# francescovezzi/quadruped-springs

Hardware: AMD Instinct MI355X
Metric: env-steps/sec (whole node), Go1+PEA jump-in-place, N=8192 envs (higher is better)
Workload: dtype f32

## Files before the change

include/qs_amd.h:

```cpp
#ifndef QS_AMD_H
#define QS_AMD_H
#include <stdint.h>

#ifdef __cplusplus
extern "C" {
#endif

enum { QS_ACT_DEFAULT = 0, QS_ACT_SYMMETRIC = 1, QS_ACT_SYMMETRIC_NO_HIP = 2, QS_ACT_CPG = 3  };
enum { QS_MOTOR_PD = 0, QS_MOTOR_CARTESIAN_PD = 1, QS_MOTOR_TORQUE = 2 };
enum {
    QS_TASK_NO_TASK = 0, QS_TASK_JUMPING_IN_PLACE = 1, QS_TASK_JUMPING_FORWARD = 2,
    QS_TASK_CONT_JUMPING_FORWARD = 3, QS_TASK_CONT_JUMPING_FORWARD2 = 4,
    QS_TASK_JUMPING_IN_PLACE_PPO = 5, QS_TASK_JUMPING_FORWARD_PPO = 6, QS_TASK_BACKFLIP = 7,
    QS_TASK_JUMPING_IN_PLACE_PPO_HP = 8, QS_TASK_JUMPING_FORWARD_PPO_HP = 9, QS_TASK_BACKFLIP_PPO = 10,
    QS_TASK_CONT_JUMPING_FORWARD3 = 11, QS_TASK_CONT_JUMPING_FORWARD_PPO = 12,
    QS_TASK_JUMPING_IN_PLACE_DEMO = 13, QS_TASK_JUMPING_FORWARD_DEMO = 14, QS_TASK_BACKFLIP_DEMO = 15,
    QS_TASK_CONT_JUMPING_FORWARD_DEMO = 16,
};
enum {
    QS_SENS_JOINT_POS = 0, QS_SENS_JOINT_VEL = 1, QS_SENS_PITCH = 2, QS_SENS_HEIGHT = 3, QS_SENS_VEL_Z = 4,
    QS_SENS_LANDING = 5, QS_SENS_JUMPING = 6, QS_SENS_PITCH_RATE = 7, QS_SENS_VEL_X = 8, QS_SENS_BOOL_CONTACT = 9,
    QS_SENS_LIN_VEL = 10, QS_SENS_ANG_VEL = 11, QS_SENS_FEET_POS = 12, QS_SENS_FEET_VEL = 13,
    QS_SENS_PITCH_BACKFLIP = 14, QS_SENS_RPY = 15, QS_SENS_QUAT = 16,
};
#define QS_RAND_GROUND 1
#define QS_RAND_MASSES 2
#define QS_RAND_SPRINGS 4
#define QS_RAND_KEEP 8
enum { QS_WRAP_NONE = 0, QS_WRAP_LANDING = 1, QS_WRAP_GO_TO_REST = 2, QS_WRAP_LANDING2 = 3, QS_WRAP_LANDING_BACKFLIP = 4,
       QS_WRAP_LANDING_BACKFLIP2 = 5, QS_WRAP_LANDING_CONTINUOUS = 6 };
enum { QS_PHASE_POLICY = 0, QS_PHASE_TAKEOFF = 1, QS_PHASE_LANDING = 2, QS_PHASE_REST = 3 };

#define QS_MAX_SENSORS 16
#define QS_MAX_OBS 64
#define QS_STATE_DIM 37
#define QS_PARAM_DIM 24
#define QS_TASK_DIM 48
#define QS_TRACE_DIM 70

typedef struct qs_config {
    int32_t n_envs;
    int32_t action_dim;
    int32_t action_space_mode;
    int32_t motor_control_mode;
    int32_t symm_idx;
    int32_t rl_interface;
    int32_t task;
    int32_t n_sensors;
    int32_t sensors[QS_MAX_SENSORS];
    int32_t obs_dim;
    int32_t enable_springs;
    int32_t enable_filter;
    int32_t enable_interp;
    int32_t action_repeat;
    int32_t solver_iters;
    int32_t settle_steps;
    int32_t max_sim_steps;
    int32_t randomizer_flags;
    int32_t noise_enabled;
    int32_t auto_reset;
    int32_t reset_lookahead;
    int32_t env_id_offset;
    int32_t wrapper_mode;
    uint64_t seed;
    double dt;
    double filt_b[3], filt_a[3];
    float gravity;
    float kp[3], kd[3], tau_max[3];
    float cmd_lo[12], cmd_hi[12];
    float settle_cmd[12];
    float settle_action[12];
    float spring_k[3], spring_b[3], spring_rest[3];
    float fallen_height;
    float leg_len[3];
    float contact_erp, joint_erp, warmstart, vel_cap;
    float obs_noise_std[QS_MAX_OBS];
    float task_p[16];
    float contact_slop;
    int32_t body_contacts;
    int32_t self_collision;
    int32_t info_fields;
    int32_t payload_soft;
    float support_margin;
    float reserved_f[2];
    float cpg_phi[16];
    float cpg_lo[5], cpg_hi[5];
    float cpg_clearance, cpg_penetration, cpg_coupling, cpg_alpha;
    float solver_residual_threshold;
    int32_t friction_cone;
    float landing_action[12];
    float landing_kp, landing_kd;
    float rest_kp, rest_kd, rest_time;
    float reserved_h[3];
    float unit_inertia[4][6];
} qs_config;

typedef struct qs_handle qs_handle;

int qs_create(const qs_config* cfg, int device, qs_handle** out);
typedef struct qs_rack {
    int32_t on;
    float anchor_pos[3];
    float anchor_quat[4];
} qs_rack;
int qs_create_ex(const qs_config* cfg, const qs_rack* rack, int device, qs_handle** out);
int qs_set_rack(qs_handle* h, const uint8_t* mask, int hung);
void qs_destroy(qs_handle* h);
int qs_set_stream(qs_handle* h, void* hip_stream);
int qs_reset(qs_handle* h, const uint8_t* mask);
int qs_reset_to(qs_handle* h, const uint8_t* mask, const float* states);
int qs_get_obs(qs_handle* h, float* obs );
int qs_set_demo(qs_handle* h, const float* rows, int length);
int qs_set_demo_counter(qs_handle* h, const uint8_t* mask, const int32_t* values);
int qs_step(qs_handle* h, const float* actions , float* obs , float* rew ,
            uint8_t* done , uint8_t* truncated );
int qs_get_state(qs_handle* h, float* state );
enum { QS_FRAME_LINK = 1, QS_FRAME_WORLD = 2 };
int qs_set_external_wrench(qs_handle* h, const uint8_t* mask, const float* wrench , const int32_t* substeps , int frame);
int qs_set_state(qs_handle* h, const float* state );
enum {
    QS_INFO_FOOT_FORCE = 0, QS_INFO_FOOT_CONTACT = 1, QS_INFO_TORQUE = 2, QS_INFO_SPRING_TORQUE = 3, QS_INFO_TASK = 4,
    QS_INFO_N_INVALID = 5, QS_INFO_PARAMS = 6, QS_INFO_COUNTERS = 7, QS_INFO_LAST_ACTION = 8, QS_INFO_TERMINAL_OBS = 9,
    QS_INFO_FILTERED_ACTION = 11,
    QS_INFO_REWARD_END = 12,
    QS_INFO_PAYLOAD_BLOCK = 13,
    QS_INFO_WRAPPER = 10,
    QS_INFO_EXTERNAL_WRENCH = 14,
    QS_INFO_RACK = 15,
};
int qs_info_dim(const qs_handle* h, int which);
int qs_get_info(qs_handle* h, int which, float* out );
enum { QS_PARAM_MU = 0, QS_PARAM_SPRING_K = 1, QS_PARAM_SPRING_B = 2, QS_PARAM_KP = 3, QS_PARAM_KD = 4, QS_PARAM_ALL = 5 };
int qs_set_params(qs_handle* h, int which, const float* vals);
int qs_stats(qs_handle* h, uint64_t* settle_substeps, uint64_t* resets);
int qs_step_fused(qs_handle* h, const float* actions, float* fused);
typedef struct qs_host_result {
    const float* obs;
    const float* rew;
    const uint8_t* done;
    const uint8_t* truncated;
    const float* terminal_rows;
    int32_t terminal_cap;
} qs_host_result;
int qs_host_step_begin(qs_handle* h, const float* actions);
int qs_host_step_end(qs_handle* h, qs_host_result* out);

enum { QS_COUNTER_SETTLE_SUBSTEPS = 0,
       QS_COUNTER_RESETS = 1,
       QS_COUNTER_LOOKAHEAD_SERVED = 2,
       QS_COUNTER_LOOKAHEAD_SETTLED = 3,
       QS_COUNTER_LIMIT_PATH_SUBSTEPS = 4,
       QS_COUNTER_SELF_NARROW_SUBSTEPS = 5,
       QS_COUNTER_RESET_STALLS = 6,
       QS_COUNTER_LOOKAHEAD_BACKLOG = 7      };
int qs_counter(qs_handle* h, int which, uint64_t* value);
int qs_counters_async(qs_handle* h, uint64_t* dev_out);
int qs_enable_timing(qs_handle* h, int on);
int qs_last_step_kernel_ms(qs_handle* h, float* ms);
int qs_settle_lanes(qs_handle* h, int on);
int qs_set_trace(qs_handle* h, int env, float* rows);

typedef struct qs_norm qs_norm;
int qs_norm_create(int n_envs, int obs_dim, double clip_obs, double clip_reward, double gamma, double epsilon, int device, qs_norm** out);
void qs_norm_destroy(qs_norm* h);
int qs_norm_set_stream(qs_norm* h, void* hip_stream);
int qs_norm_set_stats(qs_norm* h, const double* obs_mean, const double* obs_var, double obs_count, double ret_mean, double ret_var, double ret_count);
int qs_norm_dims(const qs_norm* h, int* n_envs, int* obs_dim, int* device);
int qs_norm_get_stats(qs_norm* h, double* obs_mean, double* obs_var, double* obs_count, double* ret_mean, double* ret_var, double* ret_count);
int qs_norm_reset(qs_norm* h, float* obs , int training, int norm_obs);
int qs_norm_step(qs_norm* h, float* obs , float* rew , const uint8_t* done , float* term_obs ,
                 int training, int norm_obs, int norm_reward, float* raw_obs, float* raw_rew);

typedef struct qs_norm_io {
    float* obs; float* rew; const uint8_t* done; const uint8_t* trunc; float* term_obs; float* tail_rows; int32_t tail_cap;
    float* out_obs; float* out_rew; uint8_t* out_done; uint8_t* out_trunc; float* out_tail;
    float* raw_obs; float* raw_rew;
    const uint64_t* tail_count;
} qs_norm_io;
int qs_norm_step_io(qs_norm* h, const qs_norm_io* io, int training, int norm_obs, int norm_reward);
int qs_host_set_norm(qs_handle* h, qs_norm* norm, int training, int norm_obs, int norm_reward, float* raw_obs, float* raw_rew);

typedef struct qs_camera {
    float target[3];
    float distance, yaw_deg, pitch_deg, fov_deg, near_clip, far_clip;
    int32_t follow_base;
    int32_t draw_payload;
} qs_camera;
int qs_render(qs_handle* h, const int32_t* env_ids, int m, const qs_camera* cam, int width, int height,
              uint32_t* rgba , float* depth , int32_t* seg );
int qs_render_states(const float* states, const float* params, int m, const qs_camera* cam, int width, int height,
                     uint32_t* rgba, float* depth, int32_t* seg, void* stream);

#define QS_POLICY_MAX_HIDDEN 4
enum { QS_POLICY_ACT_NONE = 0, QS_POLICY_ACT_TANH = 1, QS_POLICY_ACT_RELU = 2 };
typedef struct qs_policy qs_policy;
typedef struct qs_policy_desc {
    int32_t n_envs, n_policies, obs_dim, action_dim, n_hidden, hidden[QS_POLICY_MAX_HIDDEN];
    int32_t activation;
    int32_t squash_output;
    int32_t has_bias;
    float clip_lo, clip_hi;
} qs_policy_desc;
int qs_policy_create(const qs_policy_desc* d, int device, qs_policy** out);
void qs_policy_destroy(qs_policy* p);
int qs_policy_set_stream(qs_policy* p, void* hip_stream);
int qs_policy_param_count(const qs_policy* p);
int qs_policy_set_params(qs_policy* p, const float* dev_params);
int qs_policy_act(qs_policy* p, const float* obs, const float* eps, const float* log_std, float* actions, float* mean_out, float* log_prob);

typedef struct qs_ac qs_ac;
int qs_ac_create(const qs_policy_desc* actor, const qs_policy_desc* critic, int device, qs_ac** out);
void qs_ac_destroy(qs_ac* h);
int qs_ac_set_stream(qs_ac* h, void* hip_stream);
int qs_ac_set_params(qs_ac* h, const float* actor_params, const float* critic_params);
int qs_ac_collect(qs_ac* h, const float* obs, const float* eps, const float* log_std, float* env_actions, float* obs_row, float* action_row,
                  float* value_row, float* log_prob_row);
int qs_ac_values(qs_ac* h, const float* obs, const uint8_t* mask_or_null, float* values_out);
int qs_ac_bootstrap(qs_ac* h, const float* terminal_obs, const uint8_t* truncated, float gamma, float* rewards_inout);
int qs_gae(const float* rewards, const float* values, const float* episode_starts, const float* last_values, const uint8_t* last_dones, int T, int N,
           float gamma, float lambda, float* advantages, float* returns, void* hip_stream);

typedef struct qs_ppo qs_ppo;
typedef struct qs_ppo_hyper {
    float clip_range, ent_coef, vf_coef;
    float max_grad_norm;
    int32_t normalize_advantage;
    int32_t reserved;
    double lr, beta_one, beta_two, adam_eps;
} qs_ppo_hyper;
enum { QS_PPO_STAT_POLICY_LOSS = 0, QS_PPO_STAT_VALUE_LOSS = 1, QS_PPO_STAT_ENTROPY_LOSS = 2, QS_PPO_STAT_APPROX_KL = 3,
       QS_PPO_STAT_CLIP_FRACTION = 4, QS_PPO_STAT_GRAD_NORM = 5, QS_PPO_STAT_REFUSED = 6, QS_PPO_STAT_LOSS = 7, QS_PPO_N_STATS = 8 };
int qs_ppo_create(const qs_policy_desc* actor, const qs_policy_desc* critic, int max_batch, int device, qs_ppo** out);
void qs_ppo_destroy(qs_ppo* h);
int qs_ppo_set_stream(qs_ppo* h, void* hip_stream);
int qs_ppo_bind(qs_ppo* h, float* actor_params, float* critic_params, float* log_std, float* exp_avg, float* exp_avg_sq);
int qs_ppo_grad(qs_ppo* h, const float* observations, const float* actions, const float* old_log_prob, const float* advantages, const float* returns,
                long long total, const long long* indices, int batch, const qs_ppo_hyper* hyper, float* grad_out, float* stats_out);
int qs_ppo_adam(qs_ppo* h, const float* grad, const qs_ppo_hyper* hyper, int step, float* stats_inout);
int qs_ppo_refusals(qs_ppo* h, unsigned long long* out);

struct qs_snapshot_info {
    uint64_t bytes;
    int32_t n_envs, row_floats, rec_floats, push_floats, obs_dim;
    int32_t layout_version;
    uint64_t layout_digest;
    uint64_t config_digest;
};
int qs_snapshot_info(const qs_handle* h, struct qs_snapshot_info* out);
int qs_snapshot(qs_handle* h, const uint8_t* mask, float* rows);
int qs_restore(qs_handle* h, const uint8_t* mask, const float* rows);
int qs_fork(qs_handle* h, const int32_t* src_of);
int qs_norm_get_returns(qs_norm* h, double* returns );
int qs_norm_set_returns(qs_norm* h, const double* returns );

const char* qs_last_error(void);
const char* qs_version(void);
#define QS_ABI_VERSION 9
int qs_abi_version(void);

#ifdef __cplusplus
}
#endif
#endif
```

quadruped-springs_amd/csrc/qs_core.h:

```cpp
#pragma once
#include "qs_lane.h"
#include "qs_layout.h"
#include "../../include/qs_amd.h"

#if defined(QS_PROFILE_PHASES) && defined(__HIPCC__)
__device__ unsigned long long qs_phase_cycles[48];
__device__ unsigned long long qs_phase_t0, qs_phase_sub0;
#endif
#if defined(QS_PROFILE_PHASES) && defined(__HIP_DEVICE_COMPILE__)
#define QS_PHASE_BEGIN if (blockIdx.x == 0 && threadIdx.x == 0) qs_phase_t0 = __builtin_readcyclecounter();
#define QS_PHASE_G(k) if (blockIdx.x == 0 && threadIdx.x == 0) { unsigned long long n_ = __builtin_readcyclecounter(); qs_phase_cycles[k] += n_ - qs_phase_t0; qs_phase_t0 = n_; }
#define QS_PHASE(k) QS_PHASE_G(k)
#define QS_PHASE_SUB(k) if (blockIdx.x == 0 && threadIdx.x == 0) { qs_phase_cycles[16 + ((k) < 15 ? (k) : 15)] += __builtin_readcyclecounter() - qs_phase_sub0; }
#define QS_PHASE_SUB_BEGIN if (blockIdx.x == 0 && threadIdx.x == 0) qs_phase_sub0 = __builtin_readcyclecounter();
#define QS_PHASE_END
#elif defined(QS_COUNT_PHASES) && defined(__HIP_DEVICE_COMPILE__)
#define QS_PHASE_BEGIN { __builtin_amdgcn_sched_barrier(0); asm volatile("; QS_PHASE_MARK 0"); __builtin_amdgcn_sched_barrier(0); }
#define QS_PHASE_G(k) { __builtin_amdgcn_sched_barrier(0); asm volatile("; QS_PHASE_MARK " #k); __builtin_amdgcn_sched_barrier(0); }
#define QS_PHASE(k) QS_PHASE_G(k)
#define QS_PHASE_SUB(k)
#define QS_PHASE_SUB_BEGIN
#define QS_PHASE_END
#else
#define QS_PHASE_BEGIN
// ... 1145 lines not shown
        M rare_mine = qgt(T::quad_sum(qflag(any_lim)), V(0.5f));
        State s_r = s; Out o_r = o;
        PayRows pay_c, pay_r;
        if (!HOT && soft) payload_rows(cfg, Pr, s, vs, Rx, Ry, Rz, Sm, Ld, blk, pay_c);
        if (!HOT && rack) rack_rows(cfg, s, vs, Rx, Ry, Rz, Sm, Ld, blk, pay_c);
        QS_PHASE_G(39)
        if (!HOT && T::any(qor(any_lim, any_extra))) {
            Row xr[12];
#pragma unroll
            for (int r = 0; r < 3; r++) xr[r] = rows[r];
#pragma unroll
            for (int r = 3; r < 12; r++) {
                Row& e_ = xr[r];
                e_.rhs = zero; e_.dinv = zero; e_.act = zero; e_.diag = zero;
#pragma unroll
                for (int i = 0; i < 6; i++) e_.w[i] = zero;
#pragma unroll
                for (int i = 0; i < 3; i++) { e_.jq[i] = zero; e_.u[i] = zero; }
            }
            M extra_live = qlt(one, zero);
#if defined(QS_PROBE_WARM) && defined(__HIP_DEVICE_COMPILE__)
            M probe_live[2] = {qlt(one, zero), qlt(one, zero)};
#endif
#if defined(QS_PROBE_LAZY) && defined(__HIP_DEVICE_COMPILE__)
            M probe_rule[2][4];
#pragma unroll
            for (int a_ = 0; a_ < 2; a_++)
#pragma unroll
                for (int m_ = 0; m_ < 4; m_++) probe_rule[a_][m_] = qlt(one, zero);
#endif
            const M lim_env = qgt(T::quad_sum(qflag(any_lim)), V(0.5f));
            if (T::any(any_extra)) {
                const V bigh = V(1e9f);
                V hh[5] = {qsel(qlt(h_trunk, V(THR_TRUNK)), h_trunk, bigh), qsel(qlt(h_hip, V(THR_HIP)), h_hip, bigh), qsel(qlt(h_th_hi, V(THR_THIGH)), h_th_hi, bigh),
                           qsel(qlt(h_th_lo, V(THR_THIGH)), h_th_lo, bigh), qsel(qlt(h_cf_hi, V(THR_CALF)), h_cf_hi, bigh)};
                V sgz = qsel(qlt(Rz.z, zero), -one, one), sga = qsel(qlt(az, zero), -one, one);
                V sg2 = qsel(qlt(gx2, zero), -one, one), sg3 = qsel(qlt(gx3, zero), -one, one);
                V rad = HIP_CYL_R * qrsqrt(qmax(one - az * az, V(1e-12f)));
                V3v pc[5];
                pc[0] = mk3<V>(fx * TRUNK_HALF[0], sy * TRUNK_HALF[1], sgz * (-TRUNK_HALF[2]));
                pc[1] = p1 - Y * (sga * HIP_CYL_HALF_LEN) - (Rz - Y * az) * rad;
                V3v toff = X2 * (sg2 * THIGH_HALF[0]) + Y * (sga * THIGH_HALF[1]);
                pc[2] = p2 - toff; pc[3] = p3 - toff;
                pc[4] = p3 - X3 * (sg3 * CALF_HALF[0]) - Y * (sga * CALF_HALF[1]);
                const float depth[5] = {0.0f, 1.0f, 2.0f, 2.0f, 3.0f};
                const M foot_off = qnot(act_m);
#pragma unroll
                for (int pass = 0; pass < 3; pass++) {
                    const int slot = pass - 1;
                    const M elig = pass == 0 ? foot_off : qlt(zero, one);
                    V best = qsel(elig, hh[0], bigh), bi = zero;
#pragma unroll
                    for (int i = 1; i < 5; i++) { M m = qand(elig, qlt(hh[i], best)); best = qsel(m, hh[i], best); bi = qsel(m, V((float)i), bi); }
                    if (!T::any(qlt(best, V(1e8f)))) { if (pass == 0) continue; else break; }
                    bi = qsel(qlt(best, V(1e8f)), bi, V(4.0f));
                    V3v pt = pc[0]; V dep = V(depth[0]);
#pragma unroll
                    for (int i = 1; i < 5; i++) {
                        M m = qgt(bi, V(i - 0.5f));
                        pt = mk3<V>(qsel(m, pc[i].x, pt.x), qsel(m, pc[i].y, pt.y), qsel(m, pc[i].z, pt.z));
                        dep = qsel(m, V(depth[i]), dep);
                    }
#pragma unroll
                    for (int i = 0; i < 5; i++) hh[i] = qsel(qand(qlt(best, V(1e8f)), qand(qgt(bi, V(i - 0.5f)), qlt(bi, V(i + 0.5f)))), bigh, hh[i]);
                    V dist_x = qsel(qlt(best, V(1e8f)), best, zero);
                    V f1 = qflag(qgt(dep, V(0.5f))), f2 = qflag(qgt(dep, V(1.5f))), f3 = qflag(qgt(dep, V(2.5f)));
                    V3v e1 = cross(ax1, pt - p1) * f1, e2 = cross(Y, pt - p2) * f2, e3 = cross(Y, pt - p3) * f3;
                    V3v jan = cross(pt, Rz);
                    V reln = jan.x * vs.a.x + jan.y * vs.a.y + jan.z * vs.a.z + Rz.x * vs.l.x + Rz.y * vs.l.y + Rz.z * vs.l.z +
                             dot(Rz, e1) * s.qd[0] + dot(Rz, e2) * s.qd[1] + dot(Rz, e3) * s.qd[2];
                    V pen_x = dist_x + cfg.contact_slop;
                    M live = qand(qlt(best, V(1e8f)), qor(qor(lim_env, qle(pen_x, zero)), qgt((-reln) - pen_x * inv_dt, V(-cfg.support_margin))));
#if defined(QS_PROBE_LAZY) && defined(__HIP_DEVICE_COMPILE__)
#pragma unroll
                    for (int m_ = 0; m_ < 4; m_++) probe_rule[slot][m_] = qand(qlt(best, V(1e8f)), qor(qor(lim_env, qle(pen_x, zero)), qgt((-reln) - pen_x * inv_dt, V(-0.25f * (float)((1 << m_) >> 1)))));
                    live = qlt(best, V(1e8f));
#endif
                    extra_live = qor(extra_live, live);
#if defined(QS_PROBE_WARM) && defined(__HIP_DEVICE_COMPILE__)
                    probe_live[pass == 0 ? 0 : slot] = pass == 0 ? probe_live[0] : live;
#endif
                    if (!T::any(live)) continue;
                    V act_x = qflag(live);
                    if (pass == 0) {
                        Row t0_, t1_, t2_;
                        QS_CONTACT_ROW_AT(t0_, Rz, true, pt, e1, e2, e3, dist_x, act_x)
                        QS_CONTACT_ROW_AT(t1_, (mk3<V>(-Ry.x, -Ry.y, -Ry.z)), false, pt, e1, e2, e3, dist_x, act_x)
                        QS_CONTACT_ROW_AT(t2_, Rx, false, pt, e1, e2, e3, dist_x, act_x)
                        const Row* tt_[3] = {&t0_, &t1_, &t2_};
#pragma unroll
                        for (int r = 0; r < 3; r++) {
                            Row& d_ = xr[r]; const Row& a_ = *tt_[r];
#pragma unroll
                            for (int i = 0; i < 6; i++) d_.w[i] = qsel(live, a_.w[i], d_.w[i]);
#pragma unroll
                            for (int i = 0; i < 3; i++) { d_.jq[i] = qsel(live, a_.jq[i], d_.jq[i]); d_.u[i] = qsel(live, a_.u[i], d_.u[i]); }
                            d_.rhs = qsel(live, a_.rhs, d_.rhs); d_.dinv = qsel(live, a_.dinv, d_.dinv); d_.diag = qsel(live, a_.diag, d_.diag); d_.act = qsel(live, a_.act, d_.act);
                        }
                    } else {
                        QS_CONTACT_ROW_AT(xr[3 + 3 * slot], Rz, true, pt, e1, e2, e3, dist_x, act_x)
                        QS_CONTACT_ROW_AT(xr[4 + 3 * slot], (mk3<V>(-Ry.x, -Ry.y, -Ry.z)), false, pt, e1, e2, e3, dist_x, act_x)
                        QS_CONTACT_ROW_AT(xr[5 + 3 * slot], Rx, false, pt, e1, e2, e3, dist_x, act_x)
                    }
                }
            }
            rare_mine = qgt(T::quad_sum(qflag(qor(any_lim, extra_live))), V(0.5f));
#if defined(QS_PROBE_WARM) && defined(__HIP_DEVICE_COMPILE__)
            {
                unsigned long long* pc = reinterpret_cast<const QsDevCfg&>(cfg).counters + 2;
                const float pts_leg = qflag(probe_live[0]) + qflag(probe_live[1]);
                const float pts = T::quad_sum(pts_leg), two = T::quad_sum(pts_leg > 1.5f ? 1.0f : 0.0f);
                const bool mine = rare_mine, lim = lim_env;
                const bool simple = mine && !lim && two < 0.5f;
                const unsigned long long b0 = __ballot(mine), b1 = __ballot(mine && lim), b2 = __ballot(mine && !lim && two > 0.5f),
                                         b3 = __ballot(simple && pts < 1.5f), b4 = __ballot(simple && pts > 1.5f && pts < 2.5f), b5 = __ballot(simple && pts > 2.5f);
                if (threadIdx.x == 0) {
                    atomicAdd(&pc[0], (unsigned long long)(__popcll(b0) / 4)); atomicAdd(&pc[1], (unsigned long long)(__popcll(b1) / 4));
                    atomicAdd(&pc[2], (unsigned long long)(__popcll(b2) / 4)); atomicAdd(&pc[3], (unsigned long long)(__popcll(b3) / 4));
                    atomicAdd(&pc[4], (unsigned long long)(__popcll(b4) / 4)); atomicAdd(&pc[5], (unsigned long long)(__popcll(b5) / 4));
                    atomicAdd(&pc[6], 1ull);
                    if (b0) atomicAdd(&pc[7], 1ull);
                    if (b0 && b0 == (b3 | b4 | b5)) atomicAdd(&pc[8], 1ull);
                }
            }
#endif
            if (T::any(rare_mine)) {
                T::count_rare_path(cfg);
                if (T::any(any_lim)) { QS_LIMIT_ROWS(xr + 9) }
                QS_PHASE_G(40)
                V lam12[12], plam[6];
                if (soft || rack) pay_r = pay_c;
                RareSolver<T, CONE>::solve(cfg, Pr.mu, xr, (soft || rack) ? &pay_r : nullptr, rare_mine, s.warm * cfg.warmstart * rows[0].act, T::wave_scratch(scratch_row), lam12, plam);
                integrate_rare(cfg, s_r, o_r, xr, lam12, Sm, Ld, BK, R, (soft || rack) ? &pay_r : nullptr, plam, active);
#if defined(QS_PROBE_LAZY) && defined(__HIP_DEVICE_COMPILE__)
                {
                    unsigned long long* pc = reinterpret_cast<const QsDevCfg&>(cfg).counters + 2;
                    const bool ext_q = T::quad_sum(qflag(any_extra)) > 0.5f;
                    const bool zero_q = !lim_env && T::quad_sum(qabs(lam12[3]) + qabs(lam12[6])) == 0.0f;
                    const unsigned long long b0 = __ballot(ext_q), b1 = __ballot(ext_q && zero_q);
                    if (threadIdx.x == 0) { atomicAdd(&pc[0], (unsigned long long)(__popcll(b0) / 4)); atomicAdd(&pc[1], (unsigned long long)(__popcll(b1) / 4)); }
#pragma unroll
                    for (int m_ = 0; m_ < 4; m_++) {
                        const bool keep_q = lim_env || T::quad_sum(qflag(probe_rule[0][m_]) + qflag(probe_rule[1][m_])) > 0.5f;
                        const float w0 = !probe_rule[0][m_] && qabs(lam12[3]) > 0.0f ? 1.0f : 0.0f, w1 = !probe_rule[1][m_] && qabs(lam12[6]) > 0.0f ? 1.0f : 0.0f;
                        const bool wrong_q = T::quad_sum(w0 + w1) > 0.5f;
                        const unsigned long long bk = __ballot(ext_q && keep_q), bw = __ballot(ext_q && wrong_q);
                        if (threadIdx.x == 0) { atomicAdd(&pc[2 + 2 * m_], (unsigned long long)(__popcll(bk) / 4)); atomicAdd(&pc[3 + 2 * m_], (unsigned long long)(__popcll(bw) / 4)); }
                    }
                }
#endif
                QS_PHASE_G(45)
            }
        }
        if (RACK ? rack : (SOFT || (!HOT && soft))) {
            if (HOT && !RACK) payload_rows(cfg, Pr, s, vs, Rx, Ry, Rz, Sm, Ld, blk, pay_c);
            if (HOT && RACK) rack_rows(cfg, s, vs, Rx, Ry, Rz, Sm, Ld, blk, pay_c);
            if (cfg.solver_residual_threshold > 0.0f) solve_and_integrate<3, true, true>(cfg, Pr.mu, s, o, rows, Sm, Ld, BK, R, &pay_c);
            else solve_and_integrate<3, false, true>(cfg, Pr.mu, s, o, rows, Sm, Ld, BK, R, &pay_c);
            if (HOT && !RACK) payload_integrate(cfg, blk, pay_c);
            if (HOT && RACK) rack_store(blk, pay_c);
        } else {
            if (cfg.solver_residual_threshold > 0.0f) solve_and_integrate<3, true>(cfg, Pr.mu, s, o, rows, Sm, Ld, BK, R);
            else solve_and_integrate<3, false>(cfg, Pr.mu, s, o, rows, Sm, Ld, BK, R);
        }
        if (!HOT) {
#pragma unroll
            for (int j = 0; j < 3; j++) s.qd[j] = qsel(rare_mine, s_r.qd[j], s.qd[j]);
            s.vang = mk3<V>(qsel(rare_mine, s_r.vang.x, s.vang.x), qsel(rare_mine, s_r.vang.y, s.vang.y), qsel(rare_mine, s_r.vang.z, s.vang.z));
            s.vlin = mk3<V>(qsel(rare_mine, s_r.vlin.x, s.vlin.x), qsel(rare_mine, s_r.vlin.y, s.vlin.y), qsel(rare_mine, s_r.vlin.z, s.vlin.z));
            s.warm = qsel(rare_mine, s_r.warm, s.warm); o.foot_force = qsel(rare_mine, o_r.foot_force, o.foot_force);
            if (soft) { keep_rare_payload(pay_c, pay_r, rare_mine); payload_integrate(cfg, blk, pay_c); }
            if (rack) { keep_rare_payload(pay_c, pay_r, rare_mine); rack_store(blk, pay_c); }
        }
#undef QS_LIMIT_ROWS
#undef QS_CONTACT_ROW_AT
        } else {
            o.foot_force = zero; s.warm = zero;
        }
        QS_PHASE(11)
        s.pos.x = s.pos.x + dt * s.vlin.x; s.pos.y = s.pos.y + dt * s.vlin.y; s.pos.z = s.pos.z + dt * s.vlin.z;
        {
            V th2 = dot(s.vang, s.vang) * (dt * dt);
            V sc = V(0.5f * dt) * (one - th2 * (1.0f / 24.0f) * (one - th2 * (1.0f / 80.0f)));
            V dw = one - th2 * 0.125f * (one - th2 * (1.0f / 48.0f));
            V dx = s.vang.x * sc, dy = s.vang.y * sc, dz = s.vang.z * sc;
            V nx = dw * s.qx + dx * s.qw + dy * s.qz - dz * s.qy;
            V ny = dw * s.qy - dx * s.qz + dy * s.qw + dz * s.qx;
            V nz = dw * s.qz + dx * s.qy - dy * s.qx + dz * s.qw;
            V nw = dw * s.qw - dx * s.qx - dy * s.qy - dz * s.qz;
            V inv = qrsqrt(nx * nx + ny * ny + nz * nz + nw * nw);
            s.qx = nx * inv; s.qy = ny * inv; s.qz = nz * inv; s.qw = nw * inv;
        }
#pragma unroll
        for (int j = 0; j < 3; j++) s.q[j] = s.q[j] + dt * s.qd[j];
        QS_PHASE(12)
        QS_PHASE_END
        return HOT && hand_over_next ? 2 : 0;
    }
};

}
```

quadruped-springs_amd/csrc/qs_hip.hip:

```cpp
#include <hip/hip_runtime.h>
#include <stdio.h>
#include <stdlib.h>
#include <string.h>
#include <new>
#include "qs_env.h"
#include "qs_host.h"

using qs::Env;
using E = Env<LaneDev>;

#define QS_TILE_FLOATS (QS_ENVS_PER_WAVE * QS_REC_END)
#ifndef QS_LEAN_WAVES
#define QS_LEAN_WAVES(W) ((W) == 2)
#endif

enum { TILE_INFO = QS_INFO_END, TILE_ALL = QS_REC_END };
__device__ __forceinline__ int tile_extent(const qs_config& cfg, bool store) {
    if (cfg.payload_soft) return TILE_ALL;
    if (cfg.info_fields) return store ? TILE_INFO : QS_HOT_ALL;
    if (cfg.action_space_mode == QS_ACT_CPG || E::demo_task(cfg.task)) return QS_HOT_ALL;
    if (cfg.wrapper_mode != QS_WRAP_NONE) return QS_HOT_WRAP;
    return QS_HOT;
}
__device__ __forceinline__ void keep_loaded(const float4& v) { asm volatile("" ::"v"(v.x), "v"(v.y), "v"(v.z), "v"(v.w)); }
__device__ __forceinline__ void keep_loaded(float v) { asm volatile("" ::"v"(v)); }
template <int PER> __device__ __forceinline__ void tile_load_rounds(float4* __restrict__ dst, const float4* __restrict__ src, int nenv, int stride4, int per_rt) {
    constexpr int MAX_PER = QS_REC_END / 4;
    constexpr int ROUNDS = PER > 0 ? (QS_ENVS_PER_WAVE * PER + QS_WAVE - 1) / QS_WAVE : (QS_ENVS_PER_WAVE * MAX_PER + QS_WAVE - 1) / QS_WAVE;
    const int per = PER > 0 ? PER : per_rt, total = QS_ENVS_PER_WAVE * per;
    const unsigned inv = ((1u << 20) + (unsigned)per - 1u) / (unsigned)per;
    float4 v[ROUNDS];
#pragma unroll
    for (int r = 0; r < ROUNDS; r++) {
        const int i = (int)threadIdx.x + r * QS_WAVE;
        const bool in = (PER > 0 && (QS_ENVS_PER_WAVE * PER) % QS_WAVE == 0) || i < total;
        const int e = PER > 0 ? i / PER : (int)(((unsigned)i * inv) >> 20), o = i - e * per;
        v[r] = src[in ? (e < nenv ? e : 0) * (QS_REC / 4) + o : 0];
    }
    if (!(PER > 0 && (QS_ENVS_PER_WAVE * PER) % QS_WAVE == 0)) {
#pragma unroll
        for (int r = 0; r < ROUNDS; r++) keep_loaded(v[r]);
    }
#pragma unroll
    for (int r = 0; r < ROUNDS; r++) {
        const int i = (int)threadIdx.x + r * QS_WAVE;
        if ((PER > 0 && (QS_ENVS_PER_WAVE * PER) % QS_WAVE == 0) || i < total) {
            const int e = PER > 0 ? i / PER : (int)(((unsigned)i * inv) >> 20), o = i - e * per;
            dst[e * stride4 + o] = v[r];
        }
    }
}
__device__ __forceinline__ void tile_load(float* lds, const float* __restrict__ g, int first_env, int n_envs, int extent, int stride = QS_REC_END) {
    const float4* src = reinterpret_cast<const float4*>(g + (size_t)first_env * QS_REC);
    float4* dst = reinterpret_cast<float4*>(lds);
    const int nenv = min(QS_ENVS_PER_WAVE, n_envs - first_env);
    if (extent == QS_HOT) tile_load_rounds<QS_HOT / 4>(dst, src, nenv, stride / 4, 0);
    else if (extent == QS_SETTLE_END) tile_load_rounds<QS_SETTLE_END / 4>(dst, src, nenv, stride / 4, 0);
    else tile_load_rounds<0>(dst, src, nenv, stride / 4, extent / 4);
}
template <int PER> __device__ __forceinline__ void tile_store_rounds(float4* __restrict__ dst, const float4* __restrict__ src, int nenv, int stride4, int b4, int per_rt) {
    constexpr int MAX_PER = QS_REC_END / 4;
    constexpr int ROUNDS = PER > 0 ? (QS_ENVS_PER_WAVE * PER + QS_WAVE - 1) / QS_WAVE : (QS_ENVS_PER_WAVE * MAX_PER + QS_WAVE - 1) / QS_WAVE;
    const int per = PER > 0 ? PER : per_rt, total = nenv * per;
    const unsigned inv = ((1u << 20) + (unsigned)per - 1u) / (unsigned)per;
    float4 v[ROUNDS];
#pragma unroll
    for (int r = 0; r < ROUNDS; r++) {
        const int i = (int)threadIdx.x + r * QS_WAVE;
        const int e = PER > 0 ? i / PER : (int)(((unsigned)i * inv) >> 20), o = i - e * per + b4;
        v[r] = src[i < total ? e * stride4 + o : 0];
    }
#pragma unroll
    for (int r = 0; r < ROUNDS; r++) keep_loaded(v[r]);
#pragma unroll
    for (int r = 0; r < ROUNDS; r++) {
        const int i = (int)threadIdx.x + r * QS_WAVE;
        if (i < total) { const int e = PER > 0 ? i / PER : (int)(((unsigned)i * inv) >> 20), o = i - e * per + b4; dst[e * (QS_REC / 4) + o] = v[r]; }
    }
}
__device__ __forceinline__ void tile_store(const float* lds, float* __restrict__ g, int first_env, int n_envs, int begin, int end, int stride = QS_REC_END) {
    float4* dst = reinterpret_cast<float4*>(g + (size_t)first_env * QS_REC);
    const float4* src = reinterpret_cast<const float4*>(lds);
    const int nenv = min(QS_ENVS_PER_WAVE, n_envs - first_env);
    if (begin == QS_RW_BEGIN && end == QS_HOT) tile_store_rounds<(QS_HOT - QS_RW_BEGIN) / 4>(dst, src, nenv, stride / 4, QS_RW_BEGIN / 4, 0);
    else if (begin == QS_RW_BEGIN && end == QS_SETTLE_END) tile_store_rounds<(QS_SETTLE_END - QS_RW_BEGIN) / 4>(dst, src, nenv, stride / 4, QS_RW_BEGIN / 4, 0);
    else tile_store_rounds<0>(dst, src, nenv, stride / 4, begin / 4, (end - begin) / 4);
}

__device__ __forceinline__ void obs_store(const float* s_obs, int nrow, int od, int first, float* __restrict__ obs_out, bool fused, float* __restrict__ obs_keep) {
    const unsigned inv = (65536u + (unsigned)od - 1u) / (unsigned)od;
    const int row = fused ? od + 2 : od, total = nrow * od;
    constexpr int ROUNDS = QS_ENVS_PER_WAVE * QS_MAX_OBS / QS_WAVE;
    float v[ROUNDS];
#pragma unroll
    for (int r = 0; r < ROUNDS; r++) {
        const int i = (int)threadIdx.x + r * QS_WAVE;
        const int e = (int)(((unsigned)i * inv) >> 16), o = i - e * od;
        v[r] = s_obs[i < total ? e * QS_MAX_OBS + o : 0];
    }
#pragma unroll
    for (int r = 0; r < ROUNDS; r++) keep_loaded(v[r]);
#pragma unroll
    for (int r = 0; r < ROUNDS; r++) {
        const int i = (int)threadIdx.x + r * QS_WAVE;
        if (i < total) {
            const int e = (int)(((unsigned)i * inv) >> 16), o = i - e * od;
            obs_out[(size_t)(first + e) * row + o] = v[r];
            obs_keep[(size_t)first * od + i] = v[r];
        }
    }
}

struct LookAhead {
    float* slots;
    int* cur;
    int* handed;
    int K;
};
#define QS_COHORTS 5
#define QS_MAX_SLICE 2048
struct SettleLanes { float* staging; const int2* stage_jobs; int n_env_waves, slice; int wave0[QS_COHORTS + 1] ,
                     spawn[QS_COHORTS], last[QS_COHORTS], settle_n[QS_COHORTS]; };
struct TraceTap { float* rows; int env; };
struct DemoTab { const float* rows; int length; };
struct TermTail { float* rows; int cap, parity; };
struct PushTab { float* rows; };
enum { QS_PUSH_F = 8, QS_PUSH_REM = 6, QS_PUSH_FRAME = 7 };
enum { CTL_SETTLE_SUBSTEPS = 0, CTL_RESETS = 1, CTL_SERVED = 2, CTL_SETTLED = 3, CTL_BACKLOG = 4, CTL_STALLS = 6,
       CTL_R = 8 , CTL_TERM_CNT = 8 + QS_COHORTS , CTL_DEV = 10 + QS_COHORTS ,
       CTL_PUSH_REFUSED = 22 + QS_COHORTS ,
       CTL_RENDER_REFUSED = 23 + QS_COHORTS ,
       CTL_FORK_REFUSED = 24 + QS_COHORTS ,
       CTL_N = 25 + QS_COHORTS };

__device__ __forceinline__ float copy_settled(float* rec, const float* __restrict__ src, bool block) {
    static_assert(R_PARAMS == 0 && R_PARAMS + QS_PARAM_DIM == R_POS, "parameters and rigid-body state are one range");
    const int lane = threadIdx.x & 3;
    constexpr int END_A = R_WARM + 4, NA = (END_A + 3) / 4;
    constexpr int NB = (R_TAU_SPRING + 12 - R_FOOT_FORCE) / 4;
    constexpr int NC = QS_BLOCK_DIM / 4;
    static_assert((R_TAU_SPRING + 12 - R_FOOT_FORCE) % 4 == 0 && QS_BLOCK_DIM % 4 == 0, "whole rounds");
    float a[NA], b[NB], c[NC];
#pragma unroll
    for (int k = 0; k < NA; k++) { const int i = lane + 4 * k; a[k] = src[i < END_A ? i : 0]; }
#pragma unroll
    for (int k = 0; k < NB; k++) b[k] = src[R_FOOT_FORCE + lane + 4 * k];
    const float ninv = src[R_N_INVALID], tag = src[R_EPISODE];
    if (block) {
#pragma unroll
        for (int k = 0; k < NC; k++) c[k] = src[R_BLOCK + lane + 4 * k];
    }
#pragma unroll
    for (int k = 0; k < NA; k++) { const int i = lane + 4 * k; if (i < END_A) rec[i] = a[k]; }
#pragma unroll
    for (int k = 0; k < NB; k++) rec[R_FOOT_FORCE + lane + 4 * k] = b[k];
    if (lane == 0) rec[R_N_INVALID] = ninv;
    if (block) {
#pragma unroll
        for (int k = 0; k < NC; k++) rec[R_BLOCK + lane + 4 * k] = c[k];
    }
    return tag;
}
__device__ __forceinline__ void quad_row_store(float* __restrict__ dst, const float* row, int n) {
    float v[QS_MAX_OBS / 4];
#pragma unroll
    for (int k = 0; k < QS_MAX_OBS / 4; k++) { const int i = (int)(threadIdx.x & 3) + 4 * k; v[k] = row[i < n ? i : 0]; }
#pragma unroll
    for (int k = 0; k < QS_MAX_OBS / 4; k++) keep_loaded(v[k]);
#pragma unroll
    for (int k = 0; k < QS_MAX_OBS / 4; k++) { const int i = (int)(threadIdx.x & 3) + 4 * k; if (i < n) dst[i] = v[k]; }
}
__device__ __forceinline__ bool lookahead_take(const LookAhead& la, unsigned long long* __restrict__ ctl, float* rec, int env, int X, bool block, bool count = true) {
    if (la.K == 0) return false;
    const float* slot = la.slots + ((size_t)env * la.K + (size_t)(X % la.K)) * QS_REC;
    const float tag = copy_settled(rec, slot, block);
    const bool ready = qs::f2i(tag) == X;
    if ((threadIdx.x & 3) == 0) {
        la.cur[env] = X;
        if (count) atomicAdd(&ctl[ready ? CTL_SERVED : CTL_STALLS], 1ull);
    }
    return ready;
}
__device__ __forceinline__ void zero_tile_tail(float* lds, int from, int stride) {
    const int per = stride - from;
    for (int i = threadIdx.x; i < QS_ENVS_PER_WAVE * per; i += QS_WAVE) { const int e = i / per; lds[e * stride + from + (i - e * per)] = 0.0f; }
}

__global__ __launch_bounds__(QS_WAVE, 1) void k_init(const qs_config* __restrict__ cfgp, float* __restrict__ recs) {
    const qs_config& cfg = *cfgp;
    int env = blockIdx.x * QS_ENVS_PER_WAVE + (threadIdx.x >> 2);
    if (env >= cfg.n_envs) return;
    float* r = recs + (size_t)env * QS_REC;
    for (int i = threadIdx.x & 3; i < QS_REC_END; i += 4) r[i] = 0.0f;
    LaneDev::sync();
    if ((threadIdx.x & 3) == 0) qs::init_record_row(r);
    E::randomize(cfg, r, (uint32_t)(env + cfg.env_id_offset), -1, true);
}

template <bool CONE, int WAVES, bool SOFT, bool RACK = false> static __device__ __forceinline__ void step_body(const qs_config* __restrict__ cfgp, float* __restrict__ recs,
                                                 const float* __restrict__ actions, float* __restrict__ obs_out,
                                                 float* __restrict__ rew_out, uint8_t* __restrict__ done_out,
                                                 uint8_t* __restrict__ trunc_out, float* __restrict__ obs_keep,
                                                 float* __restrict__ term_obs, LookAhead la,
                                                 unsigned long long* __restrict__ stats, SettleLanes lanes, TraceTap tap, DemoTab demo, TermTail tail,
                                                 PushTab push) {
    using E = Env<LaneDev, CONE, false, false, RACK>;
    using EH = Env<LaneDev, CONE, true, SOFT, RACK>;
    extern __shared__ __attribute__((aligned(16))) float s_dyn[];
    const qs_config& cfg = *cfgp;
    const int ls = (RACK || cfg.payload_soft) ? (int)QS_REC_END : (int)QS_INFO_END;
    float* const s_rec = s_dyn;
    float* const s_obs = s_dyn + QS_ENVS_PER_WAVE * ls;
    float* const s_act = s_obs + QS_ENVS_PER_WAVE * QS_MAX_OBS;
    QS_PHASE_BEGIN
    if (tail.rows && blockIdx.x == 0 && threadIdx.x == 0) stats[CTL_TERM_CNT + (tail.parity ^ 1)] = 0ull;
    const bool settling = (int)blockIdx.x >= lanes.n_env_waves;
    const int sw = (int)blockIdx.x - lanes.n_env_waves;
    int cohort = 0;
#pragma unroll
    for (int c = 1; c < QS_COHORTS; c++) cohort += settling && sw >= lanes.wave0[c] ? 1 : 0;
    const int first = settling ? cohort * lanes.slice + (sw - lanes.wave0[cohort]) * QS_ENVS_PER_WAVE : (int)blockIdx.x * QS_ENVS_PER_WAVE;
    const int limit = settling ? cohort * lanes.slice + (int)stats[CTL_R + cohort] : cfg.n_envs;
    if (first >= limit) return;
    const int settle_n = settling ? lanes.settle_n[cohort] : 0;
    if (settling && settle_n == 0) return;
    float* const base = settling ? lanes.staging : recs;
    const int slot = threadIdx.x >> 2;
    const int env = first + slot;
    const bool valid = env < limit;
    const int d = cfg.action_dim, od = cfg.obs_dim;
    QS_PHASE(26)
    float a_pre[3] = {0.0f, 0.0f, 0.0f};
    float p_rem = 0.0f;
    int2 job = make_int2(0, 0);
    if (!settling) {
#pragma unroll
        for (int j = 0; j < 3; j++) {
            const int k = (int)(threadIdx.x & 3u) + 4 * j;
            if (k < d && valid) a_pre[j] = actions[(size_t)env * d + k];
        }
        if (push.rows && valid) p_rem = push.rows[(size_t)env * QS_PUSH_F + QS_PUSH_REM];
    } else job = lanes.stage_jobs[valid ? env : first];
    const bool spawn = settling && lanes.spawn[cohort], last = settling && lanes.last[cohort];
    const int load_extent = settling ? (spawn ? 0 : ((RACK || cfg.payload_soft) ? (int)TILE_ALL : (int)QS_SETTLE_END)) : (RACK ? (int)TILE_ALL : tile_extent(cfg, false));
    if (load_extent > 0) tile_load(s_rec, base, first, limit, load_extent, ls);
    if (spawn || last) zero_tile_tail(s_rec, load_extent, ls);
    QS_PHASE(27)
    if (!settling) {
#pragma unroll
        for (int j = 0; j < 3; j++) {
            const int k = (int)(threadIdx.x & 3u) + 4 * j;
            if (k < d) s_act[slot * 12 + k] = a_pre[j];
        }
    }
    QS_PHASE(28)
    __syncthreads();
    QS_PHASE(29)
    float* rec = s_rec + slot * ls;
    float* ob = s_obs + slot * QS_MAX_OBS;
    if (cfg.info_fields && !settling && (threadIdx.x & 3) == 0) rec[QS_INFO_END - 1] = 0.0f;
    const uint32_t gid = (uint32_t)((settling ? job.x : env) + cfg.env_id_offset);
    if (spawn) { E::settle_spawn(cfg, rec, gid, job.y); LaneDev::sync(); }
    const bool any_trace = tap.rows != nullptr && !settling && tap.env >= first && tap.env < first + QS_ENVS_PER_WAVE;
    QS_PHASE(13)
    float* const trow = any_trace && env == tap.env ? tap.rows : nullptr;
    const bool any_push = push.rows != nullptr && __any(p_rem > 0.0f);
    const float* const prow = any_push ? push.rows + (size_t)(valid ? env : first) * QS_PUSH_F : nullptr;
    typename E::StepOut r;
    {
        const typename EH::StepOut rh = EH::template step<false, QS_LEAN_WAVES(WAVES)>(cfg, rec, s_act + slot * 12, ob, gid, settle_n, trow, any_trace, demo.rows, demo.length, 0, prow);
        r.reward = rh.reward; r.done = rh.done; r.trunc = rh.trunc; r.resume = rh.resume;
    }
    if (__builtin_expect(r.resume >= 0, 0)) r = E::template step<true>(cfg, rec, s_act + slot * 12, ob, gid, settle_n, trow, any_trace, demo.rows, demo.length, r.resume, prow);
    QS_PHASE(14)
    if (settling) {
        if (valid && (threadIdx.x & 3) == 0) atomicAdd(&stats[CTL_SETTLE_SUBSTEPS], (unsigned long long)settle_n);
        __syncthreads();
        tile_store(s_rec, base, first, limit, spawn ? 0 : (int)QS_RW_BEGIN,
                   (RACK || cfg.payload_soft) ? (int)TILE_ALL : (last ? (int)TILE_INFO : (int)QS_SETTLE_END), ls);
        return;
    }
    const bool dn = r.done > 0.5f;
    if (any_push && valid && p_rem > 0.0f && (threadIdx.x & 3) == 0)
        push.rows[(size_t)env * QS_PUSH_F + QS_PUSH_REM] = dn ? 0.0f : fmaxf(p_rem - (float)cfg.action_repeat, 0.0f);
    if (valid && (threadIdx.x & 3) == 0) {
        if (rew_out) { rew_out[env] = r.reward; done_out[env] = dn ? 1 : 0; trunc_out[env] = r.trunc > 0.5f ? 1 : 0; }
        else {
            float* row = obs_out + (size_t)env * (od + 2);
            row[od] = r.reward; row[od + 1] = (dn ? 1.0f : 0.0f) + (r.trunc > 0.5f ? 2.0f : 0.0f);
        }
    }
    bool any_reset = false;
    if (cfg.auto_reset) {
        const bool do_reset = dn && valid;
        if (__builtin_expect(__any(do_reset), 0)) {
            any_reset = true;
            LaneDev::sync();
            bool ahead = false;
            if (do_reset) {
                quad_row_store(term_obs + (size_t)env * od, ob, od);
                if ((threadIdx.x & 3) == 0) atomicAdd(&stats[CTL_RESETS], 1ull);
                if (tail.rows) {
                    int at = 0;
                    if ((threadIdx.x & 3) == 0) at = (int)atomicAdd(&stats[CTL_TERM_CNT + tail.parity], 1ull);
                    at = __shfl(at, (int)(threadIdx.x & ~3u));
                    if (at < tail.cap) {
                        float* row = tail.rows + (size_t)at * (od + 1);
                        if ((threadIdx.x & 3) == 0) row[0] = qs::i2f(env);
                        quad_row_store(row + 1, ob, od);
                    }
                }
                ahead = lookahead_take(la, stats, rec, env, qs::f2i(rec[R_EPISODE]) + 1, RACK || cfg.payload_soft != 0);
            }
            LaneDev::sync();
            if (__builtin_expect(__any(do_reset && !ahead), 0)) {
                __syncthreads();
                tile_store(s_rec, recs, first, cfg.n_envs, QS_RW_BEGIN, RACK ? (int)TILE_ALL : tile_extent(cfg, true), ls);
                obs_store(s_obs, min(QS_ENVS_PER_WAVE, cfg.n_envs - first), od, first, obs_out, rew_out == nullptr, obs_keep);
                __syncthreads();
                E::reset(cfg, rec, ob, gid, true);
                if (do_reset && !ahead && (threadIdx.x & 3) == 0) atomicAdd(&stats[CTL_SETTLE_SUBSTEPS], (unsigned long long)cfg.settle_steps);
                LaneDev::sync();
                if (do_reset) {
                    float* g = recs + (size_t)env * QS_REC;
                    const int end = RACK ? (int)TILE_ALL : tile_extent(cfg, true);
                    for (int i = threadIdx.x & 3; i < end; i += 4) g[i] = rec[i];
                    for (int i = threadIdx.x & 3; i < od; i += 4) {
                        if (rew_out) obs_out[(size_t)env * od + i] = ob[i];
                        else obs_out[(size_t)env * (od + 2) + i] = ob[i];
                        obs_keep[(size_t)env * od + i] = ob[i];
                    }
                }
                return;
            }
            if (do_reset) E::reset(cfg, rec, ob, gid, false);
        }
    }
    __syncthreads();
    tile_store(s_rec, recs, first, cfg.n_envs, any_reset ? 0 : (int)QS_RW_BEGIN, RACK ? (int)TILE_ALL : tile_extent(cfg, true), ls);
    obs_store(s_obs, min(QS_ENVS_PER_WAVE, cfg.n_envs - first), od, first, obs_out, rew_out == nullptr, obs_keep);
    QS_PHASE(15)
}

#define QS_STEP_ARGS const qs_config* __restrict__ cfgp, float* __restrict__ recs, const float* __restrict__ actions, float* __restrict__ obs_out,    \
                     float* __restrict__ rew_out, uint8_t* __restrict__ done_out, uint8_t* __restrict__ trunc_out, float* __restrict__ obs_keep, \
                     float* __restrict__ term_obs, LookAhead la, unsigned long long* __restrict__ stats, SettleLanes lanes, TraceTap tap, DemoTab demo, TermTail tail, \
                     PushTab push
#define QS_STEP_PASS cfgp, recs, actions, obs_out, rew_out, done_out, trunc_out, obs_keep, term_obs, la, stats, lanes, tap, demo, tail, push
template <bool CONE, bool SOFT> __global__ __launch_bounds__(QS_WAVE, 1) void k_step(QS_STEP_ARGS) { step_body<CONE, 1, SOFT>(QS_STEP_PASS); }
template <bool CONE, bool SOFT> __global__ __launch_bounds__(QS_WAVE, 2) void k_step_dense(QS_STEP_ARGS) { step_body<CONE, 2, SOFT>(QS_STEP_PASS); }
template <bool CONE> __global__ __launch_bounds__(QS_WAVE, 1) void k_step_rack(QS_STEP_ARGS) { step_body<CONE, 1, CONE, true>(QS_STEP_PASS); }
template <bool CONE> __global__ __launch_bounds__(QS_WAVE, 2) void k_step_dense_rack(QS_STEP_ARGS) { step_body<CONE, 2, CONE, true>(QS_STEP_PASS); }

__global__ void k_lookahead_publish(unsigned long long* __restrict__ ctl, const float* __restrict__ staging, const int2* __restrict__ stage_jobs,
                                    LookAhead la, int cohort, int slice) {
    const int n = (int)ctl[CTL_R + cohort];
    const float* src = staging + (size_t)cohort * slice * QS_REC;
    const int2* jobs = stage_jobs + (size_t)cohort * slice;
    for (size_t i = (size_t)blockIdx.x * blockDim.x + threadIdx.x; i < (size_t)n * QS_REC_END; i += (size_t)gridDim.x * blockDim.x) {
        const int e = (int)(i / QS_REC_END), f = (int)(i % QS_REC_END);
        const int2 job = jobs[e];
        if (job.y <= la.cur[job.x]) continue;
        float* dst = la.slots + ((size_t)job.x * la.K + (size_t)(job.y % la.K)) * QS_REC;
        dst[f] = f == R_EPISODE ? qs::i2f(job.y) : src[(size_t)e * QS_REC + f];
        if (f == 0) atomicAdd(&ctl[CTL_SETTLED], 1ull);
    }
}
__global__ __launch_bounds__(1024) void k_lookahead_plan(unsigned long long* __restrict__ ctl, LookAhead la, int n_envs, int2* __restrict__ stage_jobs, int cohort,
                                                          int slice, int base_cap, int take, int offset) {
    __shared__ int s_count, s_want, s_urgent;
    if (threadIdx.x == 0) { s_count = 0; s_want = 0; s_urgent = 0; }
    __syncthreads();
    int2* dst = stage_jobs + (size_t)cohort * slice;
    for (int pass = 0; pass < 2; pass++) {
        const int cap = take ? (pass == 0 ? slice : (s_count > base_cap ? 0 : base_cap)) : 0;
        for (int i = threadIdx.x; i < n_envs; i += blockDim.x) {
            const int e = (i + offset) % n_envs;
            const int X = la.cur[e];
            int h = la.handed[e];
            if (h < X) h = X;
            const int want = X + la.K - h;
            if (want <= 0 || (4 * want > la.K) != (pass == 0)) continue;
            atomicAdd(&s_want, want);
            if (cap <= 0) continue;
            const int at = atomicAdd(&s_count, want);
            int took = 0;
            for (int j = 0; j < want && at + j < cap; j++) { dst[at + j] = make_int2(e, h + 1 + j); took++; }
            if (took) la.handed[e] = h + took;
        }
        __syncthreads();
        if (threadIdx.x == 0 && pass == 0) { if (s_count > slice) s_count = slice; s_urgent = s_count; }
        __syncthreads();
    }
    if (threadIdx.x == 0) {
        int n = s_count;
        const int lim = s_urgent > base_cap ? s_urgent : base_cap;
        if (n > lim) n = lim;
        if (take) ctl[CTL_R + cohort] = (unsigned long long)n;
        ctl[CTL_BACKLOG] = (unsigned long long)(s_want - (take ? n : 0));
    }
}
__global__ void k_lookahead_requeue(unsigned long long* __restrict__ ctl, LookAhead la, const int2* __restrict__ stage_jobs, int slice) {
    for (int c = 0; c < QS_COHORTS; c++) {
        const int n = (int)ctl[CTL_R + c];
        for (int i = threadIdx.x; i < n; i += blockDim.x) { const int2 job = stage_jobs[(size_t)c * slice + i]; atomicMin(&la.handed[job.x], job.y - 1); }
    }
    __syncthreads();
    if (threadIdx.x == 0) for (int c = 0; c < QS_COHORTS; c++) ctl[CTL_R + c] = 0;
}

template <bool CONE, bool RACK> static __device__ __forceinline__ void reset_body(const qs_config* __restrict__ cfgp, float* __restrict__ recs,
                                                      const uint8_t* __restrict__ mask, float* __restrict__ obs_keep,
                                                      unsigned long long* __restrict__ stats, const float* __restrict__ states, LookAhead la,
                                                      float* __restrict__ push_rows, float* s_rec, float* s_obs) {
    using E = Env<LaneDev, CONE, false, false, RACK>;
    const qs_config& cfg = *cfgp;
    const int first = blockIdx.x * QS_ENVS_PER_WAVE;
    const int slot = threadIdx.x >> 2, env = first + slot;
    const bool valid = env < cfg.n_envs;
    const bool sel = valid && (mask == nullptr || mask[env] != 0);
    if (!__any(sel)) return;
    tile_load(s_rec, recs, first, cfg.n_envs, QS_REC_END);
    const int od = cfg.obs_dim;
    __syncthreads();
    float* rec = s_rec + slot * QS_REC_END;
    float* ob = s_obs + slot * QS_MAX_OBS;
    const uint32_t gid = (uint32_t)((valid ? env : 0) + cfg.env_id_offset);
    bool ahead = false;
    if (sel) {
        if (states == nullptr) ahead = lookahead_take(la, stats, rec, env, qs::f2i(rec[R_EPISODE]) + 1, RACK || cfg.payload_soft != 0);
        else if (la.K > 0 && (threadIdx.x & 3) == 0) la.cur[env] = qs::f2i(rec[R_EPISODE]) + 1;
        if ((threadIdx.x & 3) == 0) atomicAdd(&stats[CTL_RESETS], 1ull);
        if ((threadIdx.x & 3) == 0) push_rows[(size_t)env * QS_PUSH_F + QS_PUSH_REM] = 0.0f;
    }
    bool write_back = false;
    if (states) {
        if (sel) {
            E::randomize(cfg, rec, gid, qs::f2i(rec[R_EPISODE]) + 1, false);
            for (int i = threadIdx.x & 3; i < 37; i += 4) rec[R_POS + i] = states[(size_t)env * 37 + i];
            for (int i = threadIdx.x & 3; i < 4; i += 4) rec[R_WARM + i] = 0.0f;
            if (RACK) for (int i = threadIdx.x & 3; i < 6; i += 4) rec[R_BLOCK + RK_LAM + i] = 0.0f;
            if ((threadIdx.x & 3) == 0) {
                for (int i = 0; i < 4; i++) { rec[R_FOOT_FORCE + i] = 0.0f; rec[R_FOOT_CONTACT + i] = 0.0f; }
                rec[R_N_INVALID] = 0.0f;
                for (int i = 0; i < 24; i++) rec[R_TAU_PD + i] = 0.0f;
            }
        }
        LaneDev::sync();
        if (cfg.payload_soft) { E::place_block(cfg, rec); LaneDev::sync(); }
        E::reset(cfg, rec, ob, gid, false);
        LaneDev::sync();
        if (sel)
            for (int i = threadIdx.x & 3; i < 12 + 24 + 24; i += 4) rec[R_LAST_ACTION + i] = 0.0f;
        write_back = sel;
    } else {
        LaneDev::sync();
        if (ahead) {
            E::reset(cfg, rec, ob, gid, false);
            float* g = recs + (size_t)env * QS_REC;
            for (int i = threadIdx.x & 3; i < QS_REC_END; i += 4) g[i] = rec[i];
            for (int i = threadIdx.x & 3; i < od; i += 4) obs_keep[(size_t)env * od + i] = ob[i];
        }
        const bool settle = sel && !ahead;
        if (__any(settle)) {
            __syncthreads();
            E::reset(cfg, rec, ob, gid, true);
            if (settle && (threadIdx.x & 3) == 0) atomicAdd(&stats[CTL_SETTLE_SUBSTEPS], (unsigned long long)cfg.settle_steps);
        }
        write_back = settle;
    }
    __syncthreads();
    if (write_back) {
        float* g = recs + (size_t)env * QS_REC;
        for (int i = threadIdx.x & 3; i < QS_REC_END; i += 4) g[i] = rec[i];
        for (int i = threadIdx.x & 3; i < od; i += 4) obs_keep[(size_t)env * od + i] = ob[i];
    }
}
#define QS_RESET_ARGS const qs_config* __restrict__ cfgp, float* __restrict__ recs, const uint8_t* __restrict__ mask, float* __restrict__ obs_keep, \
                      unsigned long long* __restrict__ stats, const float* __restrict__ states, LookAhead la, float* __restrict__ push_rows
#define QS_RESET_PASS cfgp, recs, mask, obs_keep, stats, states, la, push_rows
#define QS_RESET_LDS __shared__ __attribute__((aligned(16))) float s_rec[QS_TILE_FLOATS]; __shared__ __attribute__((aligned(16))) float s_obs[QS_ENVS_PER_WAVE * QS_MAX_OBS];
template <bool CONE> __global__ __launch_bounds__(QS_WAVE, 1) void k_reset(QS_RESET_ARGS) { QS_RESET_LDS reset_body<CONE, false>(QS_RESET_PASS, s_rec, s_obs); }
template <bool CONE> __global__ __launch_bounds__(QS_WAVE, 1) void k_reset_rack(QS_RESET_ARGS) { QS_RESET_LDS reset_body<CONE, true>(QS_RESET_PASS, s_rec, s_obs); }

template <bool CONE, bool RACK> static __device__ __forceinline__ void lookahead_fill_body(const qs_config* __restrict__ cfgp, LookAhead la, float* s_rec, float* s_obs) {
    using E = Env<LaneDev, CONE, false, false, RACK>;
    const qs_config& cfg = *cfgp;
    const int slot = threadIdx.x >> 2;
    const long long j = (long long)blockIdx.x * QS_ENVS_PER_WAVE + slot, total = (long long)cfg.n_envs * la.K;
    const int env = (int)((j < total ? j : 0) % cfg.n_envs), episode = (int)((j < total ? j : 0) / cfg.n_envs);
    float* rec = s_rec + slot * QS_REC_END;
    for (int i = threadIdx.x & 3; i < QS_REC_END; i += 4) rec[i] = 0.0f;
    LaneDev::sync();
    if ((threadIdx.x & 3) == 0) rec[R_EPISODE] = qs::i2f(episode - 1);
    LaneDev::sync();
    E::reset(cfg, rec, s_obs + slot * QS_MAX_OBS, (uint32_t)(env + cfg.env_id_offset), true);
    LaneDev::sync();
    if (j < total) {
        float* g = la.slots + ((size_t)env * la.K + (size_t)(episode % la.K)) * QS_REC;
        for (int i = threadIdx.x & 3; i < QS_REC_END; i += 4) g[i] = rec[i];
        if (episode == la.K - 1 && (threadIdx.x & 3) == 0) { la.handed[env] = la.K - 1; la.cur[env] = -1; }
    }
}
template <bool CONE> __global__ __launch_bounds__(QS_WAVE, 1) void k_lookahead_fill(const qs_config* __restrict__ cfgp, LookAhead la) { QS_RESET_LDS lookahead_fill_body<CONE, false>(cfgp, la, s_rec, s_obs); }
template <bool CONE> __global__ __launch_bounds__(QS_WAVE, 1) void k_lookahead_fill_rack(const qs_config* __restrict__ cfgp, LookAhead la) { QS_RESET_LDS lookahead_fill_body<CONE, true>(cfgp, la, s_rec, s_obs); }
#undef QS_RESET_LDS

__global__ void k_gather(const float* __restrict__ recs, int n, int off, int dim, float* __restrict__ out, int as_int) {
    int i = blockIdx.x * blockDim.x + threadIdx.x;
    if (i >= n * dim) return;
    float v = recs[(size_t)(i / dim) * QS_REC + off + i % dim];
    out[i] = as_int ? (float)qs::f2i(v) : v;
}
__global__ void k_scatter(float* __restrict__ recs, int n, int off, int dim, const float* __restrict__ in, int zero_warm) {
    int i = blockIdx.x * blockDim.x + threadIdx.x;
    if (i >= n * dim) return;
    recs[(size_t)(i / dim) * QS_REC + off + i % dim] = in[i];
    if (zero_warm && i % dim < 4) recs[(size_t)(i / dim) * QS_REC + R_WARM + i % dim] = 0.0f;
}
__global__ void k_task_info(const float* __restrict__ recs, int n, float* __restrict__ out, int demo, int info) {
    int e = blockIdx.x * blockDim.x + threadIdx.x;
    if (e >= n) return;
    const float* r = recs + (size_t)e * QS_REC;
    float* o = out + (size_t)e * QS_TASK_DIM;
    for (int k = 0; k < T_N; k++) o[k] = r[R_TASK + k];
    for (int k = 0; k < 9; k++) o[T_N + k] = info ? r[R_POSE_CACHE + k] : 0.0f;
    o[41] = r[R_N_INVALID];
    o[42] = info ? r[R_FOOT_FORCE] + r[R_FOOT_FORCE + 1] + r[R_FOOT_FORCE + 2] + r[R_FOOT_FORCE + 3] : 0.0f;
    o[43] = (float)qs::f2i(r[R_SIM_STEP]);
    o[44] = demo ? r[R_DEMO] : 0.0f; o[45] = demo ? r[R_DEMO + 1] : 0.0f;
    for (int k = 46; k < QS_TASK_DIM; k++) o[k] = 0.0f;
}

__global__ void k_set_rack(float* __restrict__ recs, int n, const uint8_t* __restrict__ mask, int hung) {
    const int e = blockIdx.x * blockDim.x + threadIdx.x;
    if (e >= n || (mask && !mask[e])) return;
    qs::set_rack_row(recs + (size_t)e * QS_REC, hung);
}

__global__ void k_rack_info(const float* __restrict__ recs, int n, float inv_dt, float ax, float ay, float az, float* __restrict__ out) {
    const int e = blockIdx.x * blockDim.x + threadIdx.x;
    if (e >= n) return;
    qs::rack_info_row(recs + (size_t)e * QS_REC, inv_dt, ax, ay, az, out + (size_t)e * 8);
}

#ifdef QS_ISA_ONLY
#if defined(QS_ISA_PYRAMID)
template __global__ void k_step<false, false>(QS_STEP_ARGS);
#elif !defined(QS_ISA_DENSE)
template __global__ void k_step<true, false>(QS_STEP_ARGS);
#else
template __global__ void k_step_dense<true, false>(QS_STEP_ARGS);
#endif
#else
thread_local char qs_g_err[512] = "";
int qs_check_device(int device) {
    int ndev = 0;
    hipError_t derr = hipGetDeviceCount(&ndev);
    if (derr != hipSuccess || ndev <= 0)
        QS_FAIL(-3, "no HIP device available (hipGetDeviceCount: %s, %d devices): this library has no CPU path", hipGetErrorString(derr), ndev);
    if (device < 0 || device >= ndev) QS_FAIL(-3, "HIP device %d out of range (%d visible)", device, ndev);
    return 0;
}

struct HostPath;
struct qs_handle {
    qs_config cfg;
    int device;
    hipStream_t stream;
    qs_config* d_cfg;
    float* d_rec;
    float* d_obs;
    float* d_term_obs;
    LookAhead la;
    float* d_staging;
    int2* d_stage_jobs;
    int slice;
    int lanes_on;
    long long tick;
    float* trace_rows; int trace_env;
    float* d_demo; int demo_len;
    float* d_push;
    float* d_fork;
    qs_rack rack;
    int push_live;
    int n_simd, step_variant;
    unsigned long long* d_stats;
    TermTail tail;
    struct HostPath* host;
    hipEvent_t ev0, ev1;
    int timing;
    long long timed_launches;
};

static int sensor_dim(int s) {
    switch (s) {
    case QS_SENS_JOINT_POS: case QS_SENS_JOINT_VEL: case QS_SENS_FEET_POS: case QS_SENS_FEET_VEL: return 12;
    case QS_SENS_BOOL_CONTACT: case QS_SENS_QUAT: return 4;
    case QS_SENS_LIN_VEL: case QS_SENS_ANG_VEL: case QS_SENS_RPY: return 3;
    default: return 1;
    }
}
static int n_waves(int n) { return (n + QS_ENVS_PER_WAVE - 1) / QS_ENVS_PER_WAVE; }
static qs::Build handle_build(const qs_handle* h) { return qs::Build::of(h->cfg, h->rack.on != 0); }

#define QS_STR2(x) #x
#define QS_STR(x) QS_STR2(x)

extern "C" {

const char* qs_last_error(void) { return qs_g_err; }
#ifndef QS_SOURCE_SHA
#define QS_SOURCE_SHA "unknown"
#endif
const char* qs_version(void) { return "qs_amd 0.6 (gfx950, quad-per-env; ABI " QS_STR(QS_ABI_VERSION) "; source " QS_SOURCE_SHA ")"; }
int qs_abi_version(void) { return QS_ABI_VERSION; }

static int create_impl(const qs_config* cfg, const qs_rack* rack, int device, qs_handle* h);

int qs_create(const qs_config* cfg, int device, qs_handle** out) { return qs_create_ex(cfg, nullptr, device, out); }

int qs_create_ex(const qs_config* cfg, const qs_rack* rack_in, int device, qs_handle** out) {
    if (!cfg || !out) QS_FAIL(-1, "null argument");
    qs_rack rack;
    memset(&rack, 0, sizeof(rack));
    if (rack_in && rack_in->on) {
        if (rack_in->on != 1) QS_FAIL(-1, "qs_rack::on must be 0 or 1, got %d", rack_in->on);
        if (cfg->payload_soft)
            QS_FAIL(-1, "on_rack together with payload_soft is not supported: both are a six-row fixed constraint on the trunk, and the solvers hold "
                        "one such set; use the welded payload (payload_soft = 0) on a rack");
        double n2 = 0.0;
        bool finite = true;
        auto fin = [](float x) { uint32_t u; memcpy(&u, &x, 4); return (u & 0x7f800000u) != 0x7f800000u; };
        for (int i = 0; i < 3; i++) finite = finite && fin(rack_in->anchor_pos[i]);
        for (int i = 0; i < 4; i++) { finite = finite && fin(rack_in->anchor_quat[i]); n2 += (double)rack_in->anchor_quat[i] * rack_in->anchor_quat[i]; }
        if (!finite || !(n2 > 1e-12)) QS_FAIL(-1, "the rack's anchor needs a finite position and a finite, non-zero quaternion (xyzw)");
        rack.on = 1;
        for (int i = 0; i < 3; i++) rack.anchor_pos[i] = rack_in->anchor_pos[i];
        for (int i = 0; i < 4; i++) rack.anchor_quat[i] = (float)(rack_in->anchor_quat[i] / sqrt(n2));
    }
    if (cfg->n_envs <= 0) QS_FAIL(-1, "n_envs must be positive");
    if (cfg->n_envs > (1 << 24)) QS_FAIL(-1, "n_envs %d exceeds %d environments per handle (16 GB of records); shard over more handles", cfg->n_envs, 1 << 24);
    if (cfg->obs_dim <= 0 || cfg->obs_dim > QS_MAX_OBS || cfg->n_sensors > QS_MAX_SENSORS) QS_FAIL(-1, "observation bundle too large");
    if (cfg->action_dim != 12 && cfg->action_dim != 6 && cfg->action_dim != 4 && cfg->action_dim != 5) QS_FAIL(-1, "action_dim must be 12, 6, 4 or 5 (CPG)");
    if (cfg->wrapper_mode != QS_WRAP_NONE && (cfg->action_space_mode == QS_ACT_CPG || !cfg->rl_interface))
        QS_FAIL(-1, "the landing / go-to-rest phase machine needs an RL action space (not CPG, not raw commands)");
    if (cfg->task >= QS_TASK_JUMPING_IN_PLACE_DEMO && cfg->task <= QS_TASK_CONT_JUMPING_FORWARD_DEMO && (cfg->action_space_mode == QS_ACT_CPG || !cfg->rl_interface))
        QS_FAIL(-1, "the DEMO tasks compare the policy's action with a recorded one: they need an RL action space (not CPG, not raw commands)");
    if (cfg->task < 0 || cfg->task > QS_TASK_CONT_JUMPING_FORWARD_DEMO) QS_FAIL(-1, "unknown task id %d", cfg->task);
    if (cfg->friction_cone != 0 && cfg->friction_cone != 1) QS_FAIL(-1, "friction_cone must be 0 (pyramid) or 1 (implicit cone), got %d", cfg->friction_cone);
    if (cfg->action_repeat < 1 || cfg->action_repeat >= (int)E::RESUME_AT_BOUNDARY)
        QS_FAIL(-1, "action_repeat must be between 1 and %d substeps per env step, got %d", (int)E::RESUME_AT_BOUNDARY - 1, cfg->action_repeat);
    if (cfg->settle_steps < 0 || cfg->settle_steps >= (int)E::RESUME_AT_BOUNDARY)
        QS_FAIL(-1, "settle_steps must be between 0 and %d substeps, got %d", (int)E::RESUME_AT_BOUNDARY - 1, cfg->settle_steps);
    if (cfg->settle_steps == 0 && cfg->reset_lookahead > 0)
        QS_FAIL(-1, "reset_lookahead > 0 settles reset states ahead of time in slices of the settle: it needs settle_steps > 0 (got 0; use reset_lookahead = 0)");
    if (cfg->reset_lookahead < 0 || cfg->reset_lookahead > 64) QS_FAIL(-1, "reset_lookahead must be between 0 (settle inside the step) and 64 reset states per environment, got %d", cfg->reset_lookahead);
    if (cfg->motor_control_mode == QS_MOTOR_TORQUE && cfg->rl_interface)
        QS_FAIL(-1, "the motor control mode TORQUE not implemented yet for RL Gym interface.");
    int od = 0;
    for (int i = 0; i < cfg->n_sensors; i++) od += sensor_dim(cfg->sensors[i]);
    if (od != cfg->obs_dim) QS_FAIL(-1, "obs_dim %d does not match the sensor bundle (%d)", cfg->obs_dim, od);
    if (int rc = qs_check_device(device)) return rc;
    DeviceGuard guard(device);
    qs_handle* h = new (std::nothrow) qs_handle();
    if (!h) QS_FAIL(-4, "out of host memory");
    memset(h, 0, sizeof(*h));
    int rc = create_impl(cfg, &rack, device, h);
    if (rc != 0) { qs_destroy(h); return rc; }
    *out = h;
    return 0;
}

static int create_impl(const qs_config* cfg, const qs_rack* rack, int device, qs_handle* h) {
    h->cfg = *cfg; h->device = device; h->stream = nullptr; h->rack = *rack;
    {
        hipDeviceProp_t prop;
        QS_HIP(hipGetDeviceProperties(&prop, device));
        h->n_simd = 4 * prop.multiProcessorCount;
        const char* v = getenv("QS_STEP_VARIANT");
        h->step_variant = v ? atoi(v) : 0;
    }
    const size_t n = (size_t)cfg->n_envs;
    QS_HIP(hipMalloc(&h->d_cfg, sizeof(QsDevCfg)));
    QS_HIP(hipMalloc(&h->d_rec, n * QS_REC * sizeof(float)));
    QS_HIP(hipMalloc(&h->d_obs, n * cfg->obs_dim * sizeof(float)));
    QS_HIP(hipMalloc(&h->d_term_obs, n * cfg->obs_dim * sizeof(float)));
    QS_HIP(hipMalloc(&h->d_stats, CTL_N * sizeof(unsigned long long)));
    QS_HIP(hipMalloc(&h->d_push, n * QS_PUSH_F * sizeof(float)));
    {
        QsDevCfg dc;
        memset(&dc, 0, sizeof(dc));
        dc.cfg = h->cfg; dc.counters = h->d_stats + CTL_DEV;
        for (int i = 0; i < 3; i++) dc.rack_pos[i] = h->rack.anchor_pos[i];
        for (int i = 0; i < 4; i++) dc.rack_quat[i] = h->rack.anchor_quat[i];
        QS_HIP(hipMemcpy(h->d_cfg, &dc, sizeof(dc), hipMemcpyHostToDevice));
    }
    QS_HIP(hipMemset(h->d_obs, 0, n * cfg->obs_dim * sizeof(float)));
    QS_HIP(hipMemset(h->d_term_obs, 0, n * cfg->obs_dim * sizeof(float)));
    QS_HIP(hipMemset(h->d_stats, 0, CTL_N * sizeof(unsigned long long)));
    QS_HIP(hipMemset(h->d_push, 0, n * QS_PUSH_F * sizeof(float)));
    QS_HIP(hipEventCreate(&h->ev0));
    QS_HIP(hipEventCreate(&h->ev1));
    hipLaunchKernelGGL(k_init, dim3(n_waves(cfg->n_envs)), dim3(QS_WAVE), 0, h->stream, h->d_cfg, h->d_rec);
    QS_HIP(hipGetLastError());
    if (h->rack.on) {
        hipLaunchKernelGGL(k_set_rack, dim3((cfg->n_envs + 255) / 256), dim3(256), 0, h->stream, h->d_rec, cfg->n_envs, (const uint8_t*)nullptr, 1);
        QS_HIP(hipGetLastError());
    }
    memset(&h->la, 0, sizeof(h->la));
    if (cfg->reset_lookahead > 0 && !(cfg->randomizer_flags & QS_RAND_KEEP)) {
        const int K = cfg->reset_lookahead;
        h->la.K = K;
        h->slice = (int)((2 * n + QS_ENVS_PER_WAVE - 1) / QS_ENVS_PER_WAVE * QS_ENVS_PER_WAVE);
        if (h->slice < QS_MAX_SLICE) h->slice = QS_MAX_SLICE;
        if (h->slice > 131072) h->slice = 131072;
        QS_HIP(hipMalloc(&h->la.slots, n * K * QS_REC * sizeof(float)));
        QS_HIP(hipMalloc(&h->la.cur, n * sizeof(int)));
        QS_HIP(hipMalloc(&h->la.handed, n * sizeof(int)));
        QS_HIP(hipMalloc(&h->d_staging, (size_t)QS_COHORTS * h->slice * QS_REC * sizeof(float)));
        QS_HIP(hipMalloc(&h->d_stage_jobs, (size_t)QS_COHORTS * h->slice * sizeof(int2)));
        QS_HIP(hipMemsetAsync(h->d_staging, 0, (size_t)QS_COHORTS * h->slice * QS_REC * sizeof(float), h->stream));
        QS_HIP(hipMemsetAsync(h->d_stage_jobs, 0, (size_t)QS_COHORTS * h->slice * sizeof(int2), h->stream));

        const unsigned fill_grid = (unsigned)((n * K + QS_ENVS_PER_WAVE - 1) / QS_ENVS_PER_WAVE);
        auto launch = [&](auto kernel) { hipLaunchKernelGGL(kernel, dim3(fill_grid), dim3(QS_WAVE), 0, h->stream, h->d_cfg, h->la); };
        qs::with_build(handle_build(h), [&](auto cone, auto, auto rack) {
            if constexpr (rack()) launch(k_lookahead_fill_rack<cone()>); else launch(k_lookahead_fill<cone()>);
        });
        QS_HIP(hipGetLastError());
        h->lanes_on = 1;
    }
    QS_HIP(hipStreamSynchronize(h->stream));
    return 0;
}

static void host_path_free(qs_handle* h);
void qs_destroy(qs_handle* h) {
    if (!h) return;
    QS_ON_DEVICE(h);
    hipStreamSynchronize(h->stream);
    hipFree(h->d_cfg); hipFree(h->d_rec); hipFree(h->d_obs); hipFree(h->d_term_obs); hipFree(h->d_stats);
    if (h->la.slots) hipFree(h->la.slots);
    if (h->la.cur) hipFree(h->la.cur);
    if (h->la.handed) hipFree(h->la.handed);
    if (h->d_staging) hipFree(h->d_staging);
    if (h->d_stage_jobs) hipFree(h->d_stage_jobs);
    if (h->d_demo) hipFree(h->d_demo);
    if (h->d_push) hipFree(h->d_push);
    if (h->d_fork) hipFree(h->d_fork);
    host_path_free(h);
    if (h->ev0) hipEventDestroy(h->ev0);
    if (h->ev1) hipEventDestroy(h->ev1);
    delete h;
}

#if defined(QS_PROBE_LAZY) || defined(QS_PROBE_SWEEPS) || defined(QS_PROBE_WARM)
extern "C" int qs_probe_counters(qs_handle* h, unsigned long long* out10) {
    QS_ON_DEVICE(h);
    QS_HIP(hipStreamSynchronize(h->stream));
    QS_HIP(hipMemcpy(out10, h->d_stats + CTL_DEV + 2, 10 * sizeof(unsigned long long), hipMemcpyDeviceToHost));
    return 0;
}
#endif
int qs_set_stream(qs_handle* h, void* s) { if (!h) QS_FAIL(-1, "null handle"); h->stream = (hipStream_t)s; return 0; }
int qs_enable_timing(qs_handle* h, int on) {
    if (!h) QS_FAIL(-1, "null handle");
    if (on == 2) {
        if (h->timing != 2 || h->timed_launches <= 0) QS_FAIL(-1, "no step has been launched since qs_enable_timing(h, 1)");
        QS_ON_DEVICE(h);
        QS_HIP(hipEventRecord(h->ev1, h->stream));
        h->timing = 3;
        return 0;
    }
    h->timing = on ? 1 : 0; h->timed_launches = 0;
    return 0;
}

static void launch_reset(qs_handle* h, const uint8_t* mask, const float* states) {
    auto launch = [&](auto kernel) {
        hipLaunchKernelGGL(kernel, dim3(n_waves(h->cfg.n_envs)), dim3(QS_WAVE), 0, h->stream, h->d_cfg, h->d_rec, mask, h->d_obs, h->d_stats, states, h->la, h->d_push);
    };
    qs::with_build(handle_build(h), [&](auto cone, auto, auto rack) {
        if constexpr (rack()) launch(k_reset_rack<cone()>); else launch(k_reset<cone()>);
    });
}

int qs_reset(qs_handle* h, const uint8_t* mask) {
    if (!h) QS_FAIL(-1, "null handle");
    QS_ON_DEVICE(h);
    launch_reset(h, mask, nullptr);
    QS_HIP(hipGetLastError());
    if (!mask) h->push_live = 0;
    return 0;
}

int qs_reset_to(qs_handle* h, const uint8_t* mask, const float* states) {
    if (!h || !states) QS_FAIL(-1, "null argument");
    QS_ON_DEVICE(h);
    launch_reset(h, mask, states);
    QS_HIP(hipGetLastError());
    if (!mask) h->push_live = 0;
    return 0;
}

int qs_get_obs(qs_handle* h, float* obs) {
    if (!h || !obs) QS_FAIL(-1, "null argument");
    QS_ON_DEVICE(h);
    QS_HIP(hipMemcpyAsync(obs, h->d_obs, (size_t)h->cfg.n_envs * h->cfg.obs_dim * sizeof(float), hipMemcpyDeviceToDevice, h->stream));
    return 0;
}

int qs_settle_lanes(qs_handle* h, int on) {
    if (!h) QS_FAIL(-1, "null handle");
    QS_ON_DEVICE(h);
    if (h->la.K == 0) { if (on) QS_FAIL(-1, "this handle keeps no look-ahead reset states (cfg.reset_lookahead = 0, or QS_RAND_KEEP)"); return 0; }
    if (!on && h->lanes_on) {
        hipLaunchKernelGGL(k_lookahead_requeue, dim3(1), dim3(256), 0, h->stream, h->d_stats, h->la, h->d_stage_jobs, h->slice);
        QS_HIP(hipGetLastError());
    }
    if (on && !h->lanes_on) h->tick = 0;
    h->lanes_on = on ? 1 : 0;
    return 0;
}

static int launch_step(qs_handle* h, const float* actions, float* obs, float* rew, uint8_t* done, uint8_t* trunc);

int qs_step(qs_handle* h, const float* actions, float* obs, float* rew, uint8_t* done, uint8_t* trunc) {
    if (!h || !actions || !obs || !rew || !done || !trunc) QS_FAIL(-1, "null argument");
    return launch_step(h, actions, obs, rew, done, trunc);
}

int qs_step_fused(qs_handle* h, const float* actions, float* fused) {
    if (!h || !actions || !fused) QS_FAIL(-1, "null argument");
    return launch_step(h, actions, fused, nullptr, nullptr, nullptr);
}

static int launch_step(qs_handle* h, const float* actions, float* obs, float* rew, uint8_t* done, uint8_t* trunc) {
    QS_ON_DEVICE(h);
    SettleLanes lanes;
    memset(&lanes, 0, sizeof(lanes));
    lanes.n_env_waves = n_waves(h->cfg.n_envs); lanes.slice = 0;
    TraceTap tap; tap.rows = h->trace_rows; tap.env = h->trace_env;
    DemoTab demo; demo.rows = h->d_demo; demo.length = h->demo_len;
    if (E::demo_task(h->cfg.task) && !h->d_demo) QS_FAIL(-1, "the DEMO tasks need a demonstration: qs_set_demo first");
    TermTail tail = h->tail;
    memset(&h->tail, 0, sizeof(h->tail));
    PushTab push; push.rows = h->push_live ? h->d_push : nullptr;
    int grid = lanes.n_env_waves;
    bool lanes_fit = true;
    if (h->la.K > 0 && h->lanes_on) {
        const int rep = h->cfg.action_repeat, epoch = (h->cfg.settle_steps + rep - 1) / rep;
        const int slice = h->slice;
        lanes.staging = h->d_staging; lanes.stage_jobs = h->d_stage_jobs; lanes.slice = slice;
        const int free_simd = h->n_simd - lanes.n_env_waves;
        const int cohort_waves = slice / QS_ENVS_PER_WAVE;
        int base_waves = cohort_waves;
        if (h->step_variant != 2 && free_simd / QS_COHORTS >= 64 && base_waves > free_simd / QS_COHORTS) base_waves = free_simd / QS_COHORTS;
        lanes_fit = n_waves(h->cfg.n_envs) + QS_COHORTS * base_waves <= h->n_simd;
        for (int c = 0; c < QS_COHORTS; c++) {
            const long long t = h->tick - (long long)c * epoch / QS_COHORTS;
            lanes.wave0[c] = c * cohort_waves;
            if (t < 0) continue;
            const int phase = (int)(t % epoch);
            if (phase == 0) {
                hipLaunchKernelGGL(k_lookahead_publish, dim3(128), dim3(256), 0, h->stream, h->d_stats, h->d_staging, h->d_stage_jobs, h->la, c, slice);
                hipLaunchKernelGGL(k_lookahead_plan, dim3(1), dim3(1024), 0, h->stream, h->d_stats, h->la, h->cfg.n_envs, h->d_stage_jobs, c, slice, base_waves * QS_ENVS_PER_WAVE, 1,
                                   (int)((h->tick / (epoch / QS_COHORTS > 0 ? epoch / QS_COHORTS : 1)) * 4099 % h->cfg.n_envs));
            }
            lanes.spawn[c] = phase == 0; lanes.last[c] = phase == epoch - 1;
            lanes.settle_n[c] = phase == epoch - 1 ? h->cfg.settle_steps - rep * (epoch - 1) : rep;
        }
        lanes.wave0[QS_COHORTS] = QS_COHORTS * cohort_waves;
        grid += lanes.wave0[QS_COHORTS];
        h->tick++;
    }
    if (h->timing == 1) { hipEventRecord(h->ev0, h->stream); h->timing = 2; }
    if (h->timing == 1 || h->timing == 2) h->timed_launches++;
    const bool dense = h->step_variant == 2 || (h->step_variant == 0 && (lanes.n_env_waves > h->n_simd || !lanes_fit));
    const qs::Build build = handle_build(h);
    auto launch = [&](auto kernel) {
        hipLaunchKernelGGL(kernel, dim3(grid), dim3(QS_WAVE), build.step_lds_bytes(), h->stream, h->d_cfg, h->d_rec, actions, obs, rew, done, trunc,
                           h->d_obs, h->d_term_obs, h->la, h->d_stats, lanes, tap, demo, tail, push);
    };
    qs::with_build(build, [&](auto cone, auto soft, auto rack) {
        if constexpr (rack()) launch(dense ? k_step_dense_rack<cone()> : k_step_rack<cone()>);
        else launch(dense ? k_step_dense<cone(), soft()> : k_step<cone(), soft()>);
    });
    QS_HIP(hipGetLastError());
    return 0;
}

struct HostPath {
    size_t bytes, off_rew, off_done, off_trunc, off_tail;
    int cap;
    int zero_copy;
    uint8_t* d_block;
    uint8_t* h_block[2];
    uint8_t* hd_block[2];
    float* h_act; float* d_act; float* hd_act;
    int cur, parity, pending;
    int late_rc;
    int registered;
    hipEvent_t ev;
    qs_norm* norm; int norm_training, norm_obs, norm_rew; float* raw_obs; float* raw_rew;
};
static void host_path_release(HostPath* p) {
    if (!p) return;
    for (int k = 0; k < 2; k++) if (p->h_block[k]) { if (p->registered & (1 << k)) hipHostUnregister(p->h_block[k]); free(p->h_block[k]); }
    if (p->h_act) { if (p->registered & 4) hipHostUnregister(p->h_act); free(p->h_act); }
    if (p->d_block) hipFree(p->d_block);
    if (p->d_act) hipFree(p->d_act);
    if (p->ev) hipEventDestroy(p->ev);
    delete p;
}
static void host_path_free(qs_handle* h) { host_path_release(h->host); h->host = nullptr; }
static int host_path_build(qs_handle* h, HostPath* p);
static int host_path_init(qs_handle* h) {
    if (h->host) return 0;
    HostPath* p = new (std::nothrow) HostPath();
    if (!p) QS_FAIL(-4, "out of host memory");
    memset(p, 0, sizeof(*p));
    if (int rc = host_path_build(h, p)) { host_path_release(p); return rc; }
    h->host = p;
    return 0;
}
static int host_path_build(qs_handle* h, HostPath* p) {
    const size_t n = (size_t)h->cfg.n_envs, o = (size_t)h->cfg.obs_dim, d = (size_t)h->cfg.action_dim;
    p->cap = (int)(n < 256 ? n : 256);
    p->off_rew = n * o * 4; p->off_done = p->off_rew + n * 4; p->off_trunc = p->off_done + n;
    p->off_tail = (p->off_trunc + n + 15) / 16 * 16;
    p->bytes = p->off_tail + (size_t)p->cap * (o + 1) * 4;
    const char* mode = getenv("QS_HOST_PATH");
    p->zero_copy = !(mode && strcmp(mode, "copy") == 0);
    const unsigned flags = p->zero_copy ? hipHostRegisterMapped : hipHostRegisterDefault;
    const size_t page = 4096, hb = (p->bytes + page - 1) / page * page, ab = (n * d * 4 + page - 1) / page * page;
    for (int k = 0; k < 2; k++) {
        void* m = nullptr;
        if (posix_memalign(&m, page, hb) != 0) QS_FAIL(-4, "out of host memory");
        memset(m, 0, hb);
        p->h_block[k] = (uint8_t*)m;
        QS_HIP(hipHostRegister(m, hb, flags));
        p->registered |= 1 << k;
        if (p->zero_copy) QS_HIP(hipHostGetDevicePointer((void**)&p->hd_block[k], m, 0));
    }
    void* m = nullptr;
    if (posix_memalign(&m, page, ab) != 0) QS_FAIL(-4, "out of host memory");
    memset(m, 0, ab);
    p->h_act = (float*)m;
    QS_HIP(hipHostRegister(m, ab, flags));
    p->registered |= 4;
    if (p->zero_copy) QS_HIP(hipHostGetDevicePointer((void**)&p->hd_act, m, 0));
    else {
        QS_HIP(hipMalloc(&p->d_block, p->bytes));
        QS_HIP(hipMemset(p->d_block, 0, p->bytes));
        QS_HIP(hipMalloc(&p->d_act, n * d * 4));
    }
    QS_HIP(hipEventCreateWithFlags(&p->ev, hipEventDisableTiming));
    return 0;
}

static int host_step_after_launch(qs_handle* h, HostPath* p, uint8_t* blk, bool via_device) {
    if (p->norm) {
        if (int rc = qs_norm_set_stream(p->norm, (void*)h->stream)) return rc;
        qs_norm_io io;
        memset(&io, 0, sizeof(io));
        io.obs = (float*)blk; io.rew = (float*)(blk + p->off_rew); io.done = blk + p->off_done; io.trunc = blk + p->off_trunc;
        io.tail_rows = (float*)(blk + p->off_tail); io.tail_cap = p->cap; io.raw_obs = p->raw_obs; io.raw_rew = p->raw_rew;
        io.tail_count = (const uint64_t*)&h->d_stats[CTL_TERM_CNT + p->parity];
        if (p->zero_copy) {
            uint8_t* to = p->hd_block[p->cur];
            io.out_obs = (float*)to; io.out_rew = (float*)(to + p->off_rew); io.out_done = to + p->off_done; io.out_trunc = to + p->off_trunc;
            io.out_tail = (float*)(to + p->off_tail);
        }
        if (int rc = qs_norm_step_io(p->norm, &io, p->norm_training, p->norm_obs, p->norm_rew)) return rc;
    }
    if (via_device && !(p->norm && p->zero_copy)) QS_HIP(hipMemcpyAsync(p->h_block[p->cur], p->d_block, p->bytes, hipMemcpyDeviceToHost, h->stream));
    return 0;
}

int qs_host_step_begin(qs_handle* h, const float* actions_host) {
    if (!h || !actions_host) QS_FAIL(-1, "null argument");
    QS_ON_DEVICE(h);
    if (int rc = host_path_init(h)) return rc;
    HostPath* p = h->host;
    if (p->pending) QS_FAIL(-1, "qs_host_step_begin: the previous step has not been collected (qs_host_step_end)");
    const size_t n = (size_t)h->cfg.n_envs, d = (size_t)h->cfg.action_dim;
    memcpy(p->h_act, actions_host, n * d * 4);
    const int cur = p->cur ^ 1, parity = p->parity ^ 1;
    const bool via_device = !p->zero_copy || p->norm != nullptr;
    if (via_device && !p->d_block) {
        QS_HIP(hipMalloc(&p->d_block, p->bytes));
        QS_HIP(hipMemsetAsync(p->d_block, 0, p->bytes, h->stream));
    }
    uint8_t* blk = via_device ? p->d_block : p->hd_block[cur];
    const float* act = p->zero_copy ? p->hd_act : p->d_act;
    if (!p->zero_copy) QS_HIP(hipMemcpyAsync(p->d_act, p->h_act, n * d * 4, hipMemcpyHostToDevice, h->stream));
    h->tail.rows = (float*)(blk + p->off_tail); h->tail.cap = p->cap; h->tail.parity = parity;
    if (int rc = launch_step(h, act, (float*)blk, (float*)(blk + p->off_rew), blk + p->off_done, blk + p->off_trunc)) { memset(&h->tail, 0, sizeof(h->tail)); return rc; }
    p->cur = cur; p->parity = parity;
    const int late = host_step_after_launch(h, p, blk, via_device);
    hipEventRecord(p->ev, h->stream);
    p->pending = 1; p->late_rc = late;
    return late;
}

int qs_host_set_norm(qs_handle* h, qs_norm* norm, int training, int norm_obs, int norm_reward, float* raw_obs, float* raw_rew) {
    if (!h) QS_FAIL(-1, "null handle");
    QS_ON_DEVICE(h);
    if (!norm && !h->host) return 0;
    if (int rc = host_path_init(h)) return rc;
    HostPath* p = h->host;
    if (p->pending && norm) QS_FAIL(-1, "qs_host_set_norm between qs_host_step_begin and qs_host_step_end");
    if (norm) {
        int nn = 0, no = 0, nd = -1;
        if (int rc = qs_norm_dims(norm, &nn, &no, &nd)) return rc;
        if (nn != h->cfg.n_envs || no != h->cfg.obs_dim || nd != h->device)
            QS_FAIL(-1, "qs_host_set_norm: the normalisation handle is for %d environments x %d observations on device %d, the simulation handle for %d x %d on device %d",
                    nn, no, nd, h->cfg.n_envs, h->cfg.obs_dim, h->device);
    }
    p->norm = norm; p->norm_training = training; p->norm_obs = norm_obs; p->norm_rew = norm_reward; p->raw_obs = raw_obs; p->raw_rew = raw_rew;
    return 0;
}

int qs_host_step_end(qs_handle* h, qs_host_result* out) {
    if (!h || !out) QS_FAIL(-1, "null argument");
    HostPath* p = h->host;
    if (!p || !p->pending) QS_FAIL(-1, "qs_host_step_end without qs_host_step_begin");
    QS_ON_DEVICE(h);
    QS_HIP(hipEventSynchronize(p->ev));
    p->pending = 0;
    if (p->late_rc) {
        const int rc = p->late_rc;
        p->late_rc = 0;
        QS_FAIL(rc, "qs_host_step_end: the step ran, but what qs_host_step_begin enqueued behind it (normalisation / copy) had failed with %d: the host block does not hold its results", rc);
    }
// ... 1 lines not shown
    out->obs = (const float*)b; out->rew = (const float*)(b + p->off_rew); out->done = b + p->off_done; out->truncated = b + p->off_trunc;
    out->terminal_rows = (const float*)(b + p->off_tail); out->terminal_cap = p->cap;
    return 0;
}

__global__ void k_set_demo_counter(float* __restrict__ recs, int n, const uint8_t* __restrict__ mask, const int32_t* __restrict__ values, int length) {
    int e = blockIdx.x * blockDim.x + threadIdx.x;
    if (e >= n || (mask && !mask[e])) return;
    int v = values[e];
    v = v < 0 ? 0 : (v >= length ? length - 1 : v);
    float* r = recs + (size_t)e * QS_REC + R_DEMO;
    r[0] = (float)v; r[1] = (float)v;
}

int qs_set_demo(qs_handle* h, const float* rows, int length) {
    if (!h || !rows) QS_FAIL(-1, "null argument");
    if (!E::demo_task(h->cfg.task)) QS_FAIL(-1, "task %d is not a DEMO task", h->cfg.task);
    if (length <= 0 || length >= (1 << 24)) QS_FAIL(-1, "a demonstration has between 1 and 2^24 rows (got %d)", length);
    QS_ON_DEVICE(h);
    const size_t bytes = (size_t)length * (size_t)(h->cfg.action_dim + 38) * sizeof(float);
    float* copy = nullptr;
    QS_HIP(hipMalloc(&copy, bytes));
    hipError_t e = hipMemcpyAsync(copy, rows, bytes, hipMemcpyDeviceToDevice, h->stream);
    if (e == hipSuccess) e = hipStreamSynchronize(h->stream);
    if (e != hipSuccess) { hipFree(copy); QS_FAIL(-2, "copying the demonstration failed: %s", hipGetErrorString(e)); }
    if (h->d_demo) hipFree(h->d_demo);
    h->d_demo = copy; h->demo_len = length;
    return 0;
}

int qs_set_demo_counter(qs_handle* h, const uint8_t* mask, const int32_t* values) {
    if (!h || !values) QS_FAIL(-1, "null argument");
    if (!h->d_demo) QS_FAIL(-1, "no demonstration (qs_set_demo)");
    QS_ON_DEVICE(h);
    hipLaunchKernelGGL(k_set_demo_counter, dim3((h->cfg.n_envs + 255) / 256), dim3(256), 0, h->stream, h->d_rec, h->cfg.n_envs, mask, values, h->demo_len);
    QS_HIP(hipGetLastError());
    return 0;
}

__global__ void k_set_wrench(float* __restrict__ rows, int n, const uint8_t* __restrict__ mask, const float* __restrict__ wrench,
                             const int32_t* __restrict__ substeps, int frame, unsigned long long* __restrict__ refused) {
    const int e = blockIdx.x * blockDim.x + threadIdx.x;
    if (e >= n || (mask && !mask[e])) return;
    float w[6];
    bool ok = substeps[e] >= 0;
    for (int i = 0; i < 6; i++) { w[i] = wrench[(size_t)e * 6 + i]; ok = ok && (__float_as_uint(w[i]) & 0x7f800000u) != 0x7f800000u; }
    if (!ok) { atomicCAS(refused, 0ull, (unsigned long long)e + 1ull); return; }
    const int k = min(substeps[e], 1 << 24);
    float* r = rows + (size_t)e * QS_PUSH_F;
    for (int i = 0; i < 6; i++) r[i] = w[i];
    r[QS_PUSH_REM] = (float)k; r[QS_PUSH_FRAME] = (float)frame;
}

int qs_set_external_wrench(qs_handle* h, const uint8_t* mask, const float* wrench, const int32_t* substeps, int frame) {
    if (!h || !wrench || !substeps) QS_FAIL(-1, "null argument");
    if (frame != QS_FRAME_LINK && frame != QS_FRAME_WORLD) QS_FAIL(-1, "unknown frame %d (QS_FRAME_LINK = 1, QS_FRAME_WORLD = 2)", frame);
    QS_ON_DEVICE(h);
    hipLaunchKernelGGL(k_set_wrench, dim3((h->cfg.n_envs + 255) / 256), dim3(256), 0, h->stream, h->d_push, h->cfg.n_envs, mask, wrench, substeps, frame,
                       h->d_stats + CTL_PUSH_REFUSED);
    QS_HIP(hipGetLastError());
    h->push_live = 1;
    return 0;
}

int qs_set_rack(qs_handle* h, const uint8_t* mask, int hung) {
    if (!h) QS_FAIL(-1, "null handle");
    if (!h->rack.on) QS_FAIL(-1, "this handle was created without a rack (qs_create_ex with qs_rack::on = 1)");
    if (hung != 0 && hung != 1) QS_FAIL(-1, "hung must be 0 (release) or 1 (hang), got %d", hung);
    QS_ON_DEVICE(h);
    hipLaunchKernelGGL(k_set_rack, dim3((h->cfg.n_envs + 255) / 256), dim3(256), 0, h->stream, h->d_rec, h->cfg.n_envs, mask, hung);
    QS_HIP(hipGetLastError());
    return 0;
}

static int push_refusal(qs_handle* h) {
    unsigned long long v = 0, r = 0, f = 0;
    QS_HIP(hipMemcpy(&f, &h->d_stats[CTL_FORK_REFUSED], sizeof(f), hipMemcpyDeviceToHost));
    if (f != 0) {
        QS_HIP(hipMemset(&h->d_stats[CTL_FORK_REFUSED], 0, sizeof(f)));
        QS_FAIL(-1, "qs_fork refused the source of environment %llu (and maybe others): outside [-1, %d); those environments were left alone", f - 1, h->cfg.n_envs);
    }
    QS_HIP(hipMemcpy(&v, &h->d_stats[CTL_PUSH_REFUSED], sizeof(v), hipMemcpyDeviceToHost));
    QS_HIP(hipMemcpy(&r, &h->d_stats[CTL_RENDER_REFUSED], sizeof(r), hipMemcpyDeviceToHost));
    if (v == 0 && r != 0) {
        QS_HIP(hipMemset(&h->d_stats[CTL_RENDER_REFUSED], 0, sizeof(r)));
        QS_FAIL(-1, "qs_render got an environment id out of range (%d environments) at position %llu of env_ids (and maybe others): drawn as sky "
                    "with segmentation id -2", h->cfg.n_envs, r - 1);
    }
    if (v == 0) return 0;
    QS_HIP(hipMemset(&h->d_stats[CTL_PUSH_REFUSED], 0, sizeof(v)));
    QS_FAIL(-1, "qs_set_external_wrench refused the row of environment %llu (and maybe others): a negative duration or a non-finite force / "
                "torque; those environments kept their earlier push", v - 1);
}

}
int qs_render_view(qs_handle* h, QsRenderView* v) {
    v->rec = h->d_rec; v->n_envs = h->cfg.n_envs; v->payload_soft = h->cfg.payload_soft; v->device = h->device;
    v->stream = h->stream; v->refused = h->d_stats + CTL_RENDER_REFUSED;
    return 0;
}
static_assert(QS_PUSH_F == 8, "qs_snapshot.h's PUSH_F");
int qs_snapshot_view(qs_handle* h, QsSnapshotView* v) {
    v->cfg = &h->cfg; v->rack = &h->rack;
    v->rec = h->d_rec; v->push = h->d_push; v->obs = h->d_obs; v->term = h->d_term_obs;
    v->la_cur = h->la.cur; v->la_handed = h->la.handed; v->la_K = h->la.K;
    v->device = h->device; v->stream = h->stream;
    v->fork_refused = h->d_stats + CTL_FORK_REFUSED; v->fork_rows = &h->d_fork; v->push_live = &h->push_live;
    return 0;
}
extern "C" {

int qs_set_trace(qs_handle* h, int env, float* rows) {
    if (!h) QS_FAIL(-1, "null handle");
    if (env >= h->cfg.n_envs) QS_FAIL(-1, "trace environment %d out of range (%d environments)", env, h->cfg.n_envs);
    h->trace_env = env; h->trace_rows = env >= 0 ? rows : nullptr;
    return 0;
}

int qs_counters_async(qs_handle* h, uint64_t* dev_out) {
    if (!h || !dev_out) QS_FAIL(-1, "null argument");
    QS_ON_DEVICE(h);
    static_assert(CTL_SETTLE_SUBSTEPS == QS_COUNTER_SETTLE_SUBSTEPS && CTL_RESETS == QS_COUNTER_RESETS && CTL_SERVED == QS_COUNTER_LOOKAHEAD_SERVED &&
                  CTL_SETTLED == QS_COUNTER_LOOKAHEAD_SETTLED && CTL_STALLS == QS_COUNTER_RESET_STALLS, "the handle's counters sit at their public indices");
    unsigned long long* out = reinterpret_cast<unsigned long long*>(dev_out);
    QS_HIP(hipMemcpyAsync(out, h->d_stats, 4 * sizeof(unsigned long long), hipMemcpyDeviceToDevice, h->stream));
    QS_HIP(hipMemcpyAsync(out + QS_COUNTER_RESET_STALLS, h->d_stats + CTL_STALLS, sizeof(unsigned long long), hipMemcpyDeviceToDevice, h->stream));
    QS_HIP(hipMemcpyAsync(out + QS_COUNTER_LIMIT_PATH_SUBSTEPS, h->d_stats + CTL_DEV + QS_DEVCTR_RARE_PATH, sizeof(unsigned long long), hipMemcpyDeviceToDevice, h->stream));
    QS_HIP(hipMemcpyAsync(out + QS_COUNTER_SELF_NARROW_SUBSTEPS, h->d_stats + CTL_DEV + QS_DEVCTR_SELF_NARROW, sizeof(unsigned long long), hipMemcpyDeviceToDevice, h->stream));
    return 0;
}

int qs_counter(qs_handle* h, int which, uint64_t* value) {
    if (!h || !value) QS_FAIL(-1, "null argument");
    QS_ON_DEVICE(h);
    QS_HIP(hipStreamSynchronize(h->stream));
    if (int rc = push_refusal(h)) return rc;
    unsigned long long v = 0;
    switch (which) {
    case QS_COUNTER_SETTLE_SUBSTEPS: QS_HIP(hipMemcpy(&v, &h->d_stats[CTL_SETTLE_SUBSTEPS], sizeof(v), hipMemcpyDeviceToHost)); break;
    case QS_COUNTER_RESETS: QS_HIP(hipMemcpy(&v, &h->d_stats[CTL_RESETS], sizeof(v), hipMemcpyDeviceToHost)); break;
    case QS_COUNTER_LOOKAHEAD_SERVED: QS_HIP(hipMemcpy(&v, &h->d_stats[CTL_SERVED], sizeof(v), hipMemcpyDeviceToHost)); break;
    case QS_COUNTER_LOOKAHEAD_SETTLED: QS_HIP(hipMemcpy(&v, &h->d_stats[CTL_SETTLED], sizeof(v), hipMemcpyDeviceToHost)); break;
    case QS_COUNTER_RESET_STALLS: QS_HIP(hipMemcpy(&v, &h->d_stats[CTL_STALLS], sizeof(v), hipMemcpyDeviceToHost)); break;
    case QS_COUNTER_LOOKAHEAD_BACKLOG:
        if (h->la.K > 0) {
            hipLaunchKernelGGL(k_lookahead_plan, dim3(1), dim3(1024), 0, h->stream, h->d_stats, h->la, h->cfg.n_envs, h->d_stage_jobs, 0, h->slice, 0, 0, 0);
            QS_HIP(hipGetLastError());
            QS_HIP(hipStreamSynchronize(h->stream));
            QS_HIP(hipMemcpy(&v, &h->d_stats[CTL_BACKLOG], sizeof(v), hipMemcpyDeviceToHost));
        }
        break;
    case QS_COUNTER_LIMIT_PATH_SUBSTEPS: QS_HIP(hipMemcpy(&v, &h->d_stats[CTL_DEV + QS_DEVCTR_RARE_PATH], sizeof(v), hipMemcpyDeviceToHost)); break;
    case QS_COUNTER_SELF_NARROW_SUBSTEPS: QS_HIP(hipMemcpy(&v, &h->d_stats[CTL_DEV + QS_DEVCTR_SELF_NARROW], sizeof(v), hipMemcpyDeviceToHost)); break;
    default: QS_FAIL(-1, "unknown counter %d", which);
    }
    *value = v;
    return 0;
}

int qs_last_step_kernel_ms(qs_handle* h, float* ms) {
    if (!h || !ms) QS_FAIL(-1, "null argument");
    if ((h->timing != 2 && h->timing != 3) || h->timed_launches <= 0) QS_FAIL(-1, "no step has been launched since qs_enable_timing(h, 1)");
    QS_ON_DEVICE(h);
    if (h->timing == 2) QS_HIP(hipEventRecord(h->ev1, h->stream));
    QS_HIP(hipEventSynchronize(h->ev1));
    float total = 0.0f;
    QS_HIP(hipEventElapsedTime(&total, h->ev0, h->ev1));
    *ms = total / (float)h->timed_launches;
    h->timing = 1; h->timed_launches = 0;
    return 0;
}

__global__ __launch_bounds__(QS_WAVE) void k_block_place(const qs_config* __restrict__ cfgp, float* __restrict__ recs) {
    const qs_config& cfg = *cfgp;
    const int env = blockIdx.x * QS_ENVS_PER_WAVE + (threadIdx.x >> 2);
    if (env >= cfg.n_envs) return;
    E::place_block(cfg, recs + (size_t)env * QS_REC);
}
static int place_blocks(qs_handle* h) {
    if (!h->cfg.payload_soft) return 0;
    hipLaunchKernelGGL(k_block_place, dim3(n_waves(h->cfg.n_envs)), dim3(QS_WAVE), 0, h->stream, h->d_cfg, h->d_rec);
    QS_HIP(hipGetLastError());
    return 0;
}
static int gather(qs_handle* h, int off, int dim, float* out, int as_int) {
    int total = h->cfg.n_envs * dim;
    hipLaunchKernelGGL(k_gather, dim3((total + 255) / 256), dim3(256), 0, h->stream, h->d_rec, h->cfg.n_envs, off, dim, out, as_int);
    QS_HIP(hipGetLastError());
    return 0;
}
static int scatter(qs_handle* h, int off, int dim, const float* in, int zero_warm) {
    int total = h->cfg.n_envs * dim;
    hipLaunchKernelGGL(k_scatter, dim3((total + 255) / 256), dim3(256), 0, h->stream, h->d_rec, h->cfg.n_envs, off, dim, in, zero_warm);
    QS_HIP(hipGetLastError());
    return 0;
}

__global__ __launch_bounds__(QS_WAVE) void k_reward_end(const qs_config* __restrict__ cfgp, const float* __restrict__ recs, float* __restrict__ out) {
    const qs_config& cfg = *cfgp;
    const int env = blockIdx.x * QS_ENVS_PER_WAVE + (threadIdx.x >> 2);
    const float* rec = recs + (size_t)(env < cfg.n_envs ? env : 0) * QS_REC;
    typename E::S::State s; E::Task t;
    E::load_state(rec, s); E::load_task(rec, t);
    t.pos[0] = s.pos.x; t.pos[1] = s.pos.y; t.pos[2] = s.pos.z;
    float term = E::task_terminated(cfg, t, s, rec[R_N_INVALID], false);
    float r = E::task_reward_end(cfg, t, term, (float)((double)qs::f2i(rec[R_SIM_STEP]) * cfg.dt));
    if (env < cfg.n_envs && (threadIdx.x & 3) == 0) out[env] = r;
}
__global__ void k_wrapper_info(const float* __restrict__ recs, int n, float* __restrict__ out) {
    int e = blockIdx.x * blockDim.x + threadIdx.x;
    if (e >= n) return;
    const float* w = recs + (size_t)e * QS_REC + R_WRAP;
    out[4 * e] = w[W_PHASE]; out[4 * e + 1] = w[W_SCRIPTED]; out[4 * e + 2] = w[W_TIMER]; out[4 * e + 3] = w[W_END];
}
static int gather_wrapper(qs_handle* h, float* out) {
    hipLaunchKernelGGL(k_wrapper_info, dim3((h->cfg.n_envs + 255) / 256), dim3(256), 0, h->stream, h->d_rec, h->cfg.n_envs, out);
    QS_HIP(hipGetLastError());
    return 0;
}

int qs_get_state(qs_handle* h, float* st) { if (!h || !st) QS_FAIL(-1, "null argument"); QS_ON_DEVICE(h); return gather(h, R_POS, QS_STATE_DIM, st, 0); }
int qs_set_state(qs_handle* h, const float* st) {
    if (!h || !st) QS_FAIL(-1, "null argument");
    QS_ON_DEVICE(h);
    if (int rc = scatter(h, R_POS, QS_STATE_DIM, st, 1)) return rc;
    return place_blocks(h);
}

int qs_info_dim(const qs_handle* h, int which) {
    switch (which) {
    case QS_INFO_FOOT_FORCE: case QS_INFO_FOOT_CONTACT: case QS_INFO_COUNTERS: return 4;
    case QS_INFO_TORQUE: case QS_INFO_SPRING_TORQUE: case QS_INFO_LAST_ACTION: return 12;
    case QS_INFO_TASK: return QS_TASK_DIM;
    case QS_INFO_N_INVALID: return 1;
    case QS_INFO_PARAMS: return QS_PARAM_DIM;
    case QS_INFO_TERMINAL_OBS: return h ? h->cfg.obs_dim : -1;
    case QS_INFO_WRAPPER: return 4;
    case QS_INFO_FILTERED_ACTION: return 12;
    case QS_INFO_REWARD_END: return 1;
    case QS_INFO_PAYLOAD_BLOCK: return QS_BLOCK_DIM;
    case QS_INFO_EXTERNAL_WRENCH: return QS_PUSH_F;
    case QS_INFO_RACK: return 8;
    default: return -1;
    }
}

int qs_get_info(qs_handle* h, int which, float* out) {
    if (!h || !out) QS_FAIL(-1, "null argument");
    QS_ON_DEVICE(h);
    if (!h->cfg.info_fields && (which == QS_INFO_FOOT_FORCE || which == QS_INFO_FOOT_CONTACT || which == QS_INFO_TORQUE || which == QS_INFO_SPRING_TORQUE))
        QS_FAIL(-1, "info id %d lives in the records' info block, which this handle does not write (cfg.info_fields = 0)", which);
    switch (which) {
    case QS_INFO_FOOT_FORCE: return gather(h, R_FOOT_FORCE, 4, out, 0);
    case QS_INFO_FOOT_CONTACT: return gather(h, R_FOOT_CONTACT, 4, out, 0);
    case QS_INFO_TORQUE: return gather(h, R_TAU_PD, 12, out, 0);
    case QS_INFO_SPRING_TORQUE: return gather(h, R_TAU_SPRING, 12, out, 0);
    case QS_INFO_N_INVALID: return gather(h, R_N_INVALID, 1, out, 0);
    case QS_INFO_PARAMS: return gather(h, R_PARAMS, QS_PARAM_DIM, out, 0);
    case QS_INFO_COUNTERS: return gather(h, R_SIM_STEP, 4, out, 1);
    case QS_INFO_LAST_ACTION: return gather(h, R_LAST_ACTION, 12, out, 0);
    case QS_INFO_WRAPPER: return gather_wrapper(h, out);
    case QS_INFO_FILTERED_ACTION: return gather(h, R_YHIST, 12, out, 0);
    case QS_INFO_PAYLOAD_BLOCK:
        if (!h->cfg.payload_soft) QS_FAIL(-1, "the payload block is a body of its own only under cfg.payload_soft");
        return gather(h, R_BLOCK, QS_BLOCK_DIM, out, 0);
    case QS_INFO_REWARD_END:
        hipLaunchKernelGGL(k_reward_end, dim3(n_waves(h->cfg.n_envs)), dim3(QS_WAVE), 0, h->stream, h->d_cfg, h->d_rec, out);
        QS_HIP(hipGetLastError());
        return 0;
    case QS_INFO_TASK:
        hipLaunchKernelGGL(k_task_info, dim3((h->cfg.n_envs + 255) / 256), dim3(256), 0, h->stream, h->d_rec, h->cfg.n_envs, out, (int)E::demo_task(h->cfg.task), h->cfg.info_fields);
        QS_HIP(hipGetLastError());
        return 0;
    case QS_INFO_EXTERNAL_WRENCH:
        QS_HIP(hipMemcpyAsync(out, h->d_push, (size_t)h->cfg.n_envs * QS_PUSH_F * sizeof(float), hipMemcpyDeviceToDevice, h->stream));
        return 0;
    case QS_INFO_RACK:
        if (!h->rack.on) QS_FAIL(-1, "this handle was created without a rack (qs_create_ex with qs_rack::on = 1)");
        hipLaunchKernelGGL(k_rack_info, dim3((h->cfg.n_envs + 255) / 256), dim3(256), 0, h->stream, h->d_rec, h->cfg.n_envs, (float)(1.0 / h->cfg.dt),
                           h->rack.anchor_pos[0], h->rack.anchor_pos[1], h->rack.anchor_pos[2], out);
        QS_HIP(hipGetLastError());
        return 0;
    case QS_INFO_TERMINAL_OBS:
        QS_HIP(hipMemcpyAsync(out, h->d_term_obs, (size_t)h->cfg.n_envs * h->cfg.obs_dim * sizeof(float), hipMemcpyDeviceToDevice, h->stream));
        return 0;
    default: QS_FAIL(-1, "unknown info id %d", which);
    }
}

int qs_set_params(qs_handle* h, int which, const float* v) {
    if (!h || !v) QS_FAIL(-1, "null argument");
    QS_ON_DEVICE(h);
    switch (which) {
    case QS_PARAM_MU: return scatter(h, R_PARAMS + P_MU, 1, v, 0);
    case QS_PARAM_SPRING_K: return scatter(h, R_PARAMS + P_K, 3, v, 0);
    case QS_PARAM_SPRING_B: return scatter(h, R_PARAMS + P_B, 3, v, 0);
    case QS_PARAM_KP: return scatter(h, R_PARAMS + P_KP, 3, v, 0);
    case QS_PARAM_KD: return scatter(h, R_PARAMS + P_KD, 3, v, 0);
    case QS_PARAM_ALL: if (int rc = scatter(h, R_PARAMS, QS_PARAM_DIM, v, 0)) return rc; return place_blocks(h);
    default: QS_FAIL(-1, "unknown param id %d", which);
    }
}

int qs_stats(qs_handle* h, uint64_t* settle_substeps, uint64_t* resets) {
    if (!h) QS_FAIL(-1, "null handle");
    QS_ON_DEVICE(h);
// ... 21 lines not shown
```

quadruped-springs_amd/csrc/qs_lane.h:

```cpp
#pragma once
#include <math.h>
#include <stdint.h>
#include "../../include/qs_amd.h"

#if defined(__HIPCC__)
#define QS_FN __host__ __device__ __forceinline__
#define QS_DEV __device__ __forceinline__
#else
#define QS_FN inline
#endif

QS_FN float qabs(float x) { return fabsf(x); }
QS_FN float qfloor(float x) { return floorf(x); }
QS_FN float qmin(float a, float b) { return fminf(a, b); }
QS_FN float qmax(float a, float b) { return fmaxf(a, b); }
QS_FN float qsin(float x) { return sinf(x); }
QS_FN float qcos(float x) { return cosf(x); }
QS_FN float qexp(float x) { return expf(x); }
QS_FN float qlog(float x) { return logf(x); }
#if defined(__HIP_DEVICE_COMPILE__)
QS_FN float qsqrt(float x) { return __builtin_amdgcn_sqrtf(x); }
QS_FN float qrcp(float x) { return __builtin_amdgcn_rcpf(x); }
QS_FN float qrsqrt(float x) { return __builtin_amdgcn_rsqf(x); }
#else
QS_FN float qsqrt(float x) { return sqrtf(x); }
QS_FN float qrcp(float x) { return 1.0f / x; }
QS_FN float qrsqrt(float x) { return 1.0f / sqrtf(x); }
#endif
QS_FN float qatan2(float y, float x) {
    const float ax = fabsf(x), ay = fabsf(y);
    const float mx = fmaxf(ax, ay), mn = fminf(ax, ay);
    float a = mx > 0.0f ? mn * qrcp(mx) : 0.0f;
    const bool mid = a > 0.4142135623730950f;
    const float t = mid ? (a - 1.0f) * qrcp(a + 1.0f) : a;
    const float z = t * t;
    float r = ((((8.05374449538e-2f * z - 1.38776856032e-1f) * z + 1.99777106478e-1f) * z - 3.33329491539e-1f) * z) * t + t;
    r = mid ? r + 0.7853981633974483f : r;
    r = ay > ax ? 1.5707963267948966f - r : r;
    r = x < 0.0f ? 3.141592653589793f - r : r;
    return y < 0.0f ? -r : r;
}
QS_FN float qasin(float x) { return qatan2(x, qsqrt(fmaxf(1.0f - x * x, 0.0f))); }
QS_FN void qsincos(float x, float& s, float& c) {
    float k = rintf(x * 0.636619772367581343f);
    float r = fmaf(k, -1.57079601287841796875f, x);
    r = fmaf(k, -3.139164786504813217e-7f, r);
    float r2 = r * r;
    float sp = fmaf(fmaf(fmaf(-1.9515295891e-4f, r2, 8.3321608736e-3f), r2, -1.6666654611e-1f), r2 * r, r);
    float cp = fmaf(fmaf(fmaf(fmaf(2.443315711809948e-5f, r2, -1.388731625493765e-3f), r2, 4.166664568298827e-2f), r2, -0.5f), r2, 1.0f);
    int q = (int)k;
    float ss = (q & 1) ? cp : sp, cc = (q & 1) ? sp : cp;
    s = (q & 2) ? -ss : ss;
    c = ((q + 1) & 2) ? -cc : cc;
}
#if defined(__HIP_DEVICE_COMPILE__)
QS_FN float qmed3(float x, float lo, float hi) { return __builtin_amdgcn_fmed3f(x, lo, hi); }
#else
QS_FN float qmed3(float x, float lo, float hi) { return fminf(fmaxf(x, lo), hi); }
#endif
QS_FN float qsel(bool m, float a, float b) { return m ? a : b; }
QS_FN bool qlt(float a, float b) { return a < b; }
QS_FN bool qgt(float a, float b) { return a > b; }
QS_FN bool qle(float a, float b) { return a <= b; }
QS_FN bool qge(float a, float b) { return a >= b; }
QS_FN bool qand(bool a, bool b) { return a && b; }
QS_FN bool qor(bool a, bool b) { return a || b; }
QS_FN bool qnot(bool a) { return !a; }
QS_FN float qflag(bool m) { return m ? 1.0f : 0.0f; }

struct QsDevCfg { qs_config cfg; unsigned long long* counters; float rack_pos[3]; float rack_quat[4]; };
#if defined(__HIPCC__)
enum { QS_DEVCTR_RARE_PATH = 0, QS_DEVCTR_SELF_NARROW = 1 };
struct LaneDev {
    using V = float;
    using M = bool;
    template <int CTRL> static QS_DEV float dpp(float x) {
        return __builtin_bit_cast(float, __builtin_amdgcn_mov_dpp(__builtin_bit_cast(int, x), CTRL, 0xF, 0xF, true));
    }
    static QS_DEV float quad_sum(float x) {
        x += dpp<0xB1>(x);
        x += dpp<0x4E>(x);
        return x;
    }
    template <int K> static QS_DEV float bcast(float x) { return dpp<K * 0x55>(x); }
    template <int K> static QS_DEV float xorl(float x) { return dpp<K == 1 ? 0xB1 : (K == 2 ? 0x4E : 0x1B)>(x); }
    template <int K> static QS_DEV float fma_bcast(float d, float a, float acc) {
        float b = __builtin_bit_cast(float, __builtin_amdgcn_update_dpp(__builtin_bit_cast(int, acc), __builtin_bit_cast(int, d), K * 0x55, 0xF, 0xF, true));
        return fmaf(b, a, acc);
    }
    typedef float F2 __attribute__((ext_vector_type(2)));
    static QS_DEV void fma2(float a0, float a1, float b, float& c0, float& c1) {
        F2 a = {a0, a1}, c = {c0, c1}, bb = {b, b};
        c = __builtin_elementwise_fma(a, bb, c);
        c0 = c.x; c1 = c.y;
    }
    static QS_DEV float absmax_mul2(float m, float x0, float d0, float x1, float d1) {
        F2 x = {x0, x1}, d = {d0, d1};
        F2 p = x * d;
        return __builtin_fmaxf(m, __builtin_fmaxf(__builtin_fabsf(p.x), __builtin_fabsf(p.y)));
    }
    typedef float Acc4 __attribute__((ext_vector_type(4)));
    static QS_DEV Acc4 acc4_zero() { Acc4 z = {0.0f, 0.0f, 0.0f, 0.0f}; return z; }
    static QS_DEV void outer_fma(float a, float b, Acc4& acc) { acc = __builtin_amdgcn_mfma_f32_4x4x1f32(a, b, acc, 0, 0, 0); }
    static QS_DEV void outer_fma_valu(float a, float b, Acc4& acc) {
        acc[0] = fmaf(bcast<0>(a), b, acc[0]); acc[1] = fmaf(bcast<1>(a), b, acc[1]);
        acc[2] = fmaf(bcast<2>(a), b, acc[2]); acc[3] = fmaf(bcast<3>(a), b, acc[3]);
    }
    template <int K> static QS_DEV float acc4_get(const Acc4& acc) { return acc[K]; }
    static QS_DEV float bcast_dyn(float x, int k) { return __shfl(x, (int)((threadIdx.x & 60u) | (unsigned)k), 64); }
    static QS_DEV int leg() { return (int)(threadIdx.x & 3u); }
    static QS_DEV float fx() { return (threadIdx.x & 2u) ? -1.0f : 1.0f; }
    static QS_DEV float sy() { return (threadIdx.x & 1u) ? 1.0f : -1.0f; }
    static QS_DEV bool is_leg(int k) { return (int)(threadIdx.x & 3u) == k; }
    static QS_DEV bool any(bool m) { return __any(m); }
    static QS_DEV float ld_leg(const float* rec, int base, int stride) { return rec[base + stride * (int)(threadIdx.x & 3u)]; }
    static QS_DEV void st_leg(float* rec, int base, int stride, float v) { rec[base + stride * (int)(threadIdx.x & 3u)] = v; }
    static QS_DEV float ld(const float* rec, int i) { return rec[i]; }
    static QS_DEV void st(float* rec, int i, float v) { if ((threadIdx.x & 3u) == 0) rec[i] = v; }
    static QS_DEV float first(float x) { return x; }
    static QS_DEV void opaque(float& x) { asm volatile("" : "+v"(x)); }
    static QS_DEV float* wave_scratch(float* row) { return row - (size_t)(threadIdx.x >> 2) * QS_MAX_OBS; }
    static QS_DEV void count_rare_path(const qs_config& cfg) { if (threadIdx.x == 0) atomicAdd(&reinterpret_cast<const QsDevCfg&>(cfg).counters[QS_DEVCTR_RARE_PATH], 1ull); }
    static QS_DEV void count_self_narrow(const qs_config& cfg) { if (threadIdx.x == 0) atomicAdd(&reinterpret_cast<const QsDevCfg&>(cfg).counters[QS_DEVCTR_SELF_NARROW], 1ull); }
    static QS_DEV void sync() {
        __builtin_amdgcn_fence(__ATOMIC_RELEASE, "wavefront");
        __builtin_amdgcn_wave_barrier();
        __builtin_amdgcn_fence(__ATOMIC_ACQUIRE, "wavefront");
    }
};
#endif

#if !defined(__HIP_DEVICE_COMPILE__)
struct V4 {
    float v[4];
    V4() : v{0, 0, 0, 0} {}
    V4(float a) : v{a, a, a, a} {}
    V4(float a, float b, float c, float d) : v{a, b, c, d} {}
};
struct M4 { bool v[4]; };
#define QS_V4_BIN(op)                                                                                          \
    inline V4 operator op(V4 a, V4 b) { V4 r; for (int i = 0; i < 4; i++) r.v[i] = a.v[i] op b.v[i]; return r; } \
    inline V4 operator op(V4 a, float b) { V4 r; for (int i = 0; i < 4; i++) r.v[i] = a.v[i] op b; return r; }   \
    inline V4 operator op(float a, V4 b) { V4 r; for (int i = 0; i < 4; i++) r.v[i] = a op b.v[i]; return r; }
QS_V4_BIN(+) QS_V4_BIN(-) QS_V4_BIN(*) QS_V4_BIN(/)
inline V4 operator-(V4 a) { V4 r; for (int i = 0; i < 4; i++) r.v[i] = -a.v[i]; return r; }
inline V4& operator+=(V4& a, V4 b) { a = a + b; return a; }
inline V4& operator-=(V4& a, V4 b) { a = a - b; return a; }
inline V4& operator*=(V4& a, V4 b) { a = a * b; return a; }
#define QS_V4_FN1(name, f) inline V4 name(V4 a) { V4 r; for (int i = 0; i < 4; i++) r.v[i] = f(a.v[i]); return r; }
QS_V4_FN1(qsqrt, sqrtf) QS_V4_FN1(qabs, fabsf) QS_V4_FN1(qfloor, floorf) QS_V4_FN1(qsin, sinf) QS_V4_FN1(qcos, cosf) QS_V4_FN1(qasin, asinf)
QS_V4_FN1(qexp, expf) QS_V4_FN1(qlog, logf) QS_V4_FN1(qrcp, qrcp) QS_V4_FN1(qrsqrt, qrsqrt)
inline void qsincos(V4 x, V4& s, V4& c) { for (int i = 0; i < 4; i++) qsincos(x.v[i], s.v[i], c.v[i]); }
inline V4 qmin(V4 a, V4 b) { V4 r; for (int i = 0; i < 4; i++) r.v[i] = fminf(a.v[i], b.v[i]); return r; }
inline V4 qmax(V4 a, V4 b) { V4 r; for (int i = 0; i < 4; i++) r.v[i] = fmaxf(a.v[i], b.v[i]); return r; }
inline V4 qatan2(V4 a, V4 b) { V4 r; for (int i = 0; i < 4; i++) r.v[i] = atan2f(a.v[i], b.v[i]); return r; }
inline V4 qmed3(V4 x, V4 lo, V4 hi) { return qmin(qmax(x, lo), hi); }
inline V4 qsel(M4 m, V4 a, V4 b) { V4 r; for (int i = 0; i < 4; i++) r.v[i] = m.v[i] ? a.v[i] : b.v[i]; return r; }
#define QS_V4_CMP(name, op) inline M4 name(V4 a, V4 b) { M4 r; for (int i = 0; i < 4; i++) r.v[i] = a.v[i] op b.v[i]; return r; }
QS_V4_CMP(qlt, <) QS_V4_CMP(qgt, >) QS_V4_CMP(qle, <=) QS_V4_CMP(qge, >=)
inline M4 qand(M4 a, M4 b) { M4 r; for (int i = 0; i < 4; i++) r.v[i] = a.v[i] && b.v[i]; return r; }
inline M4 qor(M4 a, M4 b) { M4 r; for (int i = 0; i < 4; i++) r.v[i] = a.v[i] || b.v[i]; return r; }
inline M4 qnot(M4 a) { M4 r; for (int i = 0; i < 4; i++) r.v[i] = !a.v[i]; return r; }
inline V4 qflag(M4 m) { V4 r; for (int i = 0; i < 4; i++) r.v[i] = m.v[i] ? 1.0f : 0.0f; return r; }

struct LaneEmu {
    using V = V4;
    using M = M4;
    static V4 quad_sum(V4 x) {
        V4 t, r;
        for (int i = 0; i < 4; i++) t.v[i] = x.v[i] + x.v[i ^ 1];
        for (int i = 0; i < 4; i++) r.v[i] = t.v[i] + t.v[i ^ 2];
        return r;
    }
    template <int K> static V4 bcast(V4 x) { return V4(x.v[K]); }
    template <int K> static V4 xorl(V4 x) { V4 r; for (int i = 0; i < 4; i++) r.v[i] = x.v[i ^ K]; return r; }
    static V4 bcast_dyn(V4 x, int k) { return V4(x.v[k]); }
    template <int K> static V4 fma_bcast(V4 d, V4 a, V4 acc) { V4 r; for (int i = 0; i < 4; i++) r.v[i] = acc.v[i] + d.v[K] * a.v[i]; return r; }
    static V4 fx() { return V4(1, 1, -1, -1); }
    static V4 sy() { return V4(-1, 1, -1, 1); }
    static M4 is_leg(int k) { M4 m; for (int i = 0; i < 4; i++) m.v[i] = (i == k); return m; }
    static V4 absmax_mul2(V4 m, V4 x0, V4 d0, V4 x1, V4 d1) {
        V4 r;
        for (int l = 0; l < 4; l++) r.v[l] = fmaxf(m.v[l], fmaxf(fabsf(x0.v[l] * d0.v[l]), fabsf(x1.v[l] * d1.v[l])));
        return r;
    }
    static void fma2(V4 a0, V4 a1, V4 b, V4& c0, V4& c1) { for (int l = 0; l < 4; l++) { c0.v[l] = fmaf(a0.v[l], b.v[l], c0.v[l]); c1.v[l] = fmaf(a1.v[l], b.v[l], c1.v[l]); } }
    static float* wave_scratch(float* row) { return row; }
    static void count_rare_path(const qs_config&) {}
    static void count_self_narrow(const qs_config&) {}
    struct Acc4 { V4 k[4]; };
    static Acc4 acc4_zero() { Acc4 z; for (int i = 0; i < 4; i++) z.k[i] = V4(0.0f); return z; }
    static void outer_fma(V4 a, V4 b, Acc4& acc) { for (int K = 0; K < 4; K++) for (int l = 0; l < 4; l++) acc.k[K].v[l] = fmaf(a.v[K], b.v[l], acc.k[K].v[l]); }
    static void outer_fma_valu(V4 a, V4 b, Acc4& acc) { outer_fma(a, b, acc); }
    template <int K> static V4 acc4_get(const Acc4& acc) { return acc.k[K]; }
    static bool any(M4 m) { return m.v[0] || m.v[1] || m.v[2] || m.v[3]; }
    static V4 ld_leg(const float* rec, int base, int stride) { V4 r; for (int i = 0; i < 4; i++) r.v[i] = rec[base + stride * i]; return r; }
    static void st_leg(float* rec, int base, int stride, V4 v) { for (int i = 0; i < 4; i++) rec[base + stride * i] = v.v[i]; }
    static V4 ld(const float* rec, int i) { return V4(rec[i]); }
    static void st(float* rec, int i, V4 v) { rec[i] = v.v[0]; }
    static float first(V4 x) { return x.v[0]; }
    static void opaque(V4&) {}
    static void sync() {}
};
#endif
```

quadruped-springs_amd/qs_amd/lib.py:

```python
import ctypes as C
import os

from .config import QsConfig

_HERE = os.path.dirname(os.path.abspath(__file__))
LIB_PATH = os.environ.get("QS_LIB_PATH") or os.path.join(_HERE, "libqs_hip.so")

ABI_VERSION = 8
ABI_LIBRARY = 9

EXPORTS = (
    "qs_create", "qs_destroy", "qs_set_stream", "qs_reset", "qs_reset_to", "qs_get_obs", "qs_step", "qs_step_fused", "qs_get_state", "qs_set_state",
    "qs_info_dim", "qs_get_info", "qs_set_params", "qs_stats", "qs_enable_timing", "qs_last_step_kernel_ms",
    "qs_settle_lanes", "qs_host_step_begin", "qs_host_step_end", "qs_set_trace", "qs_counter", "qs_counters_async", "qs_set_demo", "qs_set_demo_counter", "qs_set_external_wrench", "qs_create_ex", "qs_set_rack", "qs_render", "qs_render_states", "qs_last_error", "qs_version", "qs_abi_version",
    "qs_norm_create", "qs_norm_destroy", "qs_norm_dims", "qs_norm_set_stream", "qs_norm_set_stats", "qs_norm_get_stats", "qs_norm_reset", "qs_norm_step",
    "qs_norm_step_io", "qs_host_set_norm",
    "qs_policy_create", "qs_policy_destroy", "qs_policy_set_stream", "qs_policy_param_count", "qs_policy_set_params", "qs_policy_act",
    "qs_ac_create", "qs_ac_destroy", "qs_ac_set_stream", "qs_ac_set_params", "qs_ac_collect", "qs_ac_values", "qs_ac_bootstrap", "qs_gae",
    "qs_snapshot_info", "qs_snapshot", "qs_restore", "qs_fork", "qs_norm_get_returns", "qs_norm_set_returns",
    "qs_ppo_create", "qs_ppo_destroy", "qs_ppo_set_stream", "qs_ppo_bind", "qs_ppo_grad", "qs_ppo_adam", "qs_ppo_refusals",
)



class HostResult(C.Structure):
    _fields_ = [("obs", C.c_void_p), ("rew", C.c_void_p), ("done", C.c_void_p), ("truncated", C.c_void_p), ("terminal_rows", C.c_void_p),
                ("terminal_cap", C.c_int32)]


class NormIO(C.Structure):
    _fields_ = [("obs", C.c_void_p), ("rew", C.c_void_p), ("done", C.c_void_p), ("trunc", C.c_void_p), ("term_obs", C.c_void_p), ("tail_rows", C.c_void_p),
                ("tail_cap", C.c_int32),
                ("out_obs", C.c_void_p), ("out_rew", C.c_void_p), ("out_done", C.c_void_p), ("out_trunc", C.c_void_p), ("out_tail", C.c_void_p),
                ("raw_obs", C.c_void_p), ("raw_rew", C.c_void_p), ("tail_count", C.c_void_p)]


class QsCamera(C.Structure):
    _fields_ = [("target", C.c_float * 3), ("distance", C.c_float), ("yaw_deg", C.c_float), ("pitch_deg", C.c_float), ("fov_deg", C.c_float),
                ("near_clip", C.c_float), ("far_clip", C.c_float), ("follow_base", C.c_int32), ("draw_payload", C.c_int32)]


class QsPolicyDesc(C.Structure):
    _fields_ = [("n_envs", C.c_int32), ("n_policies", C.c_int32), ("obs_dim", C.c_int32), ("action_dim", C.c_int32), ("n_hidden", C.c_int32),
                ("hidden", C.c_int32 * 4), ("activation", C.c_int32), ("squash_output", C.c_int32), ("has_bias", C.c_int32),
                ("clip_lo", C.c_float), ("clip_hi", C.c_float)]


class QsRack(C.Structure):
    _fields_ = [("on", C.c_int32), ("anchor_pos", C.c_float * 3), ("anchor_quat", C.c_float * 4)]


class QsPpoHyper(C.Structure):
    _fields_ = [("clip_range", C.c_float), ("ent_coef", C.c_float), ("vf_coef", C.c_float), ("max_grad_norm", C.c_float),
                ("normalize_advantage", C.c_int32), ("reserved", C.c_int32),
                ("lr", C.c_double), ("beta_one", C.c_double), ("beta_two", C.c_double), ("adam_eps", C.c_double)]


PPO_STATS = ("policy_loss", "value_loss", "entropy_loss", "approx_kl", "clip_fraction", "grad_norm", "refused", "loss")

_lib = None


def load():
    global _lib
    if _lib is not None:
        return _lib
    if not os.path.exists(LIB_PATH):
        raise RuntimeError(f"{LIB_PATH} is missing: run `python quadruped-springs_amd/build.py` (needs hipcc). "
                           "The simulation step has no CPU fallback.")
    import torch
    lib = C.CDLL(LIB_PATH)
    vp, i32 = C.c_void_p, C.c_int
    lib.qs_create.argtypes = [C.POINTER(QsConfig), i32, C.POINTER(vp)]
    lib.qs_destroy.argtypes = [vp]
    lib.qs_destroy.restype = None
    lib.qs_set_stream.argtypes = [vp, vp]
    lib.qs_reset.argtypes = [vp, vp]
    lib.qs_reset_to.argtypes = [vp, vp, vp]
    lib.qs_get_obs.argtypes = [vp, vp]
    lib.qs_step.argtypes = [vp, vp, vp, vp, vp, vp]
    lib.qs_step_fused.argtypes = [vp, vp, vp]
    lib.qs_get_state.argtypes = [vp, vp]
    lib.qs_set_state.argtypes = [vp, vp]
    lib.qs_info_dim.argtypes = [vp, i32]
    lib.qs_get_info.argtypes = [vp, i32, vp]
    lib.qs_set_params.argtypes = [vp, i32, vp]
    lib.qs_stats.argtypes = [vp, C.POINTER(C.c_uint64), C.POINTER(C.c_uint64)]
    lib.qs_enable_timing.argtypes = [vp, i32]
    lib.qs_last_step_kernel_ms.argtypes = [vp, C.POINTER(C.c_float)]
    lib.qs_settle_lanes.argtypes = [vp, C.c_int]
    lib.qs_host_step_begin.argtypes = [vp, vp]
    lib.qs_host_step_end.argtypes = [vp, C.POINTER(HostResult)]
    lib.qs_set_trace.argtypes = [vp, C.c_int, vp]
    lib.qs_set_demo.argtypes = [vp, vp, C.c_int]
    lib.qs_set_demo_counter.argtypes = [vp, vp, vp]
    if hasattr(lib, "qs_set_external_wrench"):
        lib.qs_set_external_wrench.argtypes = [vp, vp, vp, vp, i32]
    if hasattr(lib, "qs_create_ex"):
        lib.qs_create_ex.argtypes = [C.POINTER(QsConfig), C.POINTER(QsRack), i32, C.POINTER(vp)]
        lib.qs_set_rack.argtypes = [vp, vp, i32]
    if hasattr(lib, "qs_render"):
        lib.qs_render.argtypes = [vp, vp, i32, C.POINTER(QsCamera), i32, i32, vp, vp, vp]
        lib.qs_render_states.argtypes = [vp, vp, i32, C.POINTER(QsCamera), i32, i32, vp, vp, vp, vp]
    lib.qs_counter.argtypes = [vp, C.c_int, C.POINTER(C.c_uint64)]
    lib.qs_counters_async.argtypes = [vp, vp]
    f32, f64, pd = C.c_float, C.c_double, C.POINTER(C.c_double)
    lib.qs_norm_create.argtypes = [i32, i32, f64, f64, f64, f64, i32, C.POINTER(vp)]
    lib.qs_norm_destroy.argtypes = [vp]
    lib.qs_norm_dims.argtypes = [vp, C.POINTER(C.c_int), C.POINTER(C.c_int), C.POINTER(C.c_int)]
    lib.qs_norm_destroy.restype = None
    lib.qs_norm_set_stream.argtypes = [vp, vp]
    lib.qs_norm_set_stats.argtypes = [vp, vp, vp, f64, f64, f64, f64]
    lib.qs_norm_get_stats.argtypes = [vp, vp, vp, pd, pd, pd, pd]
    lib.qs_norm_reset.argtypes = [vp, vp, i32, i32]
    lib.qs_norm_step.argtypes = [vp, vp, vp, vp, vp, i32, i32, i32, vp, vp]
    lib.qs_norm_step_io.argtypes = [vp, C.POINTER(NormIO), i32, i32, i32]
    lib.qs_host_set_norm.argtypes = [vp, vp, i32, i32, i32, vp, vp]
    if hasattr(lib, "qs_policy_create"):
        lib.qs_policy_create.argtypes = [C.POINTER(QsPolicyDesc), i32, C.POINTER(vp)]
        lib.qs_policy_destroy.argtypes = [vp]
        lib.qs_policy_destroy.restype = None
        lib.qs_policy_set_stream.argtypes = [vp, vp]
        lib.qs_policy_param_count.argtypes = [vp]
        lib.qs_policy_set_params.argtypes = [vp, vp]
        lib.qs_policy_act.argtypes = [vp, vp, vp, vp, vp, vp, vp]
    if hasattr(lib, "qs_ac_create"):
        lib.qs_ac_create.argtypes = [C.POINTER(QsPolicyDesc), C.POINTER(QsPolicyDesc), i32, C.POINTER(vp)]
        lib.qs_ac_destroy.argtypes = [vp]
        lib.qs_ac_destroy.restype = None
        lib.qs_ac_set_stream.argtypes = [vp, vp]
        lib.qs_ac_set_params.argtypes = [vp, vp, vp]
        lib.qs_ac_collect.argtypes = [vp, vp, vp, vp, vp, vp, vp, vp, vp]
        lib.qs_ac_values.argtypes = [vp, vp, vp, vp]
        lib.qs_ac_bootstrap.argtypes = [vp, vp, vp, f32, vp]
        lib.qs_gae.argtypes = [vp, vp, vp, vp, vp, i32, i32, f32, f32, vp, vp, vp]
    if hasattr(lib, "qs_snapshot_info"):
        from .snapshot import SnapshotInfo
        lib.qs_snapshot_info.argtypes = [vp, C.POINTER(SnapshotInfo)]
        lib.qs_snapshot.argtypes = [vp, vp, vp]
        lib.qs_restore.argtypes = [vp, vp, vp]
        lib.qs_fork.argtypes = [vp, vp]
        lib.qs_norm_get_returns.argtypes = [vp, vp]
        lib.qs_norm_set_returns.argtypes = [vp, vp]
    if hasattr(lib, "qs_ppo_create"):
        lib.qs_ppo_create.argtypes = [C.POINTER(QsPolicyDesc), C.POINTER(QsPolicyDesc), i32, i32, C.POINTER(vp)]
        lib.qs_ppo_destroy.argtypes = [vp]
        lib.qs_ppo_destroy.restype = None
        lib.qs_ppo_set_stream.argtypes = [vp, vp]
        lib.qs_ppo_bind.argtypes = [vp, vp, vp, vp, vp, vp]
        lib.qs_ppo_grad.argtypes = [vp, vp, vp, vp, vp, vp, C.c_longlong, vp, i32, C.POINTER(QsPpoHyper), vp, vp]
        lib.qs_ppo_adam.argtypes = [vp, vp, C.POINTER(QsPpoHyper), i32, vp]
        lib.qs_ppo_refusals.argtypes = [vp, C.POINTER(C.c_uint64)]
    lib.qs_last_error.restype = C.c_char_p
    lib.qs_version.restype = C.c_char_p
    if os.environ.get("QS_ALLOW_ABI_MISMATCH") != "1" and (not hasattr(lib, "qs_abi_version") or lib.qs_abi_version() != ABI_LIBRARY):
        have = lib.qs_abi_version() if hasattr(lib, "qs_abi_version") else "none (a library of round 4 or earlier)"
        raise RuntimeError(f"{LIB_PATH} speaks ABI {have}, this binding was written against ABI {ABI_LIBRARY} of include/qs_amd.h: rebuild it "
                           "(python quadruped-springs_amd/build.py --force)")
    _lib = lib
    return lib


def source_sha(lib=None):
    import re
    m = re.search(r"source ([0-9a-f]{64})", (lib or load()).qs_version().decode())
    return m.group(1) if m else None


def check(rc):
    if rc != 0:
        raise RuntimeError("qs_amd: " + load().qs_last_error().decode())
```

quadruped-springs_amd/qs_amd/vec_env.py:

```python
import ctypes as C

import numpy as np

from . import lib as _lib
from .config import DEMO_FILES, OBSERVATION_EPS, build_config
from .render import DEFAULT_SIZE, as_camera, check_request, rgb_view, tile_images
from .spaces import Box, SB3VecEnv

INFO = dict(foot_force=0, foot_contact=1, torque=2, spring_torque=3, task=4, n_invalid=5, params=6, counters=7,
            last_action=8, terminal_obs=9, wrapper=10, filtered_action=11, reward_end=12, payload_block=13, external_wrench=14, rack=15)
PHASE = ("policy", "take_off", "landing", "rest")
PARAM = dict(mu=0, spring_k=1, spring_b=2, kp=3, kd=4, all=5)
FRAME = dict(link=1, world=2)


class QuadrupedVecEnv(SB3VecEnv):
    def __init__(self, num_envs=1, device=0, auto_reset=True, reset_lookahead=None, copy_outputs=True, **env_kwargs):
        cfg, meta = build_config(n_envs=num_envs, auto_reset=auto_reset, **env_kwargs)
        cfg.reset_lookahead = int((16 if auto_reset else 0) if reset_lookahead is None else reset_lookahead)
        self._setup(cfg, meta, device, copy_outputs)

    @classmethod
    def from_config(cls, cfg, meta, device=0, copy_outputs=True, load_demo=True):
        self = cls.__new__(cls)
        self._setup(cfg, meta, device, copy_outputs, load_demo)
        return self

    def _setup(self, cfg, meta, device, copy_outputs, load_demo=True):
        import torch

        if not torch.cuda.is_available():
            raise RuntimeError("QuadrupedVecEnv needs a HIP device (torch.cuda.is_available() is False); there is no CPU path")
        self.torch = torch
        self.lib = _lib.load()
        self.cfg, self.meta = cfg, meta
        self.num_envs = int(cfg.n_envs)
        self.device = torch.device("cuda", device)
        lay = self.meta["layout"]
        self.observation_space = Box(lay["low"] - OBSERVATION_EPS, lay["high"] + OBSERVATION_EPS, dtype=np.float32)
        d = self.cfg.action_dim
        self.action_space = Box(-np.ones(d), np.ones(d), dtype=np.float32)
        self.action_dim, self.obs_dim = d, self.cfg.obs_dim
        self._init_vec_env_base()
        self.h = C.c_void_p()
        self._closed = False
        self._create(device)
        n, o = self.num_envs, self.obs_dim
        with torch.cuda.device(self.device):
            self._obs = torch.zeros((n, o), dtype=torch.float32, device=self.device)
            self._rew = torch.zeros(n, dtype=torch.float32, device=self.device)
            self._done = torch.zeros(n, dtype=torch.uint8, device=self.device)
            self._trunc = torch.zeros(n, dtype=torch.uint8, device=self.device)
            self._act = torch.zeros((n, d), dtype=torch.float32, device=self.device)
        self._views, self._infos, self._dirty = {}, [{} for _ in range(self.num_envs)], []
        self._terminal_hook = None
        self.copy_outputs = bool(copy_outputs)
        self._trace = None
        self._push_keep = None
        self.render_mode = None
        self.render_indices = None
        self.render_size = DEFAULT_SIZE
        self.camera_mode = "CLASSIC"
        self._render_all = None
        self._render_keep = None
        self.demo_list, self.demo_length = None, 0
        if load_demo and self.meta["task_env"] in DEMO_FILES:
            if self.meta["demo"] is None:
                self.close()
                raise ValueError(f"task {self.meta['task_env']} imitates a demonstration: pass demo=<array [L, action_dim + 38] or path of the "
                                 f".npy> (the reference loads demonstrations/{DEMO_FILES[self.meta['task_env']]}, task_base.py:173)")
            self.set_demo(self.meta["demo"])

    def _create(self, device):
        rk = self.meta.get("rack")
        self.on_rack = bool(rk and rk["on"])
        if self.on_rack:
            r = _lib.QsRack()
            r.on = 1
            for i in range(3):
                r.anchor_pos[i] = float(rk["pos"][i])
            for i in range(4):
                r.anchor_quat[i] = float(rk["quat"][i])
            _lib.check(self.lib.qs_create_ex(C.byref(self.cfg), C.byref(r), device, C.byref(self.h)))
        else:
            _lib.check(self.lib.qs_create(C.byref(self.cfg), device, C.byref(self.h)))

    def set_rack(self, hung, indices=None):
        if not self.on_rack:
            raise RuntimeError("set_rack needs a handle created with on_rack=True")
        mask = None
        if indices is not None:
            m = np.zeros(self.num_envs, np.uint8)
            m[np.asarray(self._indices(indices), np.int64)] = 1
            mask = self.torch.from_numpy(m).pin_memory().to(self.device, non_blocking=True)
            self._rack_keep = mask
        self._stream()
        _lib.check(self.lib.qs_set_rack(self.h, None if mask is None else self._ptr(mask), 1 if hung else 0))

    def _init_vec_env_base(self):
        if SB3VecEnv is not object:
            SB3VecEnv.__init__(self, self.num_envs, self.observation_space, self.action_space)

    def _stream(self):
        s = self.torch.cuda.current_stream(self.device).cuda_stream
        _lib.check(self.lib.qs_set_stream(self.h, C.c_void_p(s)))

    def _ptr(self, t):
        return C.c_void_p(t.data_ptr())

    def close(self):
        if not getattr(self, "_closed", True) and self.h:
            h, self.h = self.h, C.c_void_p()
            self.lib.qs_destroy(h)
            self._closed = True

    def __del__(self):
        try:
            self.close()
        except Exception:
            pass

    def reset_tensor(self, mask=None, states=None):
        self._stream()
        m = None
        if mask is not None:
            m = self.torch.as_tensor(mask, device=self.device).to(self.torch.uint8).contiguous()
        if states is not None:
            st = self.torch.as_tensor(states, dtype=self.torch.float32, device=self.device).reshape(self.num_envs, 37).contiguous()
            _lib.check(self.lib.qs_reset_to(self.h, None if m is None else self._ptr(m), self._ptr(st)))
        else:
            _lib.check(self.lib.qs_reset(self.h, None if m is None else self._ptr(m)))
        _lib.check(self.lib.qs_get_obs(self.h, self._ptr(self._obs)))
        return self._obs

    def step_tensor(self, actions):
        a = actions
        if a.dtype != self.torch.float32 or not a.is_contiguous() or a.device != self.device:
            a = a.to(device=self.device, dtype=self.torch.float32).contiguous()
        if a.shape != (self.num_envs, self.action_dim):
            raise ValueError(f"actions must have shape {(self.num_envs, self.action_dim)}, got {tuple(a.shape)}")
        self._stream()
        _lib.check(self.lib.qs_step(self.h, self._ptr(a), self._ptr(self._obs), self._ptr(self._rew), self._ptr(self._done), self._ptr(self._trunc)))
        return self._obs, self._rew, self._done, self._trunc

    def step_fused(self, actions, out):
        t = self.torch
        for name, x, shape in (("actions", actions, (self.num_envs, self.action_dim)), ("out", out, (self.num_envs, self.obs_dim + 2))):
            if tuple(x.shape) != shape or x.dtype != t.float32 or x.device != self.device or not x.is_contiguous():
                raise ValueError(f"{name} must be a contiguous float32 tensor of shape {shape} on {self.device}")
        self._stream()
        _lib.check(self.lib.qs_step_fused(self.h, self._ptr(actions), self._ptr(out)))
        return out

    def get_state(self):
        out = self.torch.empty((self.num_envs, 37), dtype=self.torch.float32, device=self.device)
        self._stream()
        _lib.check(self.lib.qs_get_state(self.h, self._ptr(out)))
        return out

    def set_state(self, state):
        s = self.torch.as_tensor(state, dtype=self.torch.float32, device=self.device).contiguous().reshape(self.num_envs, 37)
        self._stream()
        _lib.check(self.lib.qs_set_state(self.h, self._ptr(s)))

    def get_info(self, which):
        k = INFO[which] if isinstance(which, str) else int(which)
        dim = self.lib.qs_info_dim(self.h, k)
        out = self.torch.empty((self.num_envs, dim), dtype=self.torch.float32, device=self.device)
        self._stream()
        _lib.check(self.lib.qs_get_info(self.h, k, self._ptr(out)))
        return out

    def set_params(self, which, values):
# ... 46 lines not shown
            k = k.expand(n)
        else:
            a = k.detach().cpu().numpy() if isinstance(k, t.Tensor) else np.asarray(k)
            if a.dtype.kind not in "iu" or np.any(a < 0):
                raise ValueError(f"substeps must be a non-negative integer (or [N] of them), got {k!r}")
            if a.shape not in ((), (n,)):
                raise ValueError(f"substeps must be a scalar or have shape {(n,)}, got {tuple(a.shape)}")
            if np.any(a > 2 ** 31 - 1):
                raise ValueError("substeps must fit an int32")
            k = t.full((n,), int(a), dtype=t.int32, device=self.device) if a.shape == () else to_device(a.astype(np.int32))
        k = k.contiguous()
        m = None
        if indices is not None:
            if isinstance(indices, t.Tensor) and indices.device == self.device:
                m = t.zeros(n, dtype=t.uint8, device=self.device).index_fill_(0, indices.to(t.int64), 1)
            else:
                mh = np.zeros(n, np.uint8)
                mh[np.asarray(self._indices(indices.tolist() if isinstance(indices, (np.ndarray, t.Tensor)) else indices), np.int64)] = 1
                m = to_device(mh)
        _lib.check(self.lib.qs_set_external_wrench(self.h, None if m is None else self._ptr(m), self._ptr(w), self._ptr(k), FRAME[frame]))
        self._push_keep = (w, k, m, keep)

    def snapshot_info(self):
        from .snapshot import SnapshotInfo
        info = SnapshotInfo()
        _lib.check(self.lib.qs_snapshot_info(self.h, C.byref(info)))
        return info.as_dict()

    def _mask_of(self, indices):
        if indices is None:
            return None
        t = self.torch
        if isinstance(indices, t.Tensor) and indices.device == self.device:
            if indices.dtype == t.bool or indices.dtype == t.uint8:
                if tuple(indices.shape) != (self.num_envs,):
                    raise ValueError(f"a mask must have shape {(self.num_envs,)}, got {tuple(indices.shape)}")
                return indices.to(t.uint8).contiguous()
            return t.zeros(self.num_envs, dtype=t.uint8, device=self.device).index_fill_(0, indices.to(t.int64), 1)
        idx = np.asarray(self._indices(indices.tolist() if isinstance(indices, (np.ndarray, t.Tensor)) else indices), np.int64)
        if idx.size and (idx.min() < 0 or idx.max() >= self.num_envs):
            raise ValueError(f"environment ids must lie in [0, {self.num_envs}), got {idx.min()} .. {idx.max()}")
        m = np.zeros(self.num_envs, np.uint8)
        m[idx] = 1
        return t.from_numpy(m).pin_memory().to(self.device, non_blocking=True)

    def snapshot(self, indices=None, out=None):
        from .snapshot import EnvSnapshot, check_fits
        t = self.torch
        info = self.snapshot_info()
        if out is None:
            rows = t.zeros((info["n_envs"], info["row_floats"]), dtype=t.float32, device=self.device)
            snap = EnvSnapshot(rows, info)
        else:
            check_fits(out.info, info, strict=True)
            rows = out.rows
            if rows.device != self.device or rows.dtype != t.float32 or not rows.is_contiguous() or tuple(rows.shape) != (info["n_envs"], info["row_floats"]):
                raise ValueError(f"out.rows must be a contiguous float32 tensor of shape {(info['n_envs'], info['row_floats'])} on {self.device}")
            snap = out
        m = self._mask_of(indices)
        self._stream()
        _lib.check(self.lib.qs_snapshot(self.h, None if m is None else self._ptr(m), self._ptr(rows)))
        self._snap_keep = m
        return snap

    def restore(self, snap, indices=None, strict=True):
        from .snapshot import check_fits
        t = self.torch
        check_fits(snap.info, self.snapshot_info(), strict=strict)
        rows = snap.rows
        if tuple(rows.shape) != (snap.info["n_envs"], snap.info["row_floats"]) or rows.dtype != t.float32:
            raise ValueError(f"snapshot rows must be float32 of shape {(snap.info['n_envs'], snap.info['row_floats'])}, got {rows.dtype} {tuple(rows.shape)}")
        if rows.device != self.device or not rows.is_contiguous():
            rows = rows.contiguous().to(self.device)
        m = self._mask_of(indices)
        self._stream()
        _lib.check(self.lib.qs_restore(self.h, None if m is None else self._ptr(m), self._ptr(rows)))
        _lib.check(self.lib.qs_get_obs(self.h, self._ptr(self._obs)))
        self._snap_keep = (m, rows)
        if not self._dirty:
            pass
        elif indices is None:
            self._forget_infos(None)
        elif isinstance(indices, t.Tensor) and indices.dtype in (t.bool, t.uint8):
            self._forget_infos(t.nonzero(indices).flatten().tolist())
        else:
            self._forget_infos(self._indices(indices.tolist() if isinstance(indices, (np.ndarray, t.Tensor)) else indices))
        return self._obs

    def _forget_infos(self, idx):
        idx = range(self.num_envs) if idx is None else idx
        for i in idx:
            if self._infos[i]:
                if self.copy_outputs:
                    self._infos[i] = {}
                else:
                    self._infos[i].clear()
        gone = set(idx)
        self._dirty = [i for i in self._dirty if i not in gone]

    def fork(self, src=None, dst=None, src_of=None):
        t = self.torch
        n = self.num_envs
        if src_of is not None:
            if src is not None or dst is not None:
                raise ValueError("give either src (and dst) or src_of")
            if not (isinstance(src_of, t.Tensor) and src_of.device == self.device):
                a = np.asarray(src_of)
                if a.dtype.kind not in "iu" or a.shape != (n,):
                    raise ValueError(f"src_of must be {n} integers, got {a.dtype} {a.shape}")
                if a.min() < -1 or a.max() >= n:
                    raise ValueError(f"sources must lie in [-1, {n}), got {a.min()} .. {a.max()}")
                so = t.from_numpy(a.astype(np.int32)).pin_memory().to(self.device, non_blocking=True)
            else:
                if src_of.dtype.is_floating_point or src_of.dtype == t.bool or tuple(src_of.shape) != (n,):
                    raise ValueError(f"src_of must be an integer tensor of shape {(n,)}, got {src_of.dtype} {tuple(src_of.shape)}")
                so = src_of.to(t.int32).contiguous()
        else:
            if src is None:
                raise ValueError("fork needs src or src_of")
            s = np.atleast_1d(np.asarray(src.tolist() if isinstance(src, t.Tensor) else src))
            if s.dtype.kind not in "iu" or s.ndim != 1 or s.size == 0:
                raise ValueError(f"src must be an index or a list of indices, got {src!r}")
            if dst is None:
                if s.size != 1:
                    raise ValueError("dst=None needs exactly one source (it then goes to every other environment)")
                d = np.array([i for i in range(n) if i != int(s[0])], np.int64)
            else:
                d = np.atleast_1d(np.asarray(dst.tolist() if isinstance(dst, t.Tensor) else dst))
                if d.size and (d.dtype.kind not in "iu" or d.ndim != 1):
                    raise ValueError(f"dst must be a list of indices, got {dst!r}")
                d = d.astype(np.int64)
            if s.size != 1 and s.size != d.size:
                raise ValueError(f"{s.size} sources for {d.size} destinations: give one source, or one per destination")
            for name, a in (("src", s), ("dst", d)):
                if a.size and (a.min() < 0 or a.max() >= n):
                    raise ValueError(f"{name} must lie in [0, {n}), got {a.min()} .. {a.max()}")
            if np.unique(d).size != d.size:
                raise ValueError("dst names an environment twice")
            a = np.full(n, -1, np.int32)
            a[d] = s.astype(np.int32) if s.size > 1 else np.int32(s[0])
            so = t.from_numpy(a).pin_memory().to(self.device, non_blocking=True)
        self._stream()
        _lib.check(self.lib.qs_fork(self.h, self._ptr(so)))
        _lib.check(self.lib.qs_get_obs(self.h, self._ptr(self._obs)))
        self._fork_keep = so
        return so

    def stats(self):
        a, b = C.c_uint64(), C.c_uint64()
        _lib.check(self.lib.qs_stats(self.h, C.byref(a), C.byref(b)))
        return dict(settle_substeps=a.value, resets=b.value)

    COUNTERS = dict(settle_substeps=0, resets=1, lookahead_served=2, lookahead_settled=3, limit_path_substeps=4, self_narrow_substeps=5,
                    reset_stalls=6, lookahead_backlog=7)

    def counter(self, which):
        v = C.c_uint64(0)
        _lib.check(self.lib.qs_counter(self.h, self.COUNTERS[which] if isinstance(which, str) else int(which), C.byref(v)))
        return int(v.value)

    def counters_snapshot(self):
        out = self.torch.zeros(8, dtype=self.torch.int64, device=self.device)
        self._stream()
        _lib.check(self.lib.qs_counters_async(self.h, self._ptr(out)))
        return out

    def enable_timing(self, on=True):
        self._stream()
        _lib.check(self.lib.qs_enable_timing(self.h, int(on)))

    def last_step_kernel_ms(self):
        ms = C.c_float()
        _lib.check(self.lib.qs_last_step_kernel_ms(self.h, C.byref(ms)))
        return ms.value

    TRACE_FIELDS = dict(time=(0, 1), base_position=(1, 4), base_quaternion=(4, 8), base_linear_velocity=(8, 11), base_angular_velocity=(11, 14),
                        joint_angles=(14, 26), joint_velocities=(26, 38), torques=(38, 50), spring_tau=(50, 62), feet_normal_forces=(62, 66),
                        feet_in_contact=(66, 70))

    def set_trace(self, env=0):
        if env is None:
            self._trace = None
            _lib.check(self.lib.qs_set_trace(self.h, -1, None))
            return
        self._trace = self.torch.zeros((self.cfg.action_repeat, 70), dtype=self.torch.float32, device=self.device)
        _lib.check(self.lib.qs_set_trace(self.h, int(env), self._ptr(self._trace)))

    def get_trace(self, as_dict=True):
        rows = self._trace.cpu().numpy().astype(np.float64)
        if not as_dict:
            return rows
        out = {k: rows[:, a:b] for k, (a, b) in self.TRACE_FIELDS.items()}
        out["time"] = out["time"][:, 0]
        return out

    def set_demo(self, rows):
        rows = np.ascontiguousarray(rows, dtype=np.float32)
        if rows.ndim != 2 or rows.shape[1] != self.action_dim + 38:
            raise ValueError(f"demonstration rows have {self.action_dim + 38} entries, got shape {rows.shape}")
        t = self.torch.from_numpy(rows).to(self.device)
        self._stream()
        _lib.check(self.lib.qs_set_demo(self.h, self._ptr(t), int(rows.shape[0])))
        self.demo_list, self.demo_length = rows, int(rows.shape[0])

    def set_demo_counter(self, values, mask=None):
        t = self.torch
        v = t.as_tensor(values, device=self.device).to(t.int32).expand(self.num_envs).contiguous()
        m = None if mask is None else t.as_tensor(mask, device=self.device).to(t.uint8).contiguous()
        self._stream()
        _lib.check(self.lib.qs_set_demo_counter(self.h, None if m is None else self._ptr(m), self._ptr(v)))

    def demo_counter(self):
        return self.get_info("task")[:, 44].to(self.torch.int64)

    @staticmethod
    def demo_states(rows, action_dim):
        r = np.atleast_2d(np.asarray(rows, dtype=np.float32))
        d = action_dim
        return np.concatenate([r[:, d + 24:d + 37], r[:, d:d + 24]], axis=1)

    def demo_rows(self, done=None):
        t = self.torch
        st = self.get_state()
        if getattr(self, "_landing_started", None) is None:
            self._landing_started = t.zeros(self.num_envs, dtype=t.bool, device=self.device)
        switched = self.get_info("task")[:, 0] > 0.5
        self._landing_started |= switched & (st[:, 9] <= 0.0)
        act = (self.get_info("filtered_action") if self.cfg.enable_filter else self.get_info("last_action"))[:, : self.action_dim]
        rows = t.cat([act, st[:, 13:37], st[:, 0:13], self._landing_started.to(t.float32)[:, None]], dim=1)
        d = self._done.bool() if done is None else t.as_tensor(np.asarray(done) if not t.is_tensor(done) else done, device=self.device).bool()
        self._landing_started &= ~d
        return rows

    @staticmethod
    def read_demo(demo, action_dim=6, num_joints=12):
        cuts = np.cumsum([action_dim, num_joints, num_joints, 3, 4, 3, 3, 1])
        return [demo[a:b] for a, b in zip(np.concatenate(([0], cuts[:-1])), cuts)]

    def settle_lanes(self, on=True):
        self._stream()
        _lib.check(self.lib.qs_settle_lanes(self.h, int(bool(on))))

    def reset(self):
        return self.reset_tensor().cpu().numpy().copy()

    def step_async(self, actions):
        a = np.ascontiguousarray(actions, dtype=np.float32)
        if a.size != self.num_envs * self.action_dim:
            raise ValueError(f"actions must have shape {(self.num_envs, self.action_dim)}, got {a.shape}")
        self._stream()
        rc = self.lib.qs_host_step_begin(self.h, a.ctypes.data_as(C.c_void_p))
        if rc != 0:
            msg = self.lib.qs_last_error().decode()
            self.lib.qs_host_step_end(self.h, C.byref(_lib.HostResult()))
            raise RuntimeError("qs_amd: " + msg)

    def _host_views(self, res):
        key = res.obs
        views = self._views.get(key)
        if views is None:
            n, o = self.num_envs, self.obs_dim
            f32, u8 = C.POINTER(C.c_float), C.POINTER(C.c_uint8)
            views = (np.ctypeslib.as_array(C.cast(res.obs, f32), shape=(n, o)), np.ctypeslib.as_array(C.cast(res.rew, f32), shape=(n,)),
                     np.ctypeslib.as_array(C.cast(res.done, u8), shape=(n,)).view(np.bool_),
                     np.ctypeslib.as_array(C.cast(res.truncated, u8), shape=(n,)).view(np.bool_),
                     np.ctypeslib.as_array(C.cast(res.terminal_rows, f32), shape=(res.terminal_cap, o + 1)))
            self._views[key] = views
        return views

    def _entry(self, old, truncated, terminal_observation):
        if self.copy_outputs:
            return {"TimeLimit.truncated": truncated, "terminal_observation": terminal_observation}
        old["TimeLimit.truncated"] = truncated; old["terminal_observation"] = terminal_observation
        return old

    def step_wait(self):
        res = _lib.HostResult()
        _lib.check(self.lib.qs_host_step_end(self.h, C.byref(res)))
        obs, rew, done, trunc, term = self._host_views(res)
        if self.copy_outputs:
            obs, rew, done = obs.copy(), rew.copy(), done.copy()
        infos = self._infos
        if self.copy_outputs:
            for i in self._dirty:
                infos[i] = {}
        else:
            for i in self._dirty:
                infos[i].clear()
        dirty = self._dirty = []
        idx = np.flatnonzero(done)
        if idx.size:
            if not self.cfg.auto_reset:
                for i in idx.tolist():
                    infos[i] = self._entry(infos[i], bool(trunc[i]), obs[i].copy())
            else:
                rows = term[: idx.size] if idx.size <= term.shape[0] else None
                if rows is None:
                    full = self.get_info("terminal_obs").cpu().numpy()
                    if self._terminal_hook is not None:
                        full = self._terminal_hook(full)
                    for i in idx.tolist():
                        infos[i] = self._entry(infos[i], bool(trunc[i]), full[i])
                else:
                    rows = rows.copy()
                    envs = rows[:, 0].view(np.int32)
                    for k, i in enumerate(envs.tolist()):
                        infos[i] = self._entry(infos[i], bool(trunc[i]), rows[k, 1:])
            dirty.extend(idx.tolist())
        if self.cfg.wrapper_mode:
            w = self.get_info("wrapper").cpu().numpy()
            for i in np.nonzero((w[:, 0] > 0.5) | (w[:, 1] > 0.5))[0].tolist():
                if self.copy_outputs and not infos[i]:
                    infos[i] = {}
                infos[i]["scripted"] = bool(w[i, 1])
                infos[i]["phase"] = PHASE[int(w[i, 0])]
                dirty.append(i)
        return obs, rew, done, infos

# ... 89 lines not shown
```

Baseline: 70.13 million.

## Move near-contact envs into dedicated solo waves and skip idle contact solves

Adds extra single-env "solo" waves at the front of the step grid. Environments whose links are close to the ground (by a clearance test) are moved into these waves, so the env that needs the expensive limit/contact path no longer forces its whole 16-env wave through that path. The moved envs are parked in the original tiles, which skip their stores. A wave that has no active contacts or limits now skips the contact solver entirely. The change adds double- and triple-buffered move lists, extra launch blocks, tile parking copies and one-step latency in migration, which costs bookkeeping and risks correctness.

Result: faster. 78.54 million (median of 6 runs) (+12.0%).

```diff
diff --git a/include/qs_amd.h b/include/qs_amd.h
--- a/include/qs_amd.h
+++ b/include/qs_amd.h
@@ -152,12 +152,14 @@
        QS_COUNTER_LIMIT_PATH_SUBSTEPS = 4,
        QS_COUNTER_SELF_NARROW_SUBSTEPS = 5,
        QS_COUNTER_RESET_STALLS = 6,
-       QS_COUNTER_LOOKAHEAD_BACKLOG = 7      };
+       QS_COUNTER_LOOKAHEAD_BACKLOG = 7,
+       QS_COUNTER_SOLO_PATH_SUBSTEPS = 8     };
 int qs_counter(qs_handle* h, int which, uint64_t* value);
 int qs_counters_async(qs_handle* h, uint64_t* dev_out);
 int qs_enable_timing(qs_handle* h, int on);
 int qs_last_step_kernel_ms(qs_handle* h, float* ms);
 int qs_settle_lanes(qs_handle* h, int on);
+int qs_solo_waves(qs_handle* h, int f, float reach);
 int qs_set_trace(qs_handle* h, int env, float* rows);
 
 typedef struct qs_norm qs_norm;
diff --git a/quadruped-springs_amd/csrc/qs_core.h b/quadruped-springs_amd/csrc/qs_core.h
--- a/quadruped-springs_amd/csrc/qs_core.h
+++ b/quadruped-springs_amd/csrc/qs_core.h
@@ -1321,7 +1321,9 @@
                 QS_PHASE_G(45)
             }
         }
-        if (RACK ? rack : (SOFT || (!HOT && soft))) {
+        if (!HOT && !soft && !rack && !T::any(qand(qnot(rare_mine), qor(act_m, any_lim)))) {
+            o.foot_force = zero; s.warm = zero;
+        } else if (RACK ? rack : (SOFT || (!HOT && soft))) {
             if (HOT && !RACK) payload_rows(cfg, Pr, s, vs, Rx, Ry, Rz, Sm, Ld, blk, pay_c);
             if (HOT && RACK) rack_rows(cfg, s, vs, Rx, Ry, Rz, Sm, Ld, blk, pay_c);
             if (cfg.solver_residual_threshold > 0.0f) solve_and_integrate<3, true, true>(cfg, Pr.mu, s, o, rows, Sm, Ld, BK, R, &pay_c);
diff --git a/quadruped-springs_amd/csrc/qs_hip.hip b/quadruped-springs_amd/csrc/qs_hip.hip
--- a/quadruped-springs_amd/csrc/qs_hip.hip
+++ b/quadruped-springs_amd/csrc/qs_hip.hip
@@ -24,7 +24,7 @@
 }
 __device__ __forceinline__ void keep_loaded(const float4& v) { asm volatile("" ::"v"(v.x), "v"(v.y), "v"(v.z), "v"(v.w)); }
 __device__ __forceinline__ void keep_loaded(float v) { asm volatile("" ::"v"(v)); }
-template <int PER> __device__ __forceinline__ void tile_load_rounds(float4* __restrict__ dst, const float4* __restrict__ src, int nenv, int stride4, int per_rt) {
+template <int PER> __device__ __forceinline__ void tile_load_rounds(float4* __restrict__ dst, const float4* __restrict__ src, const float4* __restrict__ park, int nenv, int stride4, int per_rt) {
     constexpr int MAX_PER = QS_REC_END / 4;
     constexpr int ROUNDS = PER > 0 ? (QS_ENVS_PER_WAVE * PER + QS_WAVE - 1) / QS_WAVE : (QS_ENVS_PER_WAVE * MAX_PER + QS_WAVE - 1) / QS_WAVE;
     const int per = PER > 0 ? PER : per_rt, total = QS_ENVS_PER_WAVE * per;
@@ -35,7 +35,8 @@
         const int i = (int)threadIdx.x + r * QS_WAVE;
         const bool in = (PER > 0 && (QS_ENVS_PER_WAVE * PER) % QS_WAVE == 0) || i < total;
         const int e = PER > 0 ? i / PER : (int)(((unsigned)i * inv) >> 20), o = i - e * per;
-        v[r] = src[in ? (e < nenv ? e : 0) * (QS_REC / 4) + o : 0];
+        const float4* const from = e < nenv ? src + e * (QS_REC / 4) : park;
+        v[r] = in ? from[o] : src[0];
     }
     if (!(PER > 0 && (QS_ENVS_PER_WAVE * PER) % QS_WAVE == 0)) {
 #pragma unroll
@@ -50,15 +51,24 @@
         }
     }
 }
-__device__ __forceinline__ void tile_load(float* lds, const float* __restrict__ g, int first_env, int n_envs, int extent, int stride = QS_REC_END) {
+__device__ __forceinline__ void tile_load(float* lds, const float* __restrict__ g, int first_env, int n_envs, int extent, int stride = QS_REC_END, const float* __restrict__ parked = nullptr) {
     const float4* src = reinterpret_cast<const float4*>(g + (size_t)first_env * QS_REC);
     float4* dst = reinterpret_cast<float4*>(lds);
+    const float4* park = parked ? reinterpret_cast<const float4*>(parked) : src;
     const int nenv = min(QS_ENVS_PER_WAVE, n_envs - first_env);
-    if (extent == QS_HOT) tile_load_rounds<QS_HOT / 4>(dst, src, nenv, stride / 4, 0);
-    else if (extent == QS_SETTLE_END) tile_load_rounds<QS_SETTLE_END / 4>(dst, src, nenv, stride / 4, 0);
-    else tile_load_rounds<0>(dst, src, nenv, stride / 4, extent / 4);
-}
-template <int PER> __device__ __forceinline__ void tile_store_rounds(float4* __restrict__ dst, const float4* __restrict__ src, int nenv, int stride4, int b4, int per_rt) {
+    if (extent == QS_HOT) tile_load_rounds<QS_HOT / 4>(dst, src, park, nenv, stride / 4, 0);
+    else if (extent == QS_SETTLE_END) tile_load_rounds<QS_SETTLE_END / 4>(dst, src, park, nenv, stride / 4, 0);
+    else tile_load_rounds<0>(dst, src, park, nenv, stride / 4, extent / 4);
+}
+__device__ __forceinline__ void tile_park(float* lds, const float* __restrict__ parked, unsigned long long slots, int extent, int stride) {
+    const float4* src = reinterpret_cast<const float4*>(parked);
+    for (int e = 0; e < QS_ENVS_PER_WAVE; e++) {
+        if (!((slots >> (4 * e)) & 1ull)) continue;
+        float4* dst = reinterpret_cast<float4*>(lds + e * stride);
+        for (int i = threadIdx.x; i < extent / 4; i += QS_WAVE) dst[i] = src[i];
+    }
+}
+template <int PER> __device__ __forceinline__ void tile_store_rounds(float4* __restrict__ dst, const float4* __restrict__ src, int nenv, int stride4, int b4, int per_rt, unsigned long long skip) {
     constexpr int MAX_PER = QS_REC_END / 4;
     constexpr int ROUNDS = PER > 0 ? (QS_ENVS_PER_WAVE * PER + QS_WAVE - 1) / QS_WAVE : (QS_ENVS_PER_WAVE * MAX_PER + QS_WAVE - 1) / QS_WAVE;
     const int per = PER > 0 ? PER : per_rt, total = nenv * per;
@@ -75,19 +85,19 @@
 #pragma unroll
     for (int r = 0; r < ROUNDS; r++) {
         const int i = (int)threadIdx.x + r * QS_WAVE;
-        if (i < total) { const int e = PER > 0 ? i / PER : (int)(((unsigned)i * inv) >> 20), o = i - e * per + b4; dst[e * (QS_REC / 4) + o] = v[r]; }
-    }
-}
-__device__ __forceinline__ void tile_store(const float* lds, float* __restrict__ g, int first_env, int n_envs, int begin, int end, int stride = QS_REC_END) {
+        if (i < total) { const int e = PER > 0 ? i / PER : (int)(((unsigned)i * inv) >> 20), o = i - e * per + b4; if (!((skip >> (4 * e)) & 1ull)) dst[e * (QS_REC / 4) + o] = v[r]; }
+    }
+}
+__device__ __forceinline__ void tile_store(const float* lds, float* __restrict__ g, int first_env, int n_envs, int begin, int end, int stride = QS_REC_END, unsigned long long skip = 0ull) {
     float4* dst = reinterpret_cast<float4*>(g + (size_t)first_env * QS_REC);
     const float4* src = reinterpret_cast<const float4*>(lds);
     const int nenv = min(QS_ENVS_PER_WAVE, n_envs - first_env);
-    if (begin == QS_RW_BEGIN && end == QS_HOT) tile_store_rounds<(QS_HOT - QS_RW_BEGIN) / 4>(dst, src, nenv, stride / 4, QS_RW_BEGIN / 4, 0);
-    else if (begin == QS_RW_BEGIN && end == QS_SETTLE_END) tile_store_rounds<(QS_SETTLE_END - QS_RW_BEGIN) / 4>(dst, src, nenv, stride / 4, QS_RW_BEGIN / 4, 0);
-    else tile_store_rounds<0>(dst, src, nenv, stride / 4, begin / 4, (end - begin) / 4);
-}
-
-__device__ __forceinline__ void obs_store(const float* s_obs, int nrow, int od, int first, float* __restrict__ obs_out, bool fused, float* __restrict__ obs_keep) {
+    if (begin == QS_RW_BEGIN && end == QS_HOT) tile_store_rounds<(QS_HOT - QS_RW_BEGIN) / 4>(dst, src, nenv, stride / 4, QS_RW_BEGIN / 4, 0, skip);
+    else if (begin == QS_RW_BEGIN && end == QS_SETTLE_END) tile_store_rounds<(QS_SETTLE_END - QS_RW_BEGIN) / 4>(dst, src, nenv, stride / 4, QS_RW_BEGIN / 4, 0, skip);
+    else tile_store_rounds<0>(dst, src, nenv, stride / 4, begin / 4, (end - begin) / 4, skip);
+}
+
+__device__ __forceinline__ void obs_store(const float* s_obs, int nrow, int od, int first, float* __restrict__ obs_out, bool fused, float* __restrict__ obs_keep, unsigned long long skip = 0ull) {
     const unsigned inv = (65536u + (unsigned)od - 1u) / (unsigned)od;
     const int row = fused ? od + 2 : od, total = nrow * od;
     constexpr int ROUNDS = QS_ENVS_PER_WAVE * QS_MAX_OBS / QS_WAVE;
@@ -105,6 +115,7 @@
         const int i = (int)threadIdx.x + r * QS_WAVE;
         if (i < total) {
             const int e = (int)(((unsigned)i * inv) >> 16), o = i - e * od;
+            if ((skip >> (4 * e)) & 1ull) continue;
             obs_out[(size_t)(first + e) * row + o] = v[r];
             obs_keep[(size_t)first * od + i] = v[r];
         }
@@ -118,6 +129,8 @@
     int K;
 };
 #define QS_COHORTS 5
+#define QS_SOLO_DEFAULT 128
+#define QS_SOLO_REACH_DEFAULT 0.02f
 #define QS_MAX_SLICE 2048
 struct SettleLanes { float* staging; const int2* stage_jobs; int n_env_waves, slice; int wave0[QS_COHORTS + 1] ,
                      spawn[QS_COHORTS], last[QS_COHORTS], settle_n[QS_COHORTS]; };
@@ -126,12 +139,40 @@
 struct TermTail { float* rows; int cap, parity; };
 struct PushTab { float* rows; };
 enum { QS_PUSH_F = 8, QS_PUSH_REM = 6, QS_PUSH_FRAME = 7 };
+#define QS_SOLO_MAX 512
+struct SoloWaves { const float* parked;
+                   const int* moved_rd; int* moved_wr; const int* list_rd; int* list_wr; int F, rd, wr, clr; float reach; };
 enum { CTL_SETTLE_SUBSTEPS = 0, CTL_RESETS = 1, CTL_SERVED = 2, CTL_SETTLED = 3, CTL_BACKLOG = 4, CTL_STALLS = 6,
        CTL_R = 8 , CTL_TERM_CNT = 8 + QS_COHORTS , CTL_DEV = 10 + QS_COHORTS ,
        CTL_PUSH_REFUSED = 22 + QS_COHORTS ,
        CTL_RENDER_REFUSED = 23 + QS_COHORTS ,
        CTL_FORK_REFUSED = 24 + QS_COHORTS ,
-       CTL_N = 25 + QS_COHORTS };
+       CTL_SOLO_CNT = 25 + QS_COHORTS ,
+       CTL_SOLO_PATH = 28 + QS_COHORTS ,
+       CTL_N = 29 + QS_COHORTS };
+static_assert(CTL_DEV + QS_DEVCTR_SOLO_PATH == CTL_SOLO_PATH, "the solo waves' counter sits where count_rare_path (qs_lane.h) counts it");
+
+__device__ __forceinline__ float link_clearance(const float* rec) {
+    using namespace qs::go1;
+    const float fx = LaneDev::fx(), sy = LaneDev::sy();
+    const float x = rec[R_QUAT], y = rec[R_QUAT + 1], z = rec[R_QUAT + 2], w = rec[R_QUAT + 3];
+    const float sc = 2.0f / (x * x + y * y + z * z + w * w);
+    const float Rzx = (x * z - w * y) * sc, Rzy = (y * z + w * x) * sc, Rzz = 1.0f - (x * x + y * y) * sc;
+    const float zc = rec[R_POS + 2];
+    const float q1 = LaneDev::ld_leg(rec, R_Q, 3), q2 = LaneDev::ld_leg(rec, R_Q + 1, 3), q3 = LaneDev::ld_leg(rec, R_Q + 2, 3);
+    const float s1 = __sinf(q1), c1 = __cosf(q1), s2 = __sinf(q2), c2 = __cosf(q2), s23 = __sinf(q2 + q3), c23 = __cosf(q2 + q3);
+    const float p1x = fx * HIP_X, p1y = sy * HIP_Y;
+    const float p2x = p1x, p2y = p1y + c1 * (sy * THIGH_Y), p2z = s1 * (sy * THIGH_Y);
+    const float p3x = p2x + s2 * LEG_Z, p3y = p2y - s1 * c2 * LEG_Z, p3z = p2z + c1 * c2 * LEG_Z;
+    const float az = Rzy * c1 + Rzz * s1;
+    const float gx2 = Rzx * c2 + Rzy * s1 * s2 - Rzz * c1 * s2, gx3 = Rzx * c23 + Rzy * s1 * s23 - Rzz * c1 * s23;
+    const float gp1 = Rzx * p1x + Rzy * p1y, gp2 = Rzx * p2x + Rzy * p2y + Rzz * p2z, gp3 = Rzx * p3x + Rzy * p3y + Rzz * p3z;
+    const float h_trunk = zc + Rzx * (fx * TRUNK_HALF[0]) + Rzy * (sy * TRUNK_HALF[1]) - fabsf(Rzz) * TRUNK_HALF[2];
+    const float h_hip = zc + gp1 - HIP_CYL_HALF_LEN * fabsf(az) - HIP_CYL_R * sqrtf(fmaxf(1.0f - az * az, 0.0f));
+    const float th_off = fabsf(gx2) * THIGH_HALF[0] + fabsf(az) * THIGH_HALF[1], cf_off = (fabsf(gx3) + fabsf(az)) * CALF_HALF[0];
+    const float h_th_hi = zc + gp2 - th_off, h_th_lo = zc + gp3 - th_off, h_cf_hi = zc + gp3 - cf_off;
+    return fminf(fminf(fminf(h_trunk - THR_TRUNK, h_hip - THR_HIP), fminf(h_th_hi, h_th_lo) - THR_THIGH), h_cf_hi - THR_CALF);
+}
 
 __device__ __forceinline__ float copy_settled(float* rec, const float* __restrict__ src, bool block) {
     static_assert(R_PARAMS == 0 && R_PARAMS + QS_PARAM_DIM == R_POS, "parameters and rigid-body state are one range");
@@ -203,54 +244,69 @@
                                                  uint8_t* __restrict__ trunc_out, float* __restrict__ obs_keep,
                                                  float* __restrict__ term_obs, LookAhead la,
                                                  unsigned long long* __restrict__ stats, SettleLanes lanes, TraceTap tap, DemoTab demo, TermTail tail,
-                                                 PushTab push) {
+                                                 PushTab push, SoloWaves solo) {
     using E = Env<LaneDev, CONE, false, false, RACK>;
     using EH = Env<LaneDev, CONE, true, SOFT, RACK>;
     extern __shared__ __attribute__((aligned(16))) float s_dyn[];
-    const qs_config& cfg = *cfgp;
+    const int F = (WAVES == 1 && !SOFT && !RACK) ? solo.F : 0;
+    const bool solo_wave = (int)blockIdx.x < F;
+    const int bid = (int)blockIdx.x - F;
+    const qs_config& cfg = solo_wave ? reinterpret_cast<const QsDevCfg*>(cfgp)[1].cfg : *cfgp;
     const int ls = (RACK || cfg.payload_soft) ? (int)QS_REC_END : (int)QS_INFO_END;
     float* const s_rec = s_dyn;
     float* const s_obs = s_dyn + QS_ENVS_PER_WAVE * ls;
     float* const s_act = s_obs + QS_ENVS_PER_WAVE * QS_MAX_OBS;
     QS_PHASE_BEGIN
     if (tail.rows && blockIdx.x == 0 && threadIdx.x == 0) stats[CTL_TERM_CNT + (tail.parity ^ 1)] = 0ull;
-    const bool settling = (int)blockIdx.x >= lanes.n_env_waves;
-    const int sw = (int)blockIdx.x - lanes.n_env_waves;
+    if (F > 0 && blockIdx.x == 0 && threadIdx.x == 0) stats[CTL_SOLO_CNT + solo.clr] = 0ull;
+    int solo_env = 0;
+    if (solo_wave) {
+        const unsigned long long cnt = stats[CTL_SOLO_CNT + solo.rd];
+        if ((unsigned long long)blockIdx.x >= cnt) return;
+        solo_env = solo.list_rd[blockIdx.x];
+        if ((unsigned)solo_env >= (unsigned)cfg.n_envs) return;
+    }
+    const bool settling = bid >= lanes.n_env_waves;
+    const int sw = bid - lanes.n_env_waves;
     int cohort = 0;
 #pragma unroll
     for (int c = 1; c < QS_COHORTS; c++) cohort += settling && sw >= lanes.wave0[c] ? 1 : 0;
-    const int first = settling ? cohort * lanes.slice + (sw - lanes.wave0[cohort]) * QS_ENVS_PER_WAVE : (int)blockIdx.x * QS_ENVS_PER_WAVE;
-    const int limit = settling ? cohort * lanes.slice + (int)stats[CTL_R + cohort] : cfg.n_envs;
+    const int first = settling ? cohort * lanes.slice + (sw - lanes.wave0[cohort]) * QS_ENVS_PER_WAVE : (solo_wave ? solo_env : bid * QS_ENVS_PER_WAVE);
+    const int limit = settling ? cohort * lanes.slice + (int)stats[CTL_R + cohort] : (solo_wave ? first + 1 : cfg.n_envs);
     if (first >= limit) return;
     const int settle_n = settling ? lanes.settle_n[cohort] : 0;
     if (settling && settle_n == 0) return;
     float* const base = settling ? lanes.staging : recs;
     const int slot = threadIdx.x >> 2;
     const int env = first + slot;
-    const bool valid = env < limit;
     const int d = cfg.action_dim, od = cfg.obs_dim;
     QS_PHASE(26)
     float a_pre[3] = {0.0f, 0.0f, 0.0f};
     float p_rem = 0.0f;
     int2 job = make_int2(0, 0);
+    int moved = 0;
     if (!settling) {
 #pragma unroll
         for (int j = 0; j < 3; j++) {
             const int k = (int)(threadIdx.x & 3u) + 4 * j;
-            if (k < d && valid) a_pre[j] = actions[(size_t)env * d + k];
+            if (k < d && env < limit) a_pre[j] = actions[(size_t)env * d + k];
         }
-        if (push.rows && valid) p_rem = push.rows[(size_t)env * QS_PUSH_F + QS_PUSH_REM];
-    } else job = lanes.stage_jobs[valid ? env : first];
+        if (F > 0 && !solo_wave && env < limit) moved = solo.moved_rd[env];
+        if (push.rows && env < limit) p_rem = push.rows[(size_t)env * QS_PUSH_F + QS_PUSH_REM];
+    } else job = lanes.stage_jobs[env < limit ? env : first];
     const bool spawn = settling && lanes.spawn[cohort], last = settling && lanes.last[cohort];
     const int load_extent = settling ? (spawn ? 0 : ((RACK || cfg.payload_soft) ? (int)TILE_ALL : (int)QS_SETTLE_END)) : (RACK ? (int)TILE_ALL : tile_extent(cfg, false));
-    if (load_extent > 0) tile_load(s_rec, base, first, limit, load_extent, ls);
+    if (load_extent > 0) tile_load(s_rec, base, first, limit, load_extent, ls, settling ? nullptr : solo.parked);
     if (spawn || last) zero_tile_tail(s_rec, load_extent, ls);
+    const bool valid = env < limit && moved == 0;
+    const unsigned long long not_mine = F > 0 ? __ballot(moved != 0) : 0ull;
+    if (__builtin_expect(not_mine != 0ull, 0)) tile_park(s_rec, solo.parked, not_mine, load_extent, ls);
     QS_PHASE(27)
     if (!settling) {
 #pragma unroll
         for (int j = 0; j < 3; j++) {
             const int k = (int)(threadIdx.x & 3u) + 4 * j;
-            if (k < d) s_act[slot * 12 + k] = a_pre[j];
+            if (k < d) s_act[slot * 12 + k] = valid || solo.parked == nullptr ? a_pre[j] : cfg.settle_action[k];
         }
     }
     QS_PHASE(28)
@@ -263,7 +319,7 @@
     if (spawn) { E::settle_spawn(cfg, rec, gid, job.y); LaneDev::sync(); }
     const bool any_trace = tap.rows != nullptr && !settling && tap.env >= first && tap.env < first + QS_ENVS_PER_WAVE;
     QS_PHASE(13)
-    float* const trow = any_trace && env == tap.env ? tap.rows : nullptr;
+    float* const trow = any_trace && valid && env == tap.env ? tap.rows : nullptr;
     const bool any_push = push.rows != nullptr && __any(p_rem > 0.0f);
     const float* const prow = any_push ? push.rows + (size_t)(valid ? env : first) * QS_PUSH_F : nullptr;
     typename E::StepOut r;
@@ -281,6 +337,20 @@
         return;
     }
     const bool dn = r.done > 0.5f;
+    const int store_n = solo_wave ? first + 1 : cfg.n_envs;
+    if (F > 0) {
+        LaneDev::sync();
+        float clr = link_clearance(rec);
+        clr = fminf(clr, LaneDev::xorl<1>(clr)); clr = fminf(clr, LaneDev::xorl<2>(clr));
+        if (valid && (threadIdx.x & 3) == 0) {
+            int mv = 0;
+            if (clr < solo.reach && !dn) {
+                const unsigned long long ticket = atomicAdd(&stats[CTL_SOLO_CNT + solo.wr], 1ull);
+                if (ticket < (unsigned long long)F) { solo.list_wr[ticket] = env; mv = 1; }
+            }
+            solo.moved_wr[env] = mv;
+        }
+    }
     if (any_push && valid && p_rem > 0.0f && (threadIdx.x & 3) == 0)
         push.rows[(size_t)env * QS_PUSH_F + QS_PUSH_REM] = dn ? 0.0f : fmaxf(p_rem - (float)cfg.action_repeat, 0.0f);
     if (valid && (threadIdx.x & 3) == 0) {
@@ -315,8 +385,8 @@
             LaneDev::sync();
             if (__builtin_expect(__any(do_reset && !ahead), 0)) {
                 __syncthreads();
-                tile_store(s_rec, recs, first, cfg.n_envs, QS_RW_BEGIN, RACK ? (int)TILE_ALL : tile_extent(cfg, true), ls);
-                obs_store(s_obs, min(QS_ENVS_PER_WAVE, cfg.n_envs - first), od, first, obs_out, rew_out == nullptr, obs_keep);
+                tile_store(s_rec, recs, first, store_n, QS_RW_BEGIN, RACK ? (int)TILE_ALL : tile_extent(cfg, true), ls, not_mine);
+                obs_store(s_obs, min(QS_ENVS_PER_WAVE, store_n - first), od, first, obs_out, rew_out == nullptr, obs_keep, not_mine);
                 __syncthreads();
                 E::reset(cfg, rec, ob, gid, true);
                 if (do_reset && !ahead && (threadIdx.x & 3) == 0) atomicAdd(&stats[CTL_SETTLE_SUBSTEPS], (unsigned long long)cfg.settle_steps);
@@ -337,16 +407,16 @@
         }
     }
     __syncthreads();
-    tile_store(s_rec, recs, first, cfg.n_envs, any_reset ? 0 : (int)QS_RW_BEGIN, RACK ? (int)TILE_ALL : tile_extent(cfg, true), ls);
-    obs_store(s_obs, min(QS_ENVS_PER_WAVE, cfg.n_envs - first), od, first, obs_out, rew_out == nullptr, obs_keep);
+    tile_store(s_rec, recs, first, store_n, any_reset ? 0 : (int)QS_RW_BEGIN, RACK ? (int)TILE_ALL : tile_extent(cfg, true), ls, not_mine);
+    obs_store(s_obs, min(QS_ENVS_PER_WAVE, store_n - first), od, first, obs_out, rew_out == nullptr, obs_keep, not_mine);
     QS_PHASE(15)
 }
 
 #define QS_STEP_ARGS const qs_config* __restrict__ cfgp, float* __restrict__ recs, const float* __restrict__ actions, float* __restrict__ obs_out,    \
                      float* __restrict__ rew_out, uint8_t* __restrict__ done_out, uint8_t* __restrict__ trunc_out, float* __restrict__ obs_keep, \
                      float* __restrict__ term_obs, LookAhead la, unsigned long long* __restrict__ stats, SettleLanes lanes, TraceTap tap, DemoTab demo, TermTail tail, \
-                     PushTab push
-#define QS_STEP_PASS cfgp, recs, actions, obs_out, rew_out, done_out, trunc_out, obs_keep, term_obs, la, stats, lanes, tap, demo, tail, push
+                     PushTab push, SoloWaves solo
+#define QS_STEP_PASS cfgp, recs, actions, obs_out, rew_out, done_out, trunc_out, obs_keep, term_obs, la, stats, lanes, tap, demo, tail, push, solo
 template <bool CONE, bool SOFT> __global__ __launch_bounds__(QS_WAVE, 1) void k_step(QS_STEP_ARGS) { step_body<CONE, 1, SOFT>(QS_STEP_PASS); }
 template <bool CONE, bool SOFT> __global__ __launch_bounds__(QS_WAVE, 2) void k_step_dense(QS_STEP_ARGS) { step_body<CONE, 2, SOFT>(QS_STEP_PASS); }
 template <bool CONE> __global__ __launch_bounds__(QS_WAVE, 1) void k_step_rack(QS_STEP_ARGS) { step_body<CONE, 1, CONE, true>(QS_STEP_PASS); }
@@ -506,6 +576,15 @@
 template <bool CONE> __global__ __launch_bounds__(QS_WAVE, 1) void k_lookahead_fill_rack(const qs_config* __restrict__ cfgp, LookAhead la) { QS_RESET_LDS lookahead_fill_body<CONE, true>(cfgp, la, s_rec, s_obs); }
 #undef QS_RESET_LDS
 
+__global__ void k_make_parked(const float* __restrict__ slot, float* __restrict__ parked) {
+    for (int i = threadIdx.x; i < QS_REC; i += blockDim.x) {
+        float v = i < QS_REC_END ? slot[i] : 0.0f;
+        if (i == R_POS + 2) v += 5.0f;
+        if ((i >= R_VLIN && i < R_VLIN + 3) || (i >= R_VANG && i < R_VANG + 3) || (i >= R_QD && i < R_QD + 12) || (i >= R_WARM && i < R_WARM + 4)) v = 0.0f;
+        parked[i] = v;
+    }
+}
+
 __global__ void k_gather(const float* __restrict__ recs, int n, int off, int dim, float* __restrict__ out, int as_int) {
     int i = blockIdx.x * blockDim.x + threadIdx.x;
     if (i >= n * dim) return;
@@ -586,6 +665,8 @@
     int push_live;
     int n_simd, step_variant;
     unsigned long long* d_stats;
+    float* d_parked; int* d_moved; int* d_solo_list;
+    int solo_f, solo_live; float solo_reach; long long solo_tick;
     TermTail tail;
     struct HostPath* host;
     hipEvent_t ev0, ev1;
@@ -682,7 +763,7 @@
         h->step_variant = v ? atoi(v) : 0;
     }
     const size_t n = (size_t)cfg->n_envs;
-    QS_HIP(hipMalloc(&h->d_cfg, sizeof(QsDevCfg)));
+    QS_HIP(hipMalloc(&h->d_cfg, 2 * sizeof(QsDevCfg)));
     QS_HIP(hipMalloc(&h->d_rec, n * QS_REC * sizeof(float)));
     QS_HIP(hipMalloc(&h->d_obs, n * cfg->obs_dim * sizeof(float)));
     QS_HIP(hipMalloc(&h->d_term_obs, n * cfg->obs_dim * sizeof(float)));
@@ -695,6 +776,8 @@
         for (int i = 0; i < 3; i++) dc.rack_pos[i] = h->rack.anchor_pos[i];
         for (int i = 0; i < 4; i++) dc.rack_quat[i] = h->rack.anchor_quat[i];
         QS_HIP(hipMemcpy(h->d_cfg, &dc, sizeof(dc), hipMemcpyHostToDevice));
+        dc.solo = 1;
+        QS_HIP(hipMemcpy(reinterpret_cast<QsDevCfg*>(h->d_cfg) + 1, &dc, sizeof(dc), hipMemcpyHostToDevice));
     }
     QS_HIP(hipMemset(h->d_obs, 0, n * cfg->obs_dim * sizeof(float)));
     QS_HIP(hipMemset(h->d_term_obs, 0, n * cfg->obs_dim * sizeof(float)));
@@ -730,6 +813,19 @@
         });
         QS_HIP(hipGetLastError());
         h->lanes_on = 1;
+        QS_HIP(hipMalloc(&h->d_parked, QS_REC * sizeof(float)));
+        QS_HIP(hipMalloc(&h->d_moved, 2 * n * sizeof(int)));
+        QS_HIP(hipMalloc(&h->d_solo_list, 3 * QS_SOLO_MAX * sizeof(int)));
+        QS_HIP(hipMemsetAsync(h->d_moved, 0, 2 * n * sizeof(int), h->stream));
+        QS_HIP(hipMemsetAsync(h->d_solo_list, 0, 3 * QS_SOLO_MAX * sizeof(int), h->stream));
+        hipLaunchKernelGGL(k_make_parked, dim3(1), dim3(256), 0, h->stream, h->la.slots, h->d_parked);
+        QS_HIP(hipGetLastError());
+        const char* sv = getenv("QS_SOLO_WAVES");
+        const char* rv = getenv("QS_SOLO_REACH");
+        h->solo_f = sv ? atoi(sv) : QS_SOLO_DEFAULT;
+        if (h->solo_f < 0) h->solo_f = 0;
+        if (h->solo_f > QS_SOLO_MAX) h->solo_f = QS_SOLO_MAX;
+        h->solo_reach = rv ? (float)atof(rv) : QS_SOLO_REACH_DEFAULT;
     }
     QS_HIP(hipStreamSynchronize(h->stream));
     return 0;
@@ -749,6 +845,9 @@
     if (h->d_demo) hipFree(h->d_demo);
     if (h->d_push) hipFree(h->d_push);
     if (h->d_fork) hipFree(h->d_fork);
+    if (h->d_parked) hipFree(h->d_parked);
+    if (h->d_moved) hipFree(h->d_moved);
+    if (h->d_solo_list) hipFree(h->d_solo_list);
     host_path_free(h);
     if (h->ev0) hipEventDestroy(h->ev0);
     if (h->ev1) hipEventDestroy(h->ev1);
@@ -821,6 +920,15 @@
     }
     if (on && !h->lanes_on) h->tick = 0;
     h->lanes_on = on ? 1 : 0;
+    return 0;
+}
+
+int qs_solo_waves(qs_handle* h, int f, float reach) {
+    if (!h) QS_FAIL(-1, "null handle");
+    if (f < -1 || f > QS_SOLO_MAX) QS_FAIL(-1, "qs_solo_waves: between 0 (off) and %d solo waves per launch (-1: as it is), got %d", QS_SOLO_MAX, f);
+    if (f > 0 && !h->d_parked) QS_FAIL(-1, "solo waves need the look-ahead reset states (cfg.reset_lookahead > 0, not QS_RAND_KEEP): the parked record is made from one");
+    if (f >= 0) h->solo_f = f;
+    if (reach > 0.0f) h->solo_reach = reach;
     return 0;
 }
 
@@ -849,15 +957,41 @@
     PushTab push; push.rows = h->push_live ? h->d_push : nullptr;
     int grid = lanes.n_env_waves;
     bool lanes_fit = true;
-    if (h->la.K > 0 && h->lanes_on) {
+    const bool with_lanes = h->la.K > 0 && h->lanes_on;
+    auto lanes_share = [&](int extra, bool* fit) {
+        const int free_simd = h->n_simd - lanes.n_env_waves - extra;
+        int base_waves = h->slice / QS_ENVS_PER_WAVE;
+        if (h->step_variant != 2 && free_simd / QS_COHORTS >= 64 && base_waves > free_simd / QS_COHORTS) base_waves = free_simd / QS_COHORTS;
+        *fit = lanes.n_env_waves + extra + (with_lanes ? QS_COHORTS * base_waves : 0) <= h->n_simd;
+        return base_waves;
+    };
+    int F = 0;
+    if (h->solo_f > 0 && h->d_parked && h->cfg.body_contacts && !h->cfg.payload_soft && !h->rack.on && h->step_variant != 2) {
+        bool fit = false;
+        lanes_share(h->solo_f, &fit);
+        if (fit) F = h->solo_f;
+    }
+    if (F != h->solo_live) {
+        if (h->d_moved) QS_HIP(hipMemsetAsync(h->d_moved, 0, 2 * (size_t)h->cfg.n_envs * sizeof(int), h->stream));
+        QS_HIP(hipMemsetAsync(h->d_stats + CTL_SOLO_CNT, 0, 3 * sizeof(unsigned long long), h->stream));
+        h->solo_live = F; h->solo_tick = 0;
+    }
+    SoloWaves solo;
+    memset(&solo, 0, sizeof(solo));
+    solo.parked = h->d_parked;
+    if (F > 0) {
+        const long long i = h->solo_tick++;
+        solo.F = F; solo.rd = (int)(i % 3); solo.wr = (int)((i + 1) % 3); solo.clr = (int)((i + 2) % 3); solo.reach = h->solo_reach;
+        solo.moved_rd = h->d_moved + (size_t)(i & 1) * h->cfg.n_envs; solo.moved_wr = h->d_moved + (size_t)((i + 1) & 1) * h->cfg.n_envs;
+        solo.list_rd = h->d_solo_list + solo.rd * QS_SOLO_MAX; solo.list_wr = h->d_solo_list + solo.wr * QS_SOLO_MAX;
+        grid += F;
+    }
+    if (with_lanes) {
         const int rep = h->cfg.action_repeat, epoch = (h->cfg.settle_steps + rep - 1) / rep;
         const int slice = h->slice;
         lanes.staging = h->d_staging; lanes.stage_jobs = h->d_stage_jobs; lanes.slice = slice;
-        const int free_simd = h->n_simd - lanes.n_env_waves;
         const int cohort_waves = slice / QS_ENVS_PER_WAVE;
-        int base_waves = cohort_waves;
-        if (h->step_variant != 2 && free_simd / QS_COHORTS >= 64 && base_waves > free_simd / QS_COHORTS) base_waves = free_simd / QS_COHORTS;
-        lanes_fit = n_waves(h->cfg.n_envs) + QS_COHORTS * base_waves <= h->n_simd;
+        const int base_waves = lanes_share(F, &lanes_fit);
         for (int c = 0; c < QS_COHORTS; c++) {
             const long long t = h->tick - (long long)c * epoch / QS_COHORTS;
             lanes.wave0[c] = c * cohort_waves;
@@ -881,7 +1015,7 @@
     const qs::Build build = handle_build(h);
     auto launch = [&](auto kernel) {
         hipLaunchKernelGGL(kernel, dim3(grid), dim3(QS_WAVE), build.step_lds_bytes(), h->stream, h->d_cfg, h->d_rec, actions, obs, rew, done, trunc,
-                           h->d_obs, h->d_term_obs, h->la, h->d_stats, lanes, tap, demo, tail, push);
+                           h->d_obs, h->d_term_obs, h->la, h->d_stats, lanes, tap, demo, tail, push, solo);
     };
     qs::with_build(build, [&](auto cone, auto soft, auto rack) {
         if constexpr (rack()) launch(dense ? k_step_dense_rack<cone()> : k_step_rack<cone()>);
@@ -1189,6 +1323,7 @@
         break;
     case QS_COUNTER_LIMIT_PATH_SUBSTEPS: QS_HIP(hipMemcpy(&v, &h->d_stats[CTL_DEV + QS_DEVCTR_RARE_PATH], sizeof(v), hipMemcpyDeviceToHost)); break;
     case QS_COUNTER_SELF_NARROW_SUBSTEPS: QS_HIP(hipMemcpy(&v, &h->d_stats[CTL_DEV + QS_DEVCTR_SELF_NARROW], sizeof(v), hipMemcpyDeviceToHost)); break;
+    case QS_COUNTER_SOLO_PATH_SUBSTEPS: QS_HIP(hipMemcpy(&v, &h->d_stats[CTL_SOLO_PATH], sizeof(v), hipMemcpyDeviceToHost)); break;
     default: QS_FAIL(-1, "unknown counter %d", which);
     }
     *value = v;
diff --git a/quadruped-springs_amd/csrc/qs_lane.h b/quadruped-springs_amd/csrc/qs_lane.h
--- a/quadruped-springs_amd/csrc/qs_lane.h
+++ b/quadruped-springs_amd/csrc/qs_lane.h
@@ -68,9 +68,9 @@
 QS_FN bool qnot(bool a) { return !a; }
 QS_FN float qflag(bool m) { return m ? 1.0f : 0.0f; }
 
-struct QsDevCfg { qs_config cfg; unsigned long long* counters; float rack_pos[3]; float rack_quat[4]; };
+struct QsDevCfg { qs_config cfg; unsigned long long* counters; float rack_pos[3]; float rack_quat[4]; int solo; };
 #if defined(__HIPCC__)
-enum { QS_DEVCTR_RARE_PATH = 0, QS_DEVCTR_SELF_NARROW = 1 };
+enum { QS_DEVCTR_RARE_PATH = 0, QS_DEVCTR_SELF_NARROW = 1, QS_DEVCTR_SOLO_PATH = 18  };
 struct LaneDev {
     using V = float;
     using M = bool;
@@ -120,7 +120,13 @@
     static QS_DEV float first(float x) { return x; }
     static QS_DEV void opaque(float& x) { asm volatile("" : "+v"(x)); }
     static QS_DEV float* wave_scratch(float* row) { return row - (size_t)(threadIdx.x >> 2) * QS_MAX_OBS; }
-    static QS_DEV void count_rare_path(const qs_config& cfg) { if (threadIdx.x == 0) atomicAdd(&reinterpret_cast<const QsDevCfg&>(cfg).counters[QS_DEVCTR_RARE_PATH], 1ull); }
+    static QS_DEV void count_rare_path(const qs_config& cfg) {
+        if (threadIdx.x == 0) {
+            const QsDevCfg& dc = reinterpret_cast<const QsDevCfg&>(cfg);
+            atomicAdd(&dc.counters[QS_DEVCTR_RARE_PATH], 1ull);
+            if (dc.solo) atomicAdd(&dc.counters[QS_DEVCTR_SOLO_PATH], 1ull);
+        }
+    }
     static QS_DEV void count_self_narrow(const qs_config& cfg) { if (threadIdx.x == 0) atomicAdd(&reinterpret_cast<const QsDevCfg&>(cfg).counters[QS_DEVCTR_SELF_NARROW], 1ull); }
     static QS_DEV void sync() {
         __builtin_amdgcn_fence(__ATOMIC_RELEASE, "wavefront");
diff --git a/quadruped-springs_amd/qs_amd/lib.py b/quadruped-springs_amd/qs_amd/lib.py
--- a/quadruped-springs_amd/qs_amd/lib.py
+++ b/quadruped-springs_amd/qs_amd/lib.py
@@ -12,7 +12,7 @@
 EXPORTS = (
     "qs_create", "qs_destroy", "qs_set_stream", "qs_reset", "qs_reset_to", "qs_get_obs", "qs_step", "qs_step_fused", "qs_get_state", "qs_set_state",
     "qs_info_dim", "qs_get_info", "qs_set_params", "qs_stats", "qs_enable_timing", "qs_last_step_kernel_ms",
-    "qs_settle_lanes", "qs_host_step_begin", "qs_host_step_end", "qs_set_trace", "qs_counter", "qs_counters_async", "qs_set_demo", "qs_set_demo_counter", "qs_set_external_wrench", "qs_create_ex", "qs_set_rack", "qs_render", "qs_render_states", "qs_last_error", "qs_version", "qs_abi_version",
+    "qs_settle_lanes", "qs_solo_waves", "qs_host_step_begin", "qs_host_step_end", "qs_set_trace", "qs_counter", "qs_counters_async", "qs_set_demo", "qs_set_demo_counter", "qs_set_external_wrench", "qs_create_ex", "qs_set_rack", "qs_render", "qs_render_states", "qs_last_error", "qs_version", "qs_abi_version",
     "qs_norm_create", "qs_norm_destroy", "qs_norm_dims", "qs_norm_set_stream", "qs_norm_set_stats", "qs_norm_get_stats", "qs_norm_reset", "qs_norm_step",
     "qs_norm_step_io", "qs_host_set_norm",
     "qs_policy_create", "qs_policy_destroy", "qs_policy_set_stream", "qs_policy_param_count", "qs_policy_set_params", "qs_policy_act",
@@ -102,6 +102,8 @@
     if hasattr(lib, "qs_render"):
         lib.qs_render.argtypes = [vp, vp, i32, C.POINTER(QsCamera), i32, i32, vp, vp, vp]
         lib.qs_render_states.argtypes = [vp, vp, i32, C.POINTER(QsCamera), i32, i32, vp, vp, vp, vp]
+    if hasattr(lib, "qs_solo_waves"):
+        lib.qs_solo_waves.argtypes = [vp, i32, C.c_float]
     lib.qs_counter.argtypes = [vp, C.c_int, C.POINTER(C.c_uint64)]
     lib.qs_counters_async.argtypes = [vp, vp]
     f32, f64, pd = C.c_float, C.c_double, C.POINTER(C.c_double)
diff --git a/quadruped-springs_amd/qs_amd/vec_env.py b/quadruped-springs_amd/qs_amd/vec_env.py
--- a/quadruped-springs_amd/qs_amd/vec_env.py
+++ b/quadruped-springs_amd/qs_amd/vec_env.py
@@ -15,10 +15,12 @@
 
 
 class QuadrupedVecEnv(SB3VecEnv):
-    def __init__(self, num_envs=1, device=0, auto_reset=True, reset_lookahead=None, copy_outputs=True, **env_kwargs):
+    def __init__(self, num_envs=1, device=0, auto_reset=True, reset_lookahead=None, copy_outputs=True, solo_waves=None, solo_reach=None, **env_kwargs):
         cfg, meta = build_config(n_envs=num_envs, auto_reset=auto_reset, **env_kwargs)
         cfg.reset_lookahead = int((16 if auto_reset else 0) if reset_lookahead is None else reset_lookahead)
         self._setup(cfg, meta, device, copy_outputs)
+        if solo_waves is not None or solo_reach is not None:
+            self.solo_waves(solo_waves, solo_reach)
 
     @classmethod
     def from_config(cls, cfg, meta, device=0, copy_outputs=True, load_demo=True):
@@ -371,7 +373,7 @@
         return dict(settle_substeps=a.value, resets=b.value)
 
     COUNTERS = dict(settle_substeps=0, resets=1, lookahead_served=2, lookahead_settled=3, limit_path_substeps=4, self_narrow_substeps=5,
-                    reset_stalls=6, lookahead_backlog=7)
+                    reset_stalls=6, lookahead_backlog=7, solo_path_substeps=8)
 
     def counter(self, which):
         v = C.c_uint64(0)
@@ -383,6 +385,13 @@
         self._stream()
         _lib.check(self.lib.qs_counters_async(self.h, self._ptr(out)))
         return out
+
+    def solo_waves(self, f=None, reach=None):
+        if not hasattr(self.lib, "qs_solo_waves"):
+            raise RuntimeError("this libqs_hip.so has no qs_solo_waves: rebuild it (python quadruped-springs_amd/build.py --force)")
+        if f is None:
+            f = -1
+        _lib.check(self.lib.qs_solo_waves(self.h, int(f), float(reach if reach is not None else 0.0)))
 
     def enable_timing(self, on=True):
         self._stream()
```
